# vita-epfl/CrowdNav

Hardware: AMD Instinct MI355X
Metric: env-steps/sec (whole node), 4096 envs x 5 humans, ORCA step (higher is better)
Workload: dtype f32 ORCA solve + f64 env step

## Files before the change

crowdnav_amd/_lib.py:

```python
import ctypes as C
import os

HERE = os.path.dirname(os.path.abspath(__file__))
LIB_PATH = os.environ.get('CROWDNAV_AMD_LIB') or os.path.join(HERE, 'lib', 'libcrowdnav_amd.so')
ABI_VERSION = 12

CN_OK, CN_ERR_INVALID, CN_ERR_UNSUPPORTED, CN_ERR_HIP, CN_ERR_NO_DEVICE = 0, -1, -2, -3, -4
INFO_NAMES = ('Nothing', 'Danger', 'ReachGoal', 'Collision', 'Timeout')
NOTHING, DANGER, REACH_GOAL, COLLISION, TIMEOUT = range(5)
ROBOT_EXTERNAL, ROBOT_ORCA = 0, 1
CIRCLE_CROSSING, SQUARE_CROSSING, MIXED = 0, 1, 2
HOLONOMIC, UNICYCLE = 0, 1
RECORD_FIELDS, SUMMARY_FIELDS = 6, 8
LAUNCH_COUNTERS = ('rollout_kernels', 'scheduled_kernels', 'ring_fills', 'async_fills', 'sarl_narrow', 'sarl_decide_steps')
ROLLOUT_ROUTES = ('generic', 'fused', 'fused_split', 'shard')
SARL_ROUTES = ('lds_tile', 'lds_chunked', 'narrow', 'reg_sarl', 'reg_sarl_chunk', 'reg_cadrl', 'reg_lstm', 'reg_lstm2',
               'split_f16')
PRECISIONS = ('f32', 'f16x2')
FLAG_ASYNC_SCENARIO_FILL = 1
HUMANS_ORCA, HUMANS_CONSTANT_VELOCITY = 0, 1
HUMAN_MODELS = ('orca', 'constant_velocity')
MODES_MEAN, MODES_MIN = 0, 1
MODES_REDUCE = ('mean', 'min')
MODES_MAX = 8
PREDICT_CONSTANT_VELOCITY, PREDICT_TO_GOAL = 0, 1
PREDICT_MODELS = ('constant_velocity', 'to_goal')
PREDICT_ALIASES = {'cv': 'constant_velocity'}


class CrowdNavAmdError(RuntimeError):
    def __init__(self, status, message):
        super().__init__('libcrowdnav_amd: %s (status %d)' % (message, status))
        self.status = status


class CnConfig(C.Structure):
    _fields_ = [
        ('num_envs', C.c_int32), ('num_humans', C.c_int32),
        ('time_step', C.c_double), ('time_limit', C.c_double),
        ('success_reward', C.c_double), ('collision_penalty', C.c_double),
        ('discomfort_dist', C.c_double), ('discomfort_penalty_factor', C.c_double),
        ('robot_visible', C.c_int32), ('robot_policy', C.c_int32),
        ('robot_safety_space', C.c_double), ('human_safety_space', C.c_double),
        ('neighbor_dist', C.c_double),
        ('max_neighbors', C.c_int32), ('scenario_rule', C.c_int32),
        ('time_horizon', C.c_double), ('time_horizon_obst', C.c_double),
        ('circle_radius', C.c_double), ('square_width', C.c_double),
        ('human_radius', C.c_double), ('human_v_pref', C.c_double),
        ('robot_radius', C.c_double), ('robot_v_pref', C.c_double),
        ('randomize_attributes', C.c_int32), ('device', C.c_int32),
        ('robot_kinematics', C.c_int32), ('flags', C.c_int32),
    ]


class CnRolloutIo(C.Structure):
    _fields_ = [
        ('seed_base', C.c_uint32), ('seed_mod', C.c_uint32),
        ('episode_limit', C.c_int64), ('env_offset', C.c_int64), ('env_stride', C.c_int64),
        ('record_capacity', C.c_int32),
        ('ep_outcome', C.c_void_p), ('ep_steps', C.c_void_p), ('ep_return', C.c_void_p),
        ('ep_time', C.c_void_p), ('ep_danger', C.c_void_p), ('ep_danger_dmin_sum', C.c_void_p),
        ('ep_count', C.c_void_p), ('cur_steps', C.c_void_p), ('cur_return', C.c_void_p),
        ('cur_danger', C.c_void_p), ('cur_danger_dmin_sum', C.c_void_p),
        ('active', C.c_void_p), ('transitions', C.c_void_p),
        ('summary', C.c_void_p), ('blocks', C.c_void_p), ('blocks_records', C.c_int32),
        ('env_transitions', C.c_void_p),
    ]


class CnLookaheadOut(C.Structure):
    _fields_ = [
        ('ret', C.c_void_p), ('info', C.c_void_p), ('steps', C.c_void_p), ('time', C.c_void_p),
        ('final_state8', C.c_void_p), ('final_theta', C.c_void_p),
    ]


class CnPathModes(C.Structure):
    _fields_ = [
        ('n_modes', C.c_int32), ('reduce', C.c_int32), ('risk_penalty', C.c_double),
        ('human_vel', C.c_void_p), ('weight', C.c_void_p),
    ]


class CnPredictors(C.Structure):
    _fields_ = [
        ('n_modes', C.c_int32), ('model', C.c_int32 * 8), ('reduce', C.c_int32), ('risk_penalty', C.c_double),
        ('human_vel', C.c_void_p), ('weight', C.c_void_p),
    ]


class CnModesOut(C.Structure):
    _fields_ = [
        ('score', C.c_void_p), ('risk', C.c_void_p), ('worst_mode', C.c_void_p), ('worst_info', C.c_void_p),
        ('worst_steps', C.c_void_p), ('worst_time', C.c_void_p),
        ('ret', C.c_void_p), ('info', C.c_void_p), ('steps', C.c_void_p), ('time', C.c_void_p),
    ]


class CnPlanCfg(C.Structure):
    _fields_ = [
        ('n_steps', C.c_int32), ('n_candidates', C.c_int32), ('n_elites', C.c_int32), ('iterations', C.c_int32),
        ('bootstrap', C.c_int32), ('sort_humans', C.c_int32),
        ('init_std', C.c_double), ('min_std', C.c_double), ('smoothing', C.c_double), ('seed', C.c_uint64),
    ]


class CnPlan(C.Structure):
    _fields_ = [
        ('mean', C.c_void_p), ('std', C.c_void_p), ('best_actions', C.c_void_p), ('best_score', C.c_void_p),
        ('action', C.c_void_p), ('candidates', C.c_void_p), ('look', CnLookaheadOut),
        ('value', C.c_void_p), ('score', C.c_void_p), ('order', C.c_void_p),
    ]


class CnTraceOut(C.Structure):
    _fields_ = [
        ('state8', C.c_void_p), ('episode', C.c_void_p), ('step', C.c_void_p),
        ('reward', C.c_void_p), ('info', C.c_void_p), ('dmin', C.c_void_p),
    ]


class CnSarlConfig(C.Structure):
    _fields_ = [
        ('n_actions', C.c_int32), ('with_om', C.c_int32), ('cell_num', C.c_int32), ('om_channel_size', C.c_int32),
        ('cell_size', C.c_double), ('gamma', C.c_double), ('with_global_state', C.c_int32),
        ('mlp1_dims', C.c_int32 * 2), ('mlp2_dims', C.c_int32 * 2), ('attention_dims', C.c_int32 * 3),
        ('mlp3_dims', C.c_int32 * 4), ('model', C.c_int32), ('interaction_dims', C.c_int32 * 4),
        ('constant_velocity_model', C.c_int32), ('precision', C.c_int32),
    ]


_P = C.c_void_p
SYMBOLS = {
    'cn_last_error': (C.c_char_p, []),
    'cn_abi_version': (C.c_int, []),
    'cn_create': (C.c_int, [C.POINTER(CnConfig), C.POINTER(_P)]),
    'cn_destroy': (C.c_int, [_P]),
    'cn_set_stream': (C.c_int, [_P, _P]),
    'cn_sync': (C.c_int, [_P]),
    'cn_set_state': (C.c_int, [_P, _P, _P]),
    'cn_get_state': (C.c_int, [_P, _P, _P]),
    'cn_set_theta': (C.c_int, [_P, _P]),
    'cn_get_theta': (C.c_int, [_P, _P]),
    'cn_get_human_count': (C.c_int, [_P, _P]),
    'cn_drop_robot_sim': (C.c_int, [_P]),
    'cn_drop_sims': (C.c_int, [_P]),
    'cn_set_robot_sim': (C.c_int, [_P, _P, C.c_float]),
    'cn_reset': (C.c_int, [_P, _P, _P, _P]),
    'cn_orca': (C.c_int, [_P, _P]),
    'cn_step': (C.c_int, [_P, _P, C.c_int, _P, _P, _P, _P, _P, _P, _P]),
    'cn_set_gamma': (C.c_int, [_P, C.c_double]),
    'cn_rollout_begin': (C.c_int, [_P, C.POINTER(CnRolloutIo)]),
    'cn_rollout': (C.c_int, [_P, C.POINTER(CnRolloutIo), C.c_int]),
    'cn_rollout_step': (C.c_int, [_P, C.POINTER(CnRolloutIo), _P]),
    'cn_sarl_configure': (C.c_int, [_P, C.POINTER(CnSarlConfig), _P]),
    'cn_sarl_set_weights': (C.c_int, [_P, C.POINTER(_P)]),
    'cn_sarl_select': (C.c_int, [_P, _P, _P, _P]),
    'cn_sarl_select_attention': (C.c_int, [_P, _P, _P, _P, _P]),
    'cn_sarl_explore': (C.c_int, [_P, C.c_double, _P, _P, _P, _P]),
    'cn_sarl_transform': (C.c_int, [_P, _P, C.c_int64, C.c_int]),
    'cn_sarl_sample_step': (C.c_int, [_P, C.c_double, _P, _P, _P, _P, C.c_int64, C.c_int, _P, _P, _P, _P]),
    'cn_sarl_values': (C.c_int, [_P, _P, C.c_int64, _P]),
    'cn_sarl_export': (C.c_int, [_P, C.c_int, _P, C.c_uint64]),
    'cn_rollout_records': (C.c_int, [_P, C.POINTER(CnRolloutIo), C.c_int, _P]),
    'cn_gather_records': (C.c_int, [_P, _P, C.c_int, C.c_int, _P, _P]),
    'cn_records_summary': (C.c_int, [_P, C.c_int64, C.c_int, C.c_int, _P, _P]),
    'cn_rollout_summary': (C.c_int, [_P, C.POINTER(CnRolloutIo), _P]),
    'cn_launch_counts': (C.c_int, [_P, _P]),
    'cn_lagged_fills': (C.c_int, [_P, _P]),
    'cn_mt_random': (C.c_int, [_P, C.c_uint32, C.c_int, _P]),
    'cn_trainer_create': (C.c_int, [C.POINTER(CnSarlConfig), C.c_int, C.c_int, C.c_int, C.POINTER(_P)]),
    'cn_trainer_destroy': (C.c_int, [_P]),
    'cn_trainer_set_stream': (C.c_int, [_P, _P]),
    'cn_train_step': (C.c_int, [_P, C.POINTER(_P), C.POINTER(_P), _P, _P, C.c_int64, _P, C.c_int64, C.c_double, C.c_double, _P]),
    'cn_trainer_steps': (C.c_int, [_P, C.POINTER(C.c_int64)]),
    'cn_rollout_trace': (C.c_int, [_P, C.POINTER(CnRolloutIo), C.c_int, C.POINTER(CnTraceOut)]),
    'cn_rollout_route': (C.c_int, [_P, C.c_int, C.POINTER(C.c_int)]),
    'cn_sarl_network_route': (C.c_int, [_P, C.POINTER(C.c_int)]),
    'cn_rollout_actions': (C.c_int, [_P, C.POINTER(CnRolloutIo), C.c_int, _P, C.POINTER(CnTraceOut)]),
    'cn_lookahead_actions': (C.c_int, [_P, C.c_int, C.c_int, _P, C.POINTER(CnLookaheadOut)]),
    'cn_lookahead_set_human_model': (C.c_int, [_P, C.c_int]),
    'cn_lookahead_get_human_model': (C.c_int, [_P, C.POINTER(C.c_int)]),
    'cn_sarl_state_values': (C.c_int, [_P, _P, _P, C.c_int64, C.c_int, _P]),
    'cn_lookahead_values': (C.c_int, [_P, C.c_int, C.c_int, _P, C.POINTER(CnLookaheadOut), C.c_int, _P, _P]),
    'cn_plan_reset': (C.c_int, [_P, C.POINTER(CnPlanCfg), C.POINTER(CnPlan), _P]),
    'cn_plan_draw': (C.c_int, [_P, C.POINTER(CnPlanCfg), C.POINTER(CnPlan), C.c_uint32]),
    'cn_plan_refit': (C.c_int, [_P, C.POINTER(CnPlanCfg), C.POINTER(CnPlan), C.c_int]),
    'cn_plan_cem': (C.c_int, [_P, C.POINTER(CnPlanCfg), C.POINTER(CnPlan), C.c_uint32]),
    'cn_plan_shift': (C.c_int, [_P, C.POINTER(CnRolloutIo), C.POINTER(CnPlanCfg), C.POINTER(CnPlan)]),
    'cn_plan_rollout': (C.c_int, [_P, C.POINTER(CnRolloutIo), C.c_int, C.POINTER(CnPlanCfg), C.POINTER(CnPlan), C.c_uint32]),
    'cn_plan_mppi_update': (C.c_int, [_P, C.POINTER(CnPlanCfg), C.POINTER(CnPlan), C.c_double, C.c_int, C.c_int]),
    'cn_plan_mppi': (C.c_int, [_P, C.POINTER(CnPlanCfg), C.POINTER(CnPlan), C.c_double, C.c_int, C.c_uint32]),
    'cn_plan_mppi_rollout': (C.c_int, [_P, C.POINTER(CnRolloutIo), C.c_int, C.POINTER(CnPlanCfg), C.POINTER(CnPlan), C.c_double,
                                       C.c_int, C.c_uint32]),
    'cn_lookahead_paths': (C.c_int, [_P, C.c_int, C.c_int, _P, _P, C.POINTER(CnLookaheadOut)]),
    'cn_lookahead_paths_values': (C.c_int, [_P, C.c_int, C.c_int, _P, _P, C.POINTER(CnLookaheadOut), C.c_int, _P, _P]),
    'cn_plan_cem_paths': (C.c_int, [_P, C.POINTER(CnPlanCfg), C.POINTER(CnPlan), _P, C.c_uint32]),
    'cn_plan_mppi_paths': (C.c_int, [_P, C.POINTER(CnPlanCfg), C.POINTER(CnPlan), _P, C.c_double, C.c_int, C.c_uint32]),
    'cn_lookahead_modes': (C.c_int, [_P, C.c_int, C.c_int, _P, C.POINTER(CnPathModes), C.POINTER(CnModesOut)]),
    'cn_plan_cem_modes': (C.c_int, [_P, C.POINTER(CnPlanCfg), C.POINTER(CnPlan), C.POINTER(CnPathModes), C.c_uint32]),
    'cn_plan_mppi_modes': (C.c_int, [_P, C.POINTER(CnPlanCfg), C.POINTER(CnPlan), C.POINTER(CnPathModes), C.c_double, C.c_int,
                                     C.c_uint32]),
    'cn_predict': (C.c_int, [_P, C.c_int, C.c_int, C.POINTER(C.c_int32), _P]),
    'cn_plan_cem_predict_rollout': (C.c_int, [_P, C.POINTER(CnRolloutIo), C.c_int, C.POINTER(CnPlanCfg), C.POINTER(CnPlan),
                                              C.POINTER(CnPredictors), C.c_uint32]),
    'cn_plan_mppi_predict_rollout': (C.c_int, [_P, C.POINTER(CnRolloutIo), C.c_int, C.POINTER(CnPlanCfg), C.POINTER(CnPlan),
                                               C.POINTER(CnPredictors), C.c_double, C.c_int, C.c_uint32]),
    'cn_predict_orca': (C.c_int, [_P, C.c_int, C.c_int, C.c_int, _P]),
    'cn_plan_cem_predict_orca_rollout': (C.c_int, [_P, C.POINTER(CnRolloutIo), C.c_int, C.POINTER(CnPlanCfg), C.POINTER(CnPlan),
                                                   C.POINTER(CnPredictors), C.c_int, C.c_uint32]),
    'cn_plan_mppi_predict_orca_rollout': (C.c_int, [_P, C.POINTER(CnRolloutIo), C.c_int, C.POINTER(CnPlanCfg), C.POINTER(CnPlan),
                                                    C.POINTER(CnPredictors), C.c_int, C.c_double, C.c_int, C.c_uint32]),
    'cn_predict_orca_robot': (C.c_int, [_P, C.c_int, C.c_int, C.c_int, _P, C.c_int64, _P]),
    'cn_plan_cem_predict_orca_nominal_rollout': (C.c_int, [_P, C.POINTER(CnRolloutIo), C.c_int, C.POINTER(CnPlanCfg),
                                                           C.POINTER(CnPlan), C.POINTER(CnPredictors), C.c_int, C.c_uint32]),
    'cn_plan_mppi_predict_orca_nominal_rollout': (C.c_int, [_P, C.POINTER(CnRolloutIo), C.c_int, C.POINTER(CnPlanCfg),
                                                            C.POINTER(CnPlan), C.POINTER(CnPredictors), C.c_int, C.c_double, C.c_int,
                                                            C.c_uint32]),
}

_lib = None


def load():
    global _lib
    if _lib is not None:
        return _lib
    if not os.path.exists(LIB_PATH):
        raise ImportError(
            'crowdnav_amd: %s is missing. Build the HIP library first (make -C crowdnav_amd/csrc, or '
            '__graft_entry__.build()); there is no CPU fallback.' % LIB_PATH)
    lib = C.CDLL(LIB_PATH)
    for name, (res, args) in SYMBOLS.items():
        fn = getattr(lib, name)
        fn.restype = res
        fn.argtypes = args
    got = lib.cn_abi_version()
    if got != ABI_VERSION:
        raise ImportError('crowdnav_amd: library ABI %d != binding ABI %d; rebuild' % (got, ABI_VERSION))
    _lib = lib
    return lib


def check(status):
    if status != CN_OK:
        raise CrowdNavAmdError(status, load().cn_last_error().decode('utf-8', 'replace'))
```

crowdnav_amd/csrc/crowdnav_amd.hip:

```cpp
#include "engine_host.h"
#include "scenario_ring_host.h"
#include "rollout_fused.h"
#include "records_kernels.h"
#include "lookahead_cv_kernel.h"
#include "lookahead_modes_kernel.h"

thread_local char cn_g_err[512] = "";

void cn_launch_orca(cn_engine* e, float* out_vel) {
    pick_maxl(e, [&](auto maxl) {
        pick_bool(e->P.kd, [&](auto kd) {
            hipLaunchKernelGGL((cn::orca_kernel<decltype(maxl)::value, decltype(kd)::value>), dim3(grid_envs(e)), dim3(e->P.threads),
                               e->smem, e->stream, e->P, e->S, out_vel);
        });
    });
}

static bool headline_geometry(const cn::Params& P) {
    return P.A == 6 && P.NC == 5 && P.E == 2 && P.nA == 12 && P.pairs == 60 && P.threads == 64;
}

template <class F>
static void pick_fused(const cn_engine* e, int route, F&& f) {
    if (route == CN_ROUTE_FUSED_SPLIT) {
        if (e->split_assist & cn::kAssistHead) f(cn::rollout_fused_kernel<true, true, cn::kAssistHead>, 2 * cn::kWave);
        else f(cn::rollout_fused_kernel<true, true>, 2 * cn::kWave);
    } else if (headline_geometry(e->P)) {
        f(cn::rollout_fused_kernel<true>, cn::kWave);
    } else {
        f(cn::rollout_fused_kernel<false>, cn::kWave);
    }
}

int cn_lookahead_check(const cn_engine* e, int n_steps, int n_candidates, const double* actions, const cn_lookahead_out* out) {
    if (!actions) return fail(CN_ERR_INVALID, "cn_lookahead_actions: actions is NULL");
    if (!out) return fail(CN_ERR_INVALID, "cn_lookahead_actions: out is NULL");
    if (!out->ret) return fail(CN_ERR_INVALID, "cn_lookahead_actions: out->ret is NULL");
    if (!out->info) return fail(CN_ERR_INVALID, "cn_lookahead_actions: out->info is NULL");
    if (!out->steps) return fail(CN_ERR_INVALID, "cn_lookahead_actions: out->steps is NULL");
    if (!out->time) return fail(CN_ERR_INVALID, "cn_lookahead_actions: out->time is NULL");
    if (n_steps < 0) return fail(CN_ERR_INVALID, "cn_lookahead_actions: n_steps must be >= 0 (got %d)", n_steps);
    if (n_candidates < 1) return fail(CN_ERR_INVALID, "cn_lookahead_actions: n_candidates must be >= 1 (got %d)", n_candidates);
    if (!e) return fail(CN_ERR_INVALID, "cn_lookahead_actions: engine is NULL");
    if (e->P.robot_orca)
        return fail(CN_ERR_INVALID, "cn_lookahead_actions is for CN_ROBOT_EXTERNAL engines (an ORCA robot takes no actions)");
    const uint64_t virtual_envs = (uint64_t)e->P.B * (uint64_t)n_candidates, rows = virtual_envs * (uint64_t)n_steps;
    if (virtual_envs > (uint64_t)INT32_MAX - cn::kWave)
        return fail(CN_ERR_UNSUPPORTED, "cn_lookahead_actions: num_envs * n_candidates = %llu exceeds the %llu branches a launch "
                    "indexes", (unsigned long long)virtual_envs, (unsigned long long)((uint64_t)INT32_MAX - cn::kWave));
    if (rows > ((uint64_t)1 << 59))
        return fail(CN_ERR_UNSUPPORTED, "cn_lookahead_actions: num_envs * n_candidates * n_steps = %llu action rows exceed 2^59",
                    (unsigned long long)rows);
    if (!e->discount || e->discount_len <= 0)
        return fail(CN_ERR_INVALID, "cn_lookahead_actions: the engine has no discount table (cn_set_gamma)");
    return CN_OK;
}

static int upload_look(cn_engine* e, const cn_lookahead_out* out) {
    if (!e->look_valid || std::memcmp(&e->look_host, out, sizeof(*out)) != 0) {
        e->look_host = *out;
        CN_HIP(hipMemcpyAsync(e->look_dev, &e->look_host, sizeof(*out), hipMemcpyHostToDevice, e->stream));
        e->look_valid = true;
    }
    return CN_OK;
}

static cn::CvParams cv_params(const cn_engine* e, int n_steps, int n_candidates) {
    const cn::Params& P = e->P;
    cn::CvParams C{};
    C.B = P.B, C.K = n_candidates, C.A = P.A, C.n_steps = n_steps;
    C.chunks = (n_candidates + cn::kWave - 1) / cn::kWave;
    C.discount_len = e->discount_len, C.discount = e->discount;
    C.dt = P.dt, C.time_limit = P.time_limit, C.success_reward = P.success_reward, C.collision_penalty = P.collision_penalty;
    C.discomfort_dist = P.discomfort_dist, C.discomfort_factor = P.discomfort_factor;
    C.pos = e->S.pos, C.vel = e->S.vel, C.goal = e->S.goal, C.rv = e->S.rv, C.gtime = e->S.gtime, C.theta = e->S.theta;
    return C;
}

extern "C" {

const char* cn_last_error(void) { return cn_g_err; }
int cn_abi_version(void) { return CN_ABI_VERSION; }

static int check_config(const cn_config* c) {
    if (c->num_envs < 1) return fail(CN_ERR_INVALID, "num_envs must be >= 1 (got %d)", c->num_envs);
    if (c->num_humans < 1 || c->num_humans > 63)
        return fail(CN_ERR_UNSUPPORTED, "num_humans must be in 1..63 (got %d)", c->num_humans);
    if (c->max_neighbors < 0 || c->max_neighbors > cn::kMaxNb)
        return fail(CN_ERR_UNSUPPORTED, "max_neighbors must be in 0..%d (got %d)", cn::kMaxNb, c->max_neighbors);
    if (!(c->time_step > 0.0)) return fail(CN_ERR_INVALID, "time_step must be > 0");
    if (c->scenario_rule != CN_CIRCLE_CROSSING && c->scenario_rule != CN_SQUARE_CROSSING && c->scenario_rule != CN_MIXED)
        return fail(CN_ERR_UNSUPPORTED, "scenario_rule %d not supported", c->scenario_rule);
    if (c->scenario_rule == CN_MIXED) {
        if (c->num_humans < 5 || c->num_humans > 8)
            return fail(CN_ERR_UNSUPPORTED, "scenario_rule mixed draws up to 5 humans per episode: num_humans must be in 5..8 (got %d)",
                        c->num_humans);
        if (c->randomize_attributes && c->robot_policy == CN_ROBOT_ORCA)
            return fail(CN_ERR_UNSUPPORTED,
                        "mixed + randomize_attributes + the ORCA robot: the reference rebuilds the robot's rvo2 simulator "
                        "whenever the number of humans changes (orca.py:95-98), which the per-env radius capture does not model");
    }
    if (c->robot_policy != CN_ROBOT_EXTERNAL && c->robot_policy != CN_ROBOT_ORCA)
        return fail(CN_ERR_INVALID, "robot_policy %d unknown", c->robot_policy);
    if (c->robot_kinematics != CN_HOLONOMIC && c->robot_kinematics != CN_UNICYCLE)
        return fail(CN_ERR_INVALID, "robot_kinematics %d unknown", c->robot_kinematics);
    if (c->robot_kinematics == CN_UNICYCLE && c->robot_policy == CN_ROBOT_ORCA)
        return fail(CN_ERR_INVALID, "the ORCA robot policy is holonomic (orca.py:59); a unicycle robot needs CN_ROBOT_EXTERNAL");
    int ndev = 0;
    if (hipGetDeviceCount(&ndev) != hipSuccess || ndev == 0)
        return fail(CN_ERR_NO_DEVICE, "no HIP device visible: the MI355X engine has no CPU fallback");
    if (c->device < 0 || c->device >= ndev) return fail(CN_ERR_INVALID, "device %d out of range", c->device);
    return CN_OK;
}

static void copy_config(cn_engine* e) {
    const cn_config* c = &e->cfg;
    cn::Params& P = e->P;
    P.robot_visible = c->robot_visible ? 1 : 0;
    P.robot_orca = c->robot_policy == CN_ROBOT_ORCA;
    P.robot_unicycle = c->robot_kinematics == CN_UNICYCLE;
    P.dt = c->time_step;
    P.time_limit = c->time_limit;
    P.success_reward = c->success_reward;
    P.collision_penalty = c->collision_penalty;
    P.discomfort_dist = c->discomfort_dist;
    P.discomfort_factor = c->discomfort_penalty_factor;
    P.robot_safety = c->robot_safety_space;
    P.human_safety = c->human_safety_space;
    P.orca.neighbor_dist = (float)c->neighbor_dist;
    P.orca.inv_time_horizon = 1.0f / (float)c->time_horizon;
    P.orca.inv_time_step = 1.0f / (float)c->time_step;
    P.orca.max_neighbors = c->max_neighbors;
    e->C.num_agents = c->num_humans + 1;
    e->C.rule = c->scenario_rule;
    e->C.randomize = c->randomize_attributes ? 1 : 0;
    e->C.circle_radius = c->circle_radius;
    e->C.square_width = c->square_width;
    e->C.discomfort_dist = c->discomfort_dist;
    e->C.human_radius = c->human_radius;
    e->C.human_v_pref = c->human_v_pref;
    e->C.robot_radius = c->robot_radius;
    e->C.robot_v_pref = c->robot_v_pref;
}

static void pick_geometry(cn_engine* e) {
    const cn_config* c = &e->cfg;
    cn::Params& P = e->P;
    P.B = c->num_envs;
    P.A = c->num_humans + 1;
    P.NC = P.A - 1;
    const int e_max = cn::kWave / P.A;
    const bool small_lp = (P.NC < c->max_neighbors ? P.NC : c->max_neighbors) <= 5;
    int e_want = env_int("CROWDNAV_AMD_ENVS_PER_WAVE", small_lp ? (P.B > 2048 ? 2 : 1) : (P.B + 4095) / 4096);
    P.E = e_want < 1 ? 1 : (e_want > e_max ? e_max : e_want);
    int w_want = env_int("CROWDNAV_AMD_WAVES_PER_BLOCK", 1);
    const int w_useful = (P.E * P.A * P.NC + cn::kWave - 1) / cn::kWave;
    if (w_want > w_useful) w_want = w_useful;
    if (w_want > cn::kMaxBlock / cn::kWave) w_want = cn::kMaxBlock / cn::kWave;
    P.threads = cn::kWave * (w_want < 1 ? 1 : w_want);
    P.nA = P.E * P.A;
    P.pairs = P.nA * P.NC;
    e->maxl = small_lp ? 5 : 10;
    P.kd = P.A > cn::kKdLeaf ? 1 : 0;
    P.kdl = cn::kd_layout(P.nA, P.A, P.E);
    e->smem = cn::smem_bytes(P.nA, P.pairs, e->maxl, P.A, P.E);
}

static void read_knobs(cn_engine* e) {
    const cn_config* c = &e->cfg;
    cn::Params& P = e->P;
    P.sched = -1;
    e->sched_min = env_int("CROWDNAV_AMD_SCHED_MIN_STEPS", 24);
    e->sched_force = env_int("CROWDNAV_AMD_SCHED_FORCE", 0) != 0;
    e->sched_reserve = env_int("CROWDNAV_AMD_DYN_RESERVE", 0);
    e->sched_dynamic = env_int("CROWDNAV_AMD_SCHED_DYNAMIC", 1) != 0;
    e->dyn_visits = env_int("CROWDNAV_AMD_DYN_VISITS", 0);
    P.dyn_visits = 3;
    e->use_fused = env_int("CROWDNAV_AMD_FUSED", 1) != 0;
    e->fused_split = env_int("CROWDNAV_AMD_FUSED_SPLIT", 1);
    e->split_assist = env_int("CROWDNAV_AMD_SPLIT_ASSIST", 1) != 0 ? cn::kAssistHead : 0;
    int cap_log2 = env_int("CROWDNAV_AMD_MAX_ATTEMPTS_LOG2", c->num_humans > 8 ? 23 : 20);
    if (cap_log2 < 6) cap_log2 = 6;
    if (cap_log2 > 40) cap_log2 = 40;
    e->C.max_attempts = 1ull << cap_log2;
    hipDeviceProp_t prop;
    const bool ok = hipGetDeviceProperties(&prop, c->device) == hipSuccess && prop.multiProcessorCount > 0;
    e->sched_slots = 12 * (ok ? prop.multiProcessorCount : 256);
    e->ring.configure(e, ok ? prop.multiProcessorCount : 256);
    e->split_slots = 0;
    if (ok && headline_geometry(P))
        pick_fused(e, CN_ROUTE_FUSED_SPLIT, [&](auto kernel, int threads) {
            int per_cu = 0;
            if (hipOccupancyMaxActiveBlocksPerMultiprocessor(&per_cu, kernel, threads, e->smem) == hipSuccess)
                e->split_slots = per_cu * prop.multiProcessorCount;
        });
}

static int alloc_state(cn_engine* e) {
    const cn::Params& P = e->P;
    const size_t n = (size_t)P.B * P.A;
    int rc = CN_OK;
    cn::StateView& S = e->S;
    if ((rc = dev_alloc(e, &S.pos, n)) || (rc = dev_alloc(e, &S.vel, n)) || (rc = dev_alloc(e, &S.goal, n)) ||
        (rc = dev_alloc(e, &S.rv, n)) || (rc = dev_alloc(e, &S.gtime, (size_t)P.B)) ||
        (rc = dev_alloc(e, &S.theta, (size_t)P.B)) ||
        (rc = dev_alloc(e, &S.rsim_radius, n)) || (rc = dev_alloc(e, &S.rsim_max_speed, (size_t)P.B)) ||
        (rc = dev_alloc(e, &S.rsim_valid, (size_t)P.B)) || (rc = dev_alloc(e, &S.mt_key, (size_t)624 * P.B)) ||
        (rc = dev_alloc(e, &S.mt_pos, (size_t)P.B)) || (rc = dev_alloc(e, &e->probe_key, (size_t)624)) ||
        (rc = e->ring.create(e)) ||
        (rc = dev_alloc(e, &e->summary_scratch, (size_t)cn::kSummaryBlocks * cn::kSummaryFields + 1)) ||
        (rc = dev_alloc(e, &S.ep_word, (size_t)P.B)) || (rc = dev_alloc(e, &S.dyn_queue, (size_t)P.B + 1)) ||
        (rc = dev_alloc(e, &S.kd_order, P.kd ? n * cn::kd_row_bytes(P.A) : (size_t)4)) ||
        (rc = dev_alloc(e, &S.kd_valid, P.kd ? n : (size_t)4)) ||
        (rc = dev_alloc(e, &S.wg_partial, (size_t)P.B * (CN_SUMMARY_FIELDS + 1))) ||
        (rc = dev_alloc(e, &S.group_partial, (size_t)cn::kEpilogueGroups * (CN_SUMMARY_FIELDS + 1))) ||
        (rc = dev_alloc(e, &S.tickets, (size_t)(cn::kEpilogueGroups + 1) * cn::kTicketStride)) ||
        (rc = dev_alloc(e, &e->io_dev, (size_t)1)) || (rc = dev_alloc(e, &e->C.error, (size_t)1)) ||
        (rc = dev_alloc(e, &e->S_dev, (size_t)1)) || (rc = dev_alloc(e, &e->look_dev, (size_t)1)))
        return rc;
    e->S.error = e->C.error;
    if (hipMemcpy(e->S_dev, &e->S, sizeof(cn::StateView), hipMemcpyHostToDevice) != hipSuccess)
        return fail(CN_ERR_HIP, "cn_create: state view upload failed");
    return CN_OK;
}

int cn_create(const cn_config* c, cn_engine** out) {
    if (!c || !out) return fail(CN_ERR_INVALID, "cn_create: NULL argument");
    *out = nullptr;
    int rc = check_config(c);
    if (rc) return rc;
    CN_HIP(hipSetDevice(c->device));

    cn_engine* e = new (std::nothrow) cn_engine();
    if (!e) return fail(CN_ERR_INVALID, "out of host memory");
    e->cfg = *c;
    copy_config(e);
    pick_geometry(e);
    read_knobs(e);
    if ((rc = alloc_state(e)) || (rc = cn_set_gamma(e, 0.9))) {
        cn_destroy(e);
        return rc;
    }
    *out = e;
    return CN_OK;
}

int cn_destroy(cn_engine* e) {
    if (!e) return CN_OK;
    (void)hipSetDevice(e->cfg.device);
    (void)hipStreamSynchronize(e->stream);
    e->ring.destroy();
    e->alloc_rollback(cn_engine::AllocMark{});
    if (e->discount) (void)hipFree(e->discount);
    cn_sarl_release(e);
    delete e;
    return CN_OK;
}

int cn_set_stream(cn_engine* e, void* hip_stream) {
    if (!e) return fail(CN_ERR_INVALID, "engine is NULL");
    e->stream = static_cast<hipStream_t>(hip_stream);
    e->orca_fresh = false;
    return CN_OK;
}

int cn_sync(cn_engine* e) {
    int rc = bind(e);
    if (rc) return rc;
    CN_HIP(hipStreamSynchronize(e->stream));
    if ((rc = e->ring.drain(e))) return rc;
    int gen_error = 0;
    CN_HIP(hipMemcpy(&gen_error, e->C.error, sizeof(int), hipMemcpyDeviceToHost));
    if (gen_error) {
        CN_HIP(hipMemset(e->C.error, 0, sizeof(int)));
        if (gen_error & 4)
            return fail(CN_ERR_HIP,
                        "the shard kernel's dynamic schedule: a workgroup waited ~2 s for an env's previous visit and went on "
                        "without it (results of this rollout are not to be trusted); CROWDNAV_AMD_SCHED_DYNAMIC=0 selects the "
                        "static schedule");
        if (gen_error & 2)
            return fail(CN_ERR_INVALID,
                        "cn_sarl_explore needs each env's numpy stream: (re)start the episodes with cn_reset (the scenario "
                        "ring of cn_rollout_* and the wave generator used for more than 8 humans do not keep it)");
        return fail(CN_ERR_INVALID,
                    "scenario generation gave up on a human after %llu rejected placements (the reference's rejection "
                    "sampling would not have terminated either: too many humans for this circle/square); the affected "
                    "scenario holds an overlapping placement",
                    e->C.max_attempts);
    }
    return CN_OK;
}

namespace {

__global__ void pack_state_kernel(int n, const double* state8, cn::StateView S) {
    const int i = blockIdx.x * blockDim.x + threadIdx.x;
    if (i >= n) return;
    const double* s = state8 + (size_t)i * 8;
    S.pos[i] = make_double2(s[0], s[1]);
    S.vel[i] = make_double2(s[2], s[3]);
    S.goal[i] = make_double2(s[4], s[5]);
    S.rv[i] = make_double2(s[6], s[7]);
}

__global__ void unpack_state_kernel(int n, double* state8, cn::StateView S) {
    const int i = blockIdx.x * blockDim.x + threadIdx.x;
    if (i >= n) return;
    double* s = state8 + (size_t)i * 8;
    const double2 p = S.pos[i], v = S.vel[i], g = S.goal[i], q = S.rv[i];
    s[0] = p.x, s[1] = p.y, s[2] = v.x, s[3] = v.y, s[4] = g.x, s[5] = g.y, s[6] = q.x, s[7] = q.y;
}

}

int cn_set_state(cn_engine* e, const double* state8, const double* global_time) {
    int rc = bind(e);
    if (rc || (rc = e->ring.settle(e))) return rc;
    const int n = e->P.B * e->P.A;
    if (state8) hipLaunchKernelGGL(pack_state_kernel, dim3((n + 255) / 256), dim3(256), 0, e->stream, n, state8, e->S);
    if (global_time)
        CN_HIP(hipMemcpyAsync(e->S.gtime, global_time, sizeof(double) * e->P.B, hipMemcpyDeviceToDevice, e->stream));
    CN_HIP(hipGetLastError());
    return CN_OK;
}

int cn_get_state(cn_engine* e, double* state8, double* global_time) {
    int rc = bind(e);
    if (rc || (rc = e->ring.settle(e))) return rc;
    const int n = e->P.B * e->P.A;
    if (state8) hipLaunchKernelGGL(unpack_state_kernel, dim3((n + 255) / 256), dim3(256), 0, e->stream, n, state8, e->S);
    if (global_time)
        CN_HIP(hipMemcpyAsync(global_time, e->S.gtime, sizeof(double) * e->P.B, hipMemcpyDeviceToDevice, e->stream));
    CN_HIP(hipGetLastError());
    return CN_OK;
}

int cn_set_theta(cn_engine* e, const double* theta) {
    int rc = bind(e);
    if (rc) return rc;
    if (!theta) return fail(CN_ERR_INVALID, "cn_set_theta: NULL");
    CN_HIP(hipMemcpyAsync(e->S.theta, theta, sizeof(double) * e->P.B, hipMemcpyDeviceToDevice, e->stream));
    return CN_OK;
}

int cn_get_theta(cn_engine* e, double* theta) {
    int rc = bind(e);
    if (rc) return rc;
    if (!theta) return fail(CN_ERR_INVALID, "cn_get_theta: NULL");
    CN_HIP(hipMemcpyAsync(theta, e->S.theta, sizeof(double) * e->P.B, hipMemcpyDeviceToDevice, e->stream));
    return CN_OK;
}

namespace {
__global__ void human_count_kernel(int B, int A, const double2* pos, int32_t* out) {
    const int b = blockIdx.x * blockDim.x + threadIdx.x;
    if (b >= B) return;
    int n = 0;
    for (int i = 1; i < A; ++i) n += cn::is_parked(pos[(size_t)b * A + i]) ? 0 : 1;
    out[b] = n;
}
}

int cn_get_human_count(cn_engine* e, int32_t* count) {
    int rc = bind(e);
    if (rc) return rc;
    if (!count) return fail(CN_ERR_INVALID, "cn_get_human_count: NULL");
    hipLaunchKernelGGL(human_count_kernel, dim3((e->P.B + 255) / 256), dim3(256), 0, e->stream, e->P.B, e->P.A, e->S.pos, count);
    CN_HIP(hipGetLastError());
    return CN_OK;
}

namespace {
__global__ void set_robot_sim_kernel(int B, int A, const float* radii, float max_speed, cn::StateView S) {
    const int i = blockIdx.x * blockDim.x + threadIdx.x;
    if (i >= B * A) return;
    S.rsim_radius[i] = radii[i % A];
    if (i % A == 0) {
        S.rsim_max_speed[i / A] = max_speed;
        S.rsim_valid[i / A] = 1;
    }
}
}

int cn_set_robot_sim(cn_engine* e, const float* radii_host, float max_speed) {
    int rc = bind(e);
    if (rc) return rc;
    if (!radii_host) return fail(CN_ERR_INVALID, "cn_set_robot_sim: NULL");
    float* staged = reinterpret_cast<float*>(e->probe_key);
    CN_HIP(hipMemcpyAsync(staged, radii_host, sizeof(float) * e->P.A, hipMemcpyHostToDevice, e->stream));
    CN_HIP(hipStreamSynchronize(e->stream));
    hipLaunchKernelGGL(set_robot_sim_kernel, dim3((e->P.B * e->P.A + 255) / 256), dim3(256), 0, e->stream, e->P.B, e->P.A,
                       staged, max_speed, e->S);
    CN_HIP(hipGetLastError());
    return CN_OK;
}

int cn_drop_robot_sim(cn_engine* e) {
    int rc = bind(e);
    if (rc) return rc;
    CN_HIP(hipMemsetAsync(e->S.rsim_valid, 0, (size_t)e->P.B, e->stream));
    if (e->P.kd)
        CN_HIP(hipMemset2DAsync(e->S.kd_valid, (size_t)e->P.A, 0, 1, (size_t)e->P.B, e->stream));
    return CN_OK;
}

int cn_drop_sims(cn_engine* e) {
    int rc = cn_drop_robot_sim(e);
    if (rc) return rc;
    if (e->P.kd) CN_HIP(hipMemsetAsync(e->S.kd_valid, 0, (size_t)e->P.B * e->P.A, e->stream));
    return CN_OK;
}

int cn_reset(cn_engine* e, const uint32_t* seeds, const uint8_t* mask, uint64_t* draws) {
    int rc = bind(e);
    if (rc || (rc = e->ring.settle(e))) return rc;
    if (!seeds) return fail(CN_ERR_INVALID, "cn_reset: seeds is NULL");
    if (e->ring.gen_wave)
        hipLaunchKernelGGL(cn::reset_wave_kernel, dim3(e->P.B), dim3(cn::kWave), 0, e->stream, e->P, e->C, e->S, seeds, mask,
                           draws);
    else
        hipLaunchKernelGGL(cn::reset_kernel, dim3(grid_lanes(e)), dim3(cn::kWave), 0, e->stream, e->P, e->C, e->S, seeds, mask,
                           draws);
    CN_HIP(hipGetLastError());
    return CN_OK;
}

int cn_orca(cn_engine* e, float* out_vel) {
    int rc = bind(e);
    if (rc) return rc;
    if (!out_vel) return fail(CN_ERR_INVALID, "cn_orca: out_vel is NULL");
    cn_launch_orca(e, out_vel);
    CN_HIP(hipGetLastError());
    return CN_OK;
}

int cn_step(cn_engine* e, const double* action, int update, double* reward, uint8_t* done, uint8_t* info,
            double* dmin, double* action_out, float* orca_vel, double* obs) {
    int rc = bind(e);
    if (rc || (rc = e->ring.settle(e))) return rc;
    if (!reward || !done || !info) return fail(CN_ERR_INVALID, "cn_step: reward/done/info must not be NULL");
    if (e->P.robot_orca && action)
        return fail(CN_ERR_INVALID, "cn_step: action must be NULL when robot_policy == CN_ROBOT_ORCA");
    if (!e->P.robot_orca && !action)
        return fail(CN_ERR_INVALID, "cn_step: action is required when robot_policy == CN_ROBOT_EXTERNAL");
    cn::StepIo io{action, reward, done, info, dmin, action_out, orca_vel, obs, update ? 1 : 0};
    pick_maxl_uni_kd(e, [&](auto maxl, auto uni, auto kd) {
        hipLaunchKernelGGL((cn::step_kernel<decltype(maxl)::value, decltype(uni)::value, decltype(kd)::value>), dim3(grid_envs(e)),
                           dim3(e->P.threads), e->smem, e->stream, e->P, e->S, io);
    });
    CN_HIP(hipGetLastError());
    return CN_OK;
}

int cn_set_gamma(cn_engine* e, double gamma) {
    int rc = bind(e);
    if (rc) return rc;
    const int len = (int)std::ceil(e->cfg.time_limit / e->cfg.time_step) + 8;
    if (len > cn::kMaxDiscount)
        return fail(CN_ERR_UNSUPPORTED, "time_limit / time_step = %d steps per episode exceeds the %d the rollout kernel tabulates",
                    len - 8, cn::kMaxDiscount - 8);
    std::vector<double> table((size_t)len);
    for (int t = 0; t < len; ++t) table[(size_t)t] = std::pow(gamma, t * e->cfg.time_step * e->cfg.robot_v_pref);
    CN_HIP(hipStreamSynchronize(e->stream));
    if (e->discount) CN_HIP(hipFree(e->discount));
    e->discount = nullptr;
    CN_HIP(hipMalloc(reinterpret_cast<void**>(&e->discount), sizeof(double) * len));
    CN_HIP(hipMemcpy(e->discount, table.data(), sizeof(double) * len, hipMemcpyHostToDevice));
    e->discount_len = len;
    return CN_OK;
}

static int upload_io(cn_engine* e, const cn_rollout_io* io) {
    if (e->io_valid && std::memcmp(&e->io_host, io, sizeof(*io)) == 0) return CN_OK;
    if (e->rollout_begun && (io->seed_base != e->begin_seed_base || io->seed_mod != e->begin_seed_mod))
        return fail(CN_ERR_INVALID, "rollout io: seed_base / seed_mod (%u / %u) differ from cn_rollout_begin's (%u / %u); call "
                    "cn_rollout_begin to renumber the episodes", io->seed_base, io->seed_mod, e->begin_seed_base, e->begin_seed_mod);
    int rc = e->ring.drain(e);
    if (rc) return rc;
    e->io_host = *io;
    CN_HIP(hipMemcpyAsync(e->io_dev, &e->io_host, sizeof(*io), hipMemcpyHostToDevice, e->stream));
    e->io_valid = true;
    return CN_OK;
}

static int check_io(const cn_engine* e, const cn_rollout_io* io) {
    if (!io) return fail(CN_ERR_INVALID, "rollout io is NULL");
    if (io->seed_mod == 0) return fail(CN_ERR_INVALID, "seed_mod must be >= 1");
    if (!io->ep_count || !io->cur_steps || !io->cur_return || !io->active)
        return fail(CN_ERR_INVALID, "rollout io: ep_count, cur_steps, cur_return and active are required");
    if (io->record_capacity < 0) return fail(CN_ERR_INVALID, "record_capacity must be >= 0");
    if (io->blocks && io->blocks_records < 1) return fail(CN_ERR_INVALID, "rollout io: blocks needs blocks_records >= 1");
    if (io->env_offset < 0 || io->env_stride < io->env_offset + e->P.B)
        return fail(CN_ERR_INVALID, "rollout io: need env_offset >= 0 and env_stride >= env_offset + num_envs");
    return CN_OK;
}

int cn_rollout_begin(cn_engine* e, const cn_rollout_io* io) {
    int rc = bind(e);
    if (rc) return rc;
    if ((rc = check_io(e, io)) || (rc = e->ring.drain(e))) return rc;
    e->rollout_begun = false;
    if ((rc = upload_io(e, io))) return rc;
    e->rollout_begun = true, e->begin_seed_base = io->seed_base, e->begin_seed_mod = io->seed_mod;
    return e->ring.begin(e, io->seed_mod);
}

static int rollout_route(const cn_engine* e, const double* action) {
    const cn::Params& P = e->P;
    static const bool use_geom20 = env_int("CROWDNAV_AMD_GEOM20", 1) != 0;
    if (e->use_fused && e->ring.mode != ScenarioRing::Fill::WorkList && e->maxl == 5 && !P.robot_unicycle && P.NC <= cn::kFusedMaxNC && P.pairs <= cn::kWave &&
        P.nA * 5 <= cn::kWave && P.threads == cn::kWave) {
#if defined(CN_PHASE_TIMING) || defined(CN_WAVE_TRACE)
        (void)action;
        return CN_ROUTE_FUSED;
#else
        const bool split = e->fused_split != 0 && headline_geometry(P) && P.robot_orca && action == nullptr &&
                           (grid_envs(e) <= e->split_slots || e->fused_split == 2);
        return split ? CN_ROUTE_FUSED_SPLIT : CN_ROUTE_FUSED;
#endif
    }
    if (use_geom20 && e->maxl == 10 && !P.robot_unicycle && P.A == 21 && P.NC == 20 && P.E == 1 && P.threads == 64 &&
        P.orca.max_neighbors == 10 && P.kd)
        return CN_ROUTE_SHARD;
    return CN_ROUTE_GENERIC;
}

static void launch_shard(cn_engine* e, const cn::RolloutView& R, const int* levels, int n_steps, const double* action) {
    const cn::Params& P = e->P;
    const size_t smem20 = cn::smem_bytes_compact(P.nA, P.pairs, P.A, P.E);
    const auto launch = [&](const cn::Params& Pk, int grid, int steps) {
        hipLaunchKernelGGL((cn::rollout_kernel<10, false, true, true>), dim3(grid), dim3(64), smem20, e->stream, Pk,
                           (const cn::StateView*)e->S_dev, levels, R, steps, action);
    };
    cn::Params Pk = e->P;
    Pk.sched = -1;
    const int slots = e->sched_slots;
    const bool beside_generators = e->ring.mode == ScenarioRing::Fill::WorkList;
    const int reserve = beside_generators ? e->sched_reserve : 0;
    const int G = P.B < slots - reserve ? P.B : slots - reserve;
    int visits = e->dyn_visits > 0 ? e->dyn_visits : (n_steps + 28) / 56;
    if (visits < 3) visits = 3;
    if (visits > n_steps) visits = n_steps;
    Pk.dyn_visits = visits;
    const bool helps = e->sched_force || beside_generators || P.B > G;
    if (e->sched_dynamic && G > 0 && n_steps >= e->sched_min && action == nullptr && helps && !e->io_host.summary &&
        !e->io_host.blocks) {
        (void)hipMemsetAsync(e->S.dyn_queue, 0, sizeof(int) * ((size_t)P.B + 1), e->stream);
        Pk.sched = cn::kSchedDynamic;
        e->launch_counts[CN_COUNT_ROLLOUT_KERNELS] += 1;
        e->launch_counts[CN_COUNT_SCHEDULED_KERNELS] += 1;
        launch(Pk, G, n_steps);
        return;
    }
    const int rounds_plain = (P.B + slots - 1) / slots, rounds_sched = (P.B / 4 * 3 + slots - 1) / slots;
    const bool sched = P.B % 4 == 0 && n_steps >= (e->sched_min > 48 ? e->sched_min : 48) && action == nullptr &&
                       (e->sched_force || 4 * rounds_sched < 3 * rounds_plain);
    const int q = sched ? n_steps / 3 : 0, rest = n_steps - 3 * q;
    e->launch_counts[CN_COUNT_ROLLOUT_KERNELS] += (rest > 0 ? 1 : 0) + (q > 0 ? 4 : 0);
    e->launch_counts[CN_COUNT_SCHEDULED_KERNELS] += q > 0 ? 4 : 0;
    if (rest > 0) launch(Pk, grid_envs(e), rest);
    for (int k = 0; k < 4 && q > 0; ++k) {
        Pk.sched = k;
        launch(Pk, P.B / 4 * 3, q);
    }
}

static void launch_rollout(cn_engine* e, const cn::RolloutView& R, const int* levels, int n_steps, const double* action) {
    const int route = rollout_route(e, action);
    if (route == CN_ROUTE_SHARD) return launch_shard(e, R, levels, n_steps, action);
    if (route == CN_ROUTE_GENERIC)
        pick_maxl_uni_kd(e, [&](auto maxl, auto uni, auto kd) {
            hipLaunchKernelGGL((cn::rollout_kernel<decltype(maxl)::value, decltype(uni)::value, false, decltype(kd)::value>),
                               dim3(grid_envs(e)), dim3(e->P.threads), e->smem, e->stream, e->P, (const cn::StateView*)e->S_dev,
                               levels, R, n_steps, action);
        });
    else
        pick_fused(e, route, [&](auto kernel, int threads) {
            hipLaunchKernelGGL(kernel, dim3(grid_envs(e)), dim3(threads), e->smem, e->stream, e->P, (const cn::StateView*)e->S_dev,
                               levels, R, n_steps, action);
        });
    e->launch_counts[CN_COUNT_ROLLOUT_KERNELS] += 1;
}

enum { kNothingToLaunch = 1, kWrongRobotPolicy = 2, kNoAction = 3 };
static int rollout_prepare(cn_engine* e, const cn_rollout_io* io, int n_steps, bool need_orca_robot,
                           const double* action = nullptr) {
    int rc = bind(e);
    if (rc) return rc;
    if ((rc = check_io(e, io))) return rc;
    if (n_steps < 0) return fail(CN_ERR_INVALID, "n_steps must be >= 0");
    if (n_steps == 0) return kNothingToLaunch;
    if ((e->P.robot_orca != 0) != need_orca_robot) return kWrongRobotPolicy;
    if (!need_orca_robot && !action) return kNoAction;
    return upload_io(e, io);
}

int cn_rollout(cn_engine* e, const cn_rollout_io* io, int n_steps) {
    const int rc = rollout_prepare(e, io, n_steps, true);
    if (rc == kNothingToLaunch) return CN_OK;
    if (rc == kWrongRobotPolicy)
        return fail(CN_ERR_UNSUPPORTED, "cn_rollout needs an on-device robot policy (robot_policy == CN_ROBOT_ORCA); with "
                                        "CN_ROBOT_EXTERNAL use cn_rollout_step(action)");
    if (rc) return rc;
    return e->ring.around_launch(e, n_steps, [&](const cn::RolloutView& R, const int* levels) {
        launch_rollout(e, R, levels, n_steps, nullptr);
    });
}

int cn_rollout_trace(cn_engine* e, const cn_rollout_io* io, int n_steps, const cn_trace_out* out) {
    if (!e) return fail(CN_ERR_INVALID, "cn_rollout_trace: engine is NULL");
    if (!out) return fail(CN_ERR_INVALID, "cn_rollout_trace: out is NULL");
    if (!out->state8) return fail(CN_ERR_INVALID, "cn_rollout_trace: out->state8 is NULL");
    if (!out->episode) return fail(CN_ERR_INVALID, "cn_rollout_trace: out->episode is NULL");
    if (!out->step) return fail(CN_ERR_INVALID, "cn_rollout_trace: out->step is NULL");
    if (!e->P.robot_orca)
        return fail(CN_ERR_UNSUPPORTED, "cn_rollout_trace needs an on-device robot policy (robot_policy == CN_ROBOT_ORCA); with "
                                        "CN_ROBOT_EXTERNAL use cn_rollout_step(action)");
    const int rc = rollout_prepare(e, io, n_steps, true);
    if (rc == kNothingToLaunch) return CN_OK;
    if (rc) return rc;
    const cn_trace_out T = *out;
    return e->ring.around_launch(e, n_steps, [&](const cn::RolloutView& R, const int* levels) {
        pick_maxl(e, [&](auto maxl) {
            pick_bool(e->P.kd, [&](auto kd) {
                hipLaunchKernelGGL((cn::rollout_trace_kernel<decltype(maxl)::value, decltype(kd)::value>), dim3(grid_envs(e)),
                                   dim3(e->P.threads), e->smem, e->stream, e->P, (const cn::StateView*)e->S_dev, levels, R, n_steps,
                                   T);
            });
        });
        e->launch_counts[CN_COUNT_ROLLOUT_KERNELS] += 1;
    });
}

int cn_rollout_step(cn_engine* e, const cn_rollout_io* io, const double* action) {
    const int rc = rollout_prepare(e, io, 1, false, action);
    if (rc == kWrongRobotPolicy) return fail(CN_ERR_INVALID, "cn_rollout_step is for CN_ROBOT_EXTERNAL engines (use cn_rollout)");
    if (rc == kNoAction) return fail(CN_ERR_INVALID, "cn_rollout_step: action is NULL");
    if (rc) return rc;
    return e->ring.around_launch(e, 1, [&](const cn::RolloutView& R, const int* levels) { launch_rollout(e, R, levels, 1, action); });
}

int cn_rollout_actions(cn_engine* e, const cn_rollout_io* io, int n_steps, const double* actions, const cn_trace_out* out) {
    if (!actions) return fail(CN_ERR_INVALID, "cn_rollout_actions: actions is NULL");
    if (out && !out->state8) return fail(CN_ERR_INVALID, "cn_rollout_actions: out->state8 is NULL");
    if (out && !out->episode) return fail(CN_ERR_INVALID, "cn_rollout_actions: out->episode is NULL");
    if (out && !out->step) return fail(CN_ERR_INVALID, "cn_rollout_actions: out->step is NULL");
    if (n_steps < 0) return fail(CN_ERR_INVALID, "n_steps must be >= 0");
    if (!e) return fail(CN_ERR_INVALID, "cn_rollout_actions: engine is NULL");
    if (e->P.robot_orca)
        return fail(CN_ERR_INVALID, "cn_rollout_actions is for CN_ROBOT_EXTERNAL engines (use cn_rollout)");
    const int rc = rollout_prepare(e, io, n_steps, false, actions);
    if (rc == kNothingToLaunch) return CN_OK;
    if (rc) return rc;
    return e->ring.around_launch(e, n_steps, [&](const cn::RolloutView& R, const int* levels) {
        pick_maxl_uni_kd(e, [&](auto maxl, auto uni, auto kd) {
            constexpr int kMaxl = decltype(maxl)::value;
            constexpr bool kUni = decltype(uni)::value, kKd = decltype(kd)::value;
            if (out)
                hipLaunchKernelGGL((cn::rollout_actions_trace_kernel<kMaxl, kUni, kKd>), dim3(grid_envs(e)), dim3(e->P.threads),
                                   e->smem, e->stream, e->P, (const cn::StateView*)e->S_dev, levels, R, n_steps, actions, *out);
            else
                hipLaunchKernelGGL((cn::rollout_actions_kernel<kMaxl, kUni, kKd>), dim3(grid_envs(e)), dim3(e->P.threads), e->smem,
                                   e->stream, e->P, (const cn::StateView*)e->S_dev, levels, R, n_steps, actions);
        });
        e->launch_counts[CN_COUNT_ROLLOUT_KERNELS] += 1;
    });
}

int cn_lookahead_actions(cn_engine* e, int n_steps, int n_candidates, const double* actions, const cn_lookahead_out* out) {
    int rc = cn_lookahead_check(e, n_steps, n_candidates, actions, out);
    if (rc || n_steps == 0) return rc;
    if ((rc = bind(e)) || (rc = upload_look(e, out))) return rc;
    const uint64_t virtual_envs = (uint64_t)e->P.B * (uint64_t)n_candidates;
    if (e->look_human_model == CN_HUMANS_CONSTANT_VELOCITY) {
        const cn::CvParams C = cv_params(e, n_steps, n_candidates);
        pick_bool(e->P.robot_unicycle, [&](auto uni) {
            hipLaunchKernelGGL((cn::lookahead_cv_kernel<decltype(uni)::value>), dim3((unsigned)C.B * (unsigned)C.chunks),
                               dim3(cn::kWave), 0, e->stream, C, actions, (const cn_lookahead_out*)e->look_dev);
        });
        CN_HIP(hipGetLastError());
        return CN_OK;
    }
    cn::Params Pv = e->P;
    Pv.B = (int)virtual_envs;
    const cn::RolloutView R{nullptr, e->discount, e->discount_len};
    pick_maxl_uni_kd(e, [&](auto maxl, auto uni, auto kd) {
        hipLaunchKernelGGL((cn::rollout_lookahead_kernel<decltype(maxl)::value, decltype(uni)::value, decltype(kd)::value>),
                           dim3((Pv.B + Pv.E - 1) / Pv.E), dim3(Pv.threads), e->smem, e->stream, Pv, (const cn::StateView*)e->S_dev, R,
                           n_steps, actions, (const cn_lookahead_out*)e->look_dev, n_candidates);
    });
    CN_HIP(hipGetLastError());
    return CN_OK;
}

int cn_lookahead_paths(cn_engine* e, int n_steps, int n_candidates, const double* actions, const double* human_vel,
                       const cn_lookahead_out* out) {
    if (!human_vel) return fail(CN_ERR_INVALID, "cn_lookahead_paths: human_vel is NULL");
    int rc = cn_lookahead_check(e, n_steps, n_candidates, actions, out);
    if (rc || n_steps == 0) return rc;
    if ((rc = bind(e)) || (rc = upload_look(e, out))) return rc;
    const cn::CvParams C = cv_params(e, n_steps, n_candidates);
    pick_bool(e->P.robot_unicycle, [&](auto uni) {
        hipLaunchKernelGGL((cn::lookahead_paths_kernel<decltype(uni)::value>), dim3((unsigned)C.B * (unsigned)C.chunks),
                           dim3(cn::kWave), 0, e->stream, C, actions, human_vel, (const cn_lookahead_out*)e->look_dev);
    });
    CN_HIP(hipGetLastError());
    return CN_OK;
}

int cn_lookahead_modes(cn_engine* e, int n_steps, int n_candidates, const double* actions, const cn_path_modes* modes,
                       const cn_modes_out* out) {
    if (!modes) return fail(CN_ERR_INVALID, "cn_lookahead_modes: modes is NULL");
    if (!modes->human_vel) return fail(CN_ERR_INVALID, "cn_lookahead_modes: modes->human_vel is NULL");
    if (!out) return fail(CN_ERR_INVALID, "cn_lookahead_modes: out is NULL");
    if (!out->score) return fail(CN_ERR_INVALID, "cn_lookahead_modes: out->score is NULL");
    if (modes->n_modes < 1) return fail(CN_ERR_INVALID, "cn_lookahead_modes: n_modes must be >= 1 (got %d)", modes->n_modes);
    if (modes->n_modes > cn::kModesMax)
        return fail(CN_ERR_UNSUPPORTED, "cn_lookahead_modes: n_modes = %d exceeds the %d modes a lane keeps in registers",
                    modes->n_modes, cn::kModesMax);
    if (modes->reduce != CN_MODES_MEAN && modes->reduce != CN_MODES_MIN)
        return fail(CN_ERR_INVALID, "cn_lookahead_modes: reduce %d unknown (CN_MODES_MEAN = 0, CN_MODES_MIN = 1)", modes->reduce);
    if (!(modes->risk_penalty >= 0.0) || !std::isfinite(modes->risk_penalty))
        return fail(CN_ERR_INVALID, "cn_lookahead_modes: risk_penalty must be >= 0 and finite (got %g)", modes->risk_penalty);
    const cn_lookahead_out probe{out->score, reinterpret_cast<uint8_t*>(out->score), reinterpret_cast<int32_t*>(out->score),
                                 out->score, nullptr, nullptr};
    int rc = cn_lookahead_check(e, n_steps, n_candidates, actions, &probe);
    if (rc) return rc;
    const uint64_t mode_rows = (uint64_t)e->P.B * (uint64_t)n_candidates * (uint64_t)modes->n_modes;
    if (mode_rows > (uint64_t)INT32_MAX)
        return fail(CN_ERR_UNSUPPORTED, "cn_lookahead_modes: num_envs * n_candidates * n_modes = %llu exceeds the %llu per-mode "
                    "rows a launch indexes", (unsigned long long)mode_rows, (unsigned long long)INT32_MAX);
    if (n_steps == 0) return CN_OK;
    if ((rc = bind(e))) return rc;
    const cn::CvParams C = cv_params(e, n_steps, n_candidates);
    const cn::ModesParams Q{modes->n_modes, modes->reduce, modes->risk_penalty, modes->human_vel, modes->weight, *out};
    const size_t lds = cn::modes_lds_bytes(Q.M, C.A - 1);
    pick_bool(e->P.robot_unicycle, [&](auto uni) {
        hipLaunchKernelGGL((cn::lookahead_modes_kernel<decltype(uni)::value>), dim3((unsigned)C.B * (unsigned)C.chunks),
                           dim3(cn::kWave), lds, e->stream, C, actions, Q);
    });
    CN_HIP(hipGetLastError());
    return CN_OK;
}

int cn_lookahead_set_human_model(cn_engine* e, int model) {
    if (!e) return fail(CN_ERR_INVALID, "cn_lookahead_set_human_model: engine is NULL");
    if (model != CN_HUMANS_ORCA && model != CN_HUMANS_CONSTANT_VELOCITY)
        return fail(CN_ERR_INVALID, "cn_lookahead_set_human_model: model %d unknown (CN_HUMANS_ORCA = 0, "
                    "CN_HUMANS_CONSTANT_VELOCITY = 1)", model);
    e->look_human_model = model;
    return CN_OK;
}

int cn_lookahead_get_human_model(const cn_engine* e, int* model_host) {
    if (!e) return fail(CN_ERR_INVALID, "cn_lookahead_get_human_model: engine is NULL");
    if (!model_host) return fail(CN_ERR_INVALID, "cn_lookahead_get_human_model: model_host is NULL");
    *model_host = e->look_human_model;
    return CN_OK;
}

int cn_rollout_route(cn_engine* e, int n_steps, int* route_host) {
    if (!e || !route_host) return fail(CN_ERR_INVALID, "cn_rollout_route: NULL argument");
    if (n_steps < 0) return fail(CN_ERR_INVALID, "n_steps must be >= 0");
    *route_host = rollout_route(e, nullptr);
    return CN_OK;
}

int cn_lagged_fills(cn_engine* e, uint64_t* count_host) {
    if (!e || !count_host) return fail(CN_ERR_INVALID, "cn_lagged_fills: NULL argument");
    *count_host = e->ring.lagged_fills;
    return CN_OK;
}

int cn_launch_counts(cn_engine* e, uint64_t* counts_host) {
    if (!e || !counts_host) return fail(CN_ERR_INVALID, "cn_launch_counts: NULL argument");
    for (int i = 0; i < CN_LAUNCH_COUNTERS; ++i) counts_host[i] = e->launch_counts[i];
    return CN_OK;
}

int cn_rollout_records(cn_engine* e, const cn_rollout_io* io, int max_records, double* blocks) {
    int rc = bind(e);
    if (rc) return rc;
    if ((rc = check_io(e, io))) return rc;
    if (max_records < 1 || !blocks) return fail(CN_ERR_INVALID, "cn_rollout_records: need max_records >= 1 and blocks");
    if ((rc = upload_io(e, io))) return rc;
    const int n = e->P.B * max_records;
    hipLaunchKernelGGL(cn::records_pack_kernel, dim3((n + 255) / 256), dim3(256), 0, e->stream, e->P.B, max_records, e->io_dev,
                       blocks);
    CN_HIP(hipGetLastError());
    return CN_OK;
}

int cn_records_summary(cn_engine* e, int64_t n_envs, int max_records, int record_capacity, const double* blocks,
                       double* summary) {
    int rc = bind(e);
    if (rc) return rc;
    if (n_envs < 0 || max_records < 1 || record_capacity < 0 || !blocks || !summary)
        return fail(CN_ERR_INVALID, "cn_records_summary: bad arguments");
    const cn::BlockRecords src{blocks, cn::record_block_doubles(max_records)};
    if (n_envs * max_records <= cn::kSummarySmallItems)
        hipLaunchKernelGGL(cn::records_summary_small_kernel<cn::BlockRecords>, dim3(1), dim3(cn::kSummarySmallThreads), 0, e->stream,
                           n_envs, max_records, record_capacity, src, summary);
    else
        hipLaunchKernelGGL(cn::records_summary_kernel<cn::BlockRecords>, dim3(cn::kSummaryBlocks), dim3(cn::kSummaryThreads), 0,
                           e->stream, n_envs, max_records, record_capacity, src, summary, e->summary_scratch);
    CN_HIP(hipGetLastError());
    return CN_OK;
}

int cn_rollout_summary(cn_engine* e, const cn_rollout_io* io, double* summary) {
    int rc = bind(e);
    if (rc) return rc;
    if ((rc = check_io(e, io))) return rc;
    if (!summary) return fail(CN_ERR_INVALID, "cn_rollout_summary: summary is NULL");
    if (io->record_capacity < 1) return fail(CN_ERR_INVALID, "cn_rollout_summary: the rollout keeps no records (record_capacity 0)");
    if ((rc = upload_io(e, io))) return rc;
    if ((int64_t)e->P.B * io->record_capacity <= cn::kSummarySmallItems)
        hipLaunchKernelGGL(cn::records_summary_small_kernel<cn::RingRecords>, dim3(1), dim3(cn::kSummarySmallThreads), 0, e->stream,
                           (int64_t)e->P.B, io->record_capacity, io->record_capacity, cn::RingRecords{e->io_dev}, summary);
    else
        hipLaunchKernelGGL(cn::records_summary_kernel<cn::RingRecords>, dim3(cn::kSummaryBlocks), dim3(cn::kSummaryThreads), 0,
                           e->stream, (int64_t)e->P.B, io->record_capacity, io->record_capacity, cn::RingRecords{e->io_dev}, summary,
                           e->summary_scratch);
    CN_HIP(hipGetLastError());
    return CN_OK;
}

namespace {
struct RcclApi {
    int (*all_gather)(const void*, void*, size_t, int, void*, hipStream_t);
    const char* (*error_string)(int);
    bool ok;
};
const RcclApi* rccl_api() {
    static RcclApi api = [] {
        RcclApi a{};
        void* h = dlopen("librccl.so.1", RTLD_NOW | RTLD_GLOBAL);
        if (!h) h = dlopen("/opt/rocm/lib/librccl.so.1", RTLD_NOW | RTLD_GLOBAL);
        if (!h) return a;
        a.all_gather = reinterpret_cast<int (*)(const void*, void*, size_t, int, void*, hipStream_t)>(dlsym(h, "ncclAllGather"));
        a.error_string = reinterpret_cast<const char* (*)(int)>(dlsym(h, "ncclGetErrorString"));
        a.ok = a.all_gather && a.error_string;
        return a;
    }();
    return &api;
}
constexpr int kNcclFloat64 = 8;
}

int cn_gather_records(cn_engine* e, void* rccl_comm, int n_ranks, int max_records, const double* blocks,
                      double* blocks_all) {
    int rc = bind(e);
    if (rc) return rc;
    if (!rccl_comm || n_ranks < 1 || max_records < 1 || !blocks || !blocks_all)
        return fail(CN_ERR_INVALID, "cn_gather_records: bad arguments");
    const RcclApi* api = rccl_api();
    if (!api->ok) return fail(CN_ERR_UNSUPPORTED, "cn_gather_records: librccl.so.1 could not be loaded");
    const size_t n = (size_t)e->P.B * cn::record_block_doubles(max_records);
    const int st = api->all_gather(blocks, blocks_all, n, kNcclFloat64, rccl_comm, e->stream);
    if (st) return fail(CN_ERR_HIP, "cn_gather_records: RCCL error %d (%s)", st, api->error_string(st));
    return CN_OK;
}

int cn_mt_random(cn_engine* e, uint32_t seed, int n, double* out) {
    int rc = bind(e);
    if (rc) return rc;
    if (n < 0 || !out) return fail(CN_ERR_INVALID, "cn_mt_random: bad arguments");
    hipLaunchKernelGGL(cn::mt_probe_kernel, dim3(1), dim3(1), 0, e->stream, e->probe_key, seed, n, out);
    CN_HIP(hipGetLastError());
    return CN_OK;
}

}

#ifdef CN_PHASE_TIMING
extern "C" int cn_debug_phase_cycles(unsigned long long* out16, int reset) {
    if (out16 && hipMemcpyFromSymbol(out16, HIP_SYMBOL(cn::cn_phase_cycles), 16 * sizeof(unsigned long long)) != hipSuccess) return -1;
    if (reset) {
        unsigned long long zero[16] = {};
        zero[13] = ~0ull;
        if (hipMemcpyToSymbol(HIP_SYMBOL(cn::cn_phase_cycles), zero, sizeof(zero)) != hipSuccess) return -1;
    }
    return 0;
}
#endif
#ifdef CN_PHASE_TIMING
extern "C" int cn_debug_lazy_counts(unsigned long long* out8, int reset) {
    if (out8 && hipMemcpyFromSymbol(out8, HIP_SYMBOL(cn::cn_lazy_counts), 16 * sizeof(unsigned long long)) != hipSuccess) return -1;
    if (reset) {
        unsigned long long zero[16] = {};
        if (hipMemcpyToSymbol(HIP_SYMBOL(cn::cn_lazy_counts), zero, sizeof(zero)) != hipSuccess) return -1;
    }
    return 0;
}
#endif
#ifdef CN_SPLIT_PROBE
extern "C" int cn_debug_split_probe(unsigned long long* out32, int reset) {
    if (out32 && hipMemcpyFromSymbol(out32, HIP_SYMBOL(cn::cn_split_probe), 32 * sizeof(unsigned long long)) != hipSuccess) return -1;
    if (reset) {
        unsigned long long zero[32] = {};
        if (hipMemcpyToSymbol(HIP_SYMBOL(cn::cn_split_probe), zero, sizeof(zero)) != hipSuccess) return -1;
    }
    return 0;
}
#endif
#ifdef CN_WAVE_TRACE
extern "C" int cn_debug_wave_trace(unsigned long long* out, int waves) {
    if (waves > 8192) waves = 8192;
    return hipMemcpyFromSymbol(out, HIP_SYMBOL(cn::cn_wave_trace), (size_t)waves * 6 * sizeof(unsigned long long)) == hipSuccess ? 0 : -1;
}
#endif
```

crowdnav_amd/csrc/engine_host.h:

```cpp
#pragma once
#include <hip/hip_runtime.h>

#include <cmath>
#include <cstdarg>
#include <cstdio>
#include <cstdlib>
#include <cstring>
#include <dlfcn.h>
#include <new>
#include <type_traits>
#include <utility>
#include <vector>

#include "../../include/crowdnav_amd.h"
#include "fill_plan.h"
#include "step_kernels.h"



extern thread_local char cn_g_err[512];

namespace {

[[maybe_unused]] int fail(int code, const char* fmt, ...) {
    va_list ap;
    va_start(ap, fmt);
    vsnprintf(cn_g_err, sizeof(cn_g_err), fmt, ap);
    va_end(ap);
    return code;
}

#define CN_HIP(call)                                                                              \
    do {                                                                                          \
        hipError_t err__ = (call);                                                                \
        if (err__ != hipSuccess)                                                                  \
            return fail(CN_ERR_HIP, "%s failed: %s (%s:%d)", #call, hipGetErrorString(err__), __FILE__, \
                        __LINE__);                                                                \
    } while (0)

}

struct ScenarioRing {
    enum class Fill { InFront, Beside, WorkList };
    static constexpr int kFillStreams = 8;
    bool gen_wave = false;
    Fill mode = Fill::InFront;
    bool scenario_cache = true;
    cn::FillPlan plan;
    hipStream_t fill_streams[kFillStreams] = {};
    hipEvent_t rollout_done = nullptr;
    hipEvent_t fill_done = nullptr;
    int next_fill_stream = 0;
    int* fill_list = nullptr;
    int fill_queue_wgs = 1;
    int* ep_snap = nullptr;
    uint64_t lagged_fills = 0;

    void configure(cn_engine* e, int compute_units);
    int create(cn_engine* e);
    void destroy();
    int begin(cn_engine* e, uint32_t seed_mod);
    template <class Launch>
    int around_launch(cn_engine* e, int n_steps, Launch&& launch);
    int settle(cn_engine* e);
    int drain(cn_engine* e);
};

struct cn_engine {
    cn_config cfg{};
    cn::Params P{};
    cn::ScenarioCfg C{};
    cn::StateView S{};
    hipStream_t stream = nullptr;
    cn_rollout_io io_host{};
    cn_rollout_io* io_dev = nullptr;
    cn::StateView* S_dev = nullptr;
    cn_lookahead_out look_host{};
    cn_lookahead_out* look_dev = nullptr;
    bool look_valid = false;
    int look_human_model = CN_HUMANS_ORCA;
    ScenarioRing ring;
    bool io_valid = false;
    bool rollout_begun = false;
    uint32_t begin_seed_base = 0, begin_seed_mod = 0;
    struct cn_sarl* sarl = nullptr;
    bool orca_fresh = false;
    double* discount = nullptr;
    int discount_len = 0;
    uint32_t* probe_key = nullptr;
    double* summary_scratch = nullptr;
    int maxl = 10;
    size_t smem = 0;
    int sched_min = 0, sched_slots = 0, sched_reserve = 0, dyn_visits = 0;
    bool sched_force = false, sched_dynamic = true;
    bool use_fused = true;
    int fused_split = 1;
    int split_assist = 0;
    int split_slots = 0;
    uint64_t launch_counts[CN_LAUNCH_COUNTERS] = {};
    struct Slab {
        char* base;
        size_t size, used;
    };
    std::vector<Slab> slabs;
    struct AllocMark {
        std::vector<size_t> used;
    };
    AllocMark alloc_mark() const {
        AllocMark m;
        for (const Slab& s : slabs) m.used.push_back(s.used);
        return m;
    }
    void alloc_rollback(const AllocMark& m) {
        while (slabs.size() > m.used.size()) {
            (void)hipFree(slabs.back().base);
            slabs.pop_back();
        }
        for (size_t i = 0; i < slabs.size(); ++i) slabs[i].used = m.used[i];
    }
};

namespace {

constexpr size_t kSlabBytes = (size_t)32 << 20, kSlabAlign = 4096;

template <typename T>
int dev_alloc(cn_engine* e, T** out, size_t n) {
    const size_t bytes = (n * sizeof(T) + kSlabAlign - 1) / kSlabAlign * kSlabAlign;
    size_t k = 0;
    while (k < e->slabs.size() && e->slabs[k].used + bytes > e->slabs[k].size) ++k;
    if (k == e->slabs.size()) {
        const size_t size = bytes > kSlabBytes ? (bytes + ((size_t)2 << 20) - 1) >> 21 << 21 : kSlabBytes;
        void* p = nullptr;
        CN_HIP(hipMalloc(&p, size));
        e->slabs.push_back({static_cast<char*>(p), size, 0});
    }
    cn_engine::Slab& sl = e->slabs[k];
    void* p = sl.base + sl.used;
    sl.used += bytes;
    CN_HIP(hipMemset(p, 0, bytes));
    *out = static_cast<T*>(p);
    return CN_OK;
}

[[maybe_unused]] int bind(cn_engine* e) {
    if (!e) return fail(CN_ERR_INVALID, "engine is NULL");
    e->orca_fresh = false;
    CN_HIP(hipSetDevice(e->cfg.device));
    return CN_OK;
}

inline int grid_envs(const cn_engine* e) { return (e->P.B + e->P.E - 1) / e->P.E; }

template <int... Vs, class F>
inline bool pick_int(int v, F&& f) {
    return ((v == Vs ? (f(std::integral_constant<int, Vs>{}), true) : false) || ...);
}
template <class F>
inline void pick_bool(bool b, F&& f) {
    if (b) f(std::true_type{});
    else f(std::false_type{});
}
template <class F>
inline void pick_maxl(const cn_engine* e, F&& f) {
    if (!pick_int<5>(e->maxl, f)) f(std::integral_constant<int, 10>{});
}
template <class F>
inline void pick_maxl_uni_kd(const cn_engine* e, F&& f) {
    pick_maxl(e, [&](auto maxl) {
        pick_bool(e->P.robot_unicycle, [&](auto uni) { pick_bool(e->P.kd, [&](auto kd) { f(maxl, uni, kd); }); });
    });
}

[[maybe_unused]] int env_int(const char* name, int fallback) {
    const char* v = std::getenv(name);
    return (v && *v) ? std::atoi(v) : fallback;
}
inline int grid_lanes(const cn_engine* e) { return (e->P.B + cn::kWave - 1) / cn::kWave; }

}


void cn_sarl_release(cn_engine* e);
void cn_launch_orca(cn_engine* e, float* out_vel);
int cn_lookahead_check(const cn_engine* e, int n_steps, int n_candidates, const double* actions, const cn_lookahead_out* out);
```

crowdnav_amd/csrc/rollout_fused.h:

```cpp
#pragma once
#include "rollout_kernels.h"

namespace cn {

constexpr int kFusedMaxNC = 5;

template <typename T>
__device__ __forceinline__ T in_vgpr(T x) {
    asm volatile("" : "+v"(x));
    return x;
}

__device__ __forceinline__ void stage_agent(const Params& P, const Smem& s, const Lane& L, const AgentRegs& r,
                                            double human_safety, float4* kin) {
    if (L.lane >= P.nA) return;
    kin[L.lane] = make_float4((float)r.px, (float)r.py, (float)r.vx, (float)r.vy);
    s.posd[L.lane] = make_double2(r.px, r.py);
    s.rad[L.lane] = r.rad;
    s.hview[L.lane] = (float)(r.rad + 0.01 + human_safety);
}

__device__ __forceinline__ void preferred_velocity(const AgentRegs& r, float max_speed, bool solve, float4& sol, float4& start) {
    const double gdx = r.gx - r.px, gdy = r.gy - r.py;
    const double speed = norm2(gdx, gdy);
// ... 32 lines not shown
template <typename Mid>
__device__ __forceinline__ void fused_pair_body(const Params& P, const Smem& s, const PairRow& pr, float range_sq, float rsum,
                                                const float4 me, const float4 other, Mid&& mid) {
    const int my_info = pr.my_info;
    const int q = my_info & 0xff, c = (my_info >> 16) & 0xff;
    const float odx = me.x - other.x, ody = me.y - other.y;
    const float mine = odx * odx + ody * ody;
    uint32_t vbk[kFusedMaxNC];
#pragma unroll
    for (int k = 0; k < kFusedMaxNC; ++k) {
        const uint32_t got = (uint32_t)__builtin_amdgcn_ds_bpermute(pr.xbase + 4 * k, (int)__float_as_uint(mine));
        vbk[k] = k < P.NC ? got : 0x7f800000u;
    }
    int rank = 0, within = 0;
    {
        const uint32_t mb = __float_as_uint(mine), rb = __float_as_uint(range_sq);
        uint32_t before = 0u, inside = 0u;
#pragma unroll
        for (int k = 0; k < kFusedMaxNC; ++k) {
            const uint32_t vb = vbk[k];
            const uint32_t tie = (uint32_t)(k - c) >> 31;
            before = __builtin_amdgcn_alignbit(before, vb - mb - tie, 31);
            inside = __builtin_amdgcn_alignbit(inside, vb - rb, 31);
        }
        within = __popc(inside);
        rank = __popc(before & inside);
    }
    mid();
    if (c == 0) s.count[q] = within < P.orca.max_neighbors ? within : P.orca.max_neighbors;
    if (mine < range_sq && rank < P.orca.max_neighbors)
        s.lines[q * kLineStride + rank] =
            make_half_plane(P.orca, me.x, me.y, me.z, me.w, other.x, other.y, other.z, other.w, rsum);
}
template <typename Mid>
__device__ __forceinline__ void fused_pair_phase(const Params& P, const Smem& s, const PairRow& pr, float range_sq, float rsum,
                                                 Mid&& mid) {
    const float4 me = s.kin[pr.my_info & 0xff];
    const float4 other = s.kin[pr.my_slot];
    fused_pair_body(P, s, pr, range_sq, rsum, me, other, mid);
}

template <int MAXL>
__device__ __forceinline__ void fused_candidates(const Params& P, const Smem& s, int lane) {
    if (lane < P.nA * MAXL) {
        const int q = lane / MAXL, k = lane - q * MAXL;
        const float4 so = s.sol[q];
        const float4* lq = s.lines + q * kLineStride;
        s.cand2[q * kLineStride + k] = lp_line_candidate_pairs5(lq, k, lane, so.z, so.x, so.y);
    }
}

__device__ __forceinline__ void split_barrier() {
    asm volatile("s_waitcnt lgkmcnt(0)\n\ts_barrier" ::: "memory");
}

struct Lp3Item {
    int a, m, i, base;
    bool item;
    float4 li, lj;
    float radius;
};
template <int MAXL>
__device__ __forceinline__ Lp3Item lp3_item_of(const Smem& s, int lane, unsigned long long mask) {
    constexpr int kPairs = MAXL * (MAXL - 1) / 2;
    Lp3Item it;
    const int t = lane / kPairs;
    it.m = lane - t * kPairs;
    it.a = 0;
    unsigned long long rest = mask;
#pragma unroll
    for (int u = 0; u < kWave / kPairs; ++u) {
        const int bit = rest ? __ffsll((long long)rest) - 1 : 0;
        it.a = (u == t) ? bit : it.a;
        rest &= rest - 1ull;
    }
    it.item = lane < (int)__popcll(mask) * kPairs;
    it.i = lp3_program_of(it.m), it.base = it.i * (it.i - 1) / 2;
    const float4* la = s.lines + it.a * kLineStride;
    it.li = la[it.i], it.lj = la[it.m - it.base];
    it.radius = s.sol[it.a].z;
    return it;
}
template <int MAXL>
__device__ __forceinline__ void lp3_head(const Smem& s, const Lp3Item& it) {
    const float4 pr = lp3_project(it.li, it.lj);
    if (it.item) s.proj[it.a * kLineStride + it.m] = pr;
    CN_FUSED_SYNC();
    if (it.item) {
        const float4* pa = s.proj + it.a * kLineStride + it.base;
        s.cand3[it.a * kLineStride + it.m] =
            lp_line_candidate<MAXL - 2>(pa[it.m - it.base], pa, it.m - it.base, it.radius, -it.li.w, it.li.z, true);
    }
}

template <int MAXL>
__device__ __forceinline__ bool split_has_head(unsigned int pred, int u, int n_steps) {
    return pred != 0u && __popc(pred) * (MAXL * (MAXL - 1) / 2) <= kWave && u < n_steps;
}

struct NoOp {
    __device__ __forceinline__ void operator()() const {}
};
template <int MAXL, int BASE_PRIO = 0, typename AfterScan = NoOp>
__device__ __forceinline__ unsigned long long fused_solve(const Params& P, const Smem& s, int lane, bool solve, float& rx,
                                                          float& ry, PhaseClock* clk, unsigned long long have = 0ull,
                                                          AfterScan&& after_scan = NoOp{}) {
    (void)P, (void)clk;
    rx = 0.0f, ry = 0.0f;
    int n = 0, fail = 0;
    if (solve) {
        n = s.count[lane];
        const float4 start = s.res[lane];
        rx = start.x, ry = start.y;
        fail = lp_planar_scan<MAXL>(s.lines + lane * kLineStride, s.cand2 + lane * kLineStride, n, rx, ry);
    }
    CN_TICK(clk, 3);
    const bool need = solve && fail < n;
    const unsigned long long nm = __ballot(need);
#ifdef CN_PHASE_TIMING
    if (clk) clk->acc[9] += __popcll(nm);
#endif
    after_scan();
    if (nm == 0ull) __builtin_amdgcn_s_setprio(BASE_PRIO);
    if (nm != 0ull) {
        __builtin_amdgcn_s_setprio(3);
        constexpr int kPairs = MAXL * (MAXL - 1) / 2;
        const int n_todo = __popcll(nm);
        bool one_pass_done = false;
        if (n_todo * kPairs <= kWave) {
            const Lp3Item it = lp3_item_of<MAXL>(s, lane, nm);
            const bool item = it.item;
            const int a = it.a, i = it.i, m = it.m, base = it.base;
            const float4 li = it.li;
            const float radius = it.radius;
            const bool hit = (nm & ~have) == 0ull;
            if (!hit) {
                lp3_head<MAXL>(s, it);
                CN_FUSED_SYNC();
            }
            if (item && m == base)
                s.cand2[a * kLineStride + i] = lp3_inner_program(s.proj + a * kLineStride, s.cand3 + a * kLineStride, i, li, radius);
            CN_FUSED_SYNC();
            if (need)
                lp3_outer_scan(s.lines + lane * kLineStride, s.cand2 + lane * kLineStride, n, fail, s.sol[lane].z, rx, ry);
            one_pass_done = true;
        } else {
            if (need) s.todo[__popcll(nm & ((1ull << lane) - 1ull))] = lane;
            CN_FUSED_SYNC();
            const int items = n_todo * kPairs;
            for (int p = lane; p < items; p += kWave) {
                const int t = p / kPairs, m = p - t * kPairs;
                const int a = s.todo[t];
                const int i = lp3_program_of(m), j = m - i * (i - 1) / 2;
                const float4* la = s.lines + a * kLineStride;
                s.proj[a * kLineStride + m] = lp3_project(la[i], la[j]);
            }
            CN_FUSED_SYNC();
            for (int p = lane; p < items; p += kWave) {
                const int t = p / kPairs, m = p - t * kPairs;
                const int a = s.todo[t];
                const int i = lp3_program_of(m), base = i * (i - 1) / 2;
                const float4 li = s.lines[a * kLineStride + i];
                const float4* pa = s.proj + a * kLineStride + base;
                s.cand3[a * kLineStride + m] = lp_line_candidate<MAXL - 2>(pa[m - base], pa, m - base, s.sol[a].z, -li.w, li.z, true);
            }
            CN_FUSED_SYNC();
        }
        if (need && !one_pass_done)
            lp3_scan(s.lines + lane * kLineStride, s.proj + lane * kLineStride, s.cand3 + lane * kLineStride, n,
                     fail, s.sol[lane].z, rx, ry);
    }
    return nm;
}

struct StepConsts {
    double dt, limit, limit1, success, collision, ddist, dfactor, hsafety;
};
__device__ __forceinline__ StepConsts step_consts(const Params& P) {
    StepConsts K;
    K.dt = in_vgpr(P.dt), K.limit = in_vgpr(P.time_limit), K.limit1 = in_vgpr(P.time_limit - 1.0);
    K.success = in_vgpr(P.success_reward), K.collision = in_vgpr(P.collision_penalty);
    K.ddist = in_vgpr(P.discomfort_dist), K.dfactor = in_vgpr(P.discomfort_factor);
    K.hsafety = in_vgpr(P.human_safety);
    return K;
}

__device__ __forceinline__ double swept_distance(const AgentRegs& r, bool human, double2 rp, double act_x, double act_y,
                                                 double new_vx, double new_vy, double dt, double robot_rad) {
    const double x1 = r.px - rp.x, y1 = r.py - rp.y;
    const double wx = r.vx - act_x, wy = r.vy - act_y;
    const double2 cp = closest_point(x1, y1, wx, wy, dt);
    const double endx = r.px + new_vx * dt, endy = r.py + new_vy * dt;
    const double d = norm2(human ? cp.x : endx - r.gx, human ? cp.y : endy - r.gy);
    return human ? d - r.rad - robot_rad : d;
}

struct StepOutcome {
    double reward, dmin;
    int info;
    bool done;
};
__device__ __forceinline__ StepOutcome reduce_env(const Params& P, const Smem& s, int ebase, double gtime, const StepConsts& K) {
    const double goal_dist = s.closest[ebase];
    const double robot_rad = s.rad[ebase];
    double dmin = std::numeric_limits<double>::infinity();
    bool collision = false;
    for (int i = 1; i < P.A; ++i) {
        const double c = s.closest[ebase + i];
        const bool hit = c < 0.0;
        dmin = (!collision & !hit & (c < dmin)) ? c : dmin;
        collision = collision | hit;
    }
    const bool timeout = gtime >= K.limit1;
    const bool reaching = goal_dist < robot_rad;
    const bool danger = dmin < K.ddist;
    double reward = danger ? (dmin - K.ddist) * K.dfactor * K.dt : 0.0;
    int info = danger ? CN_DANGER : CN_NOTHING;
    reward = reaching ? K.success : reward, info = reaching ? CN_REACH_GOAL : info;
    reward = collision ? K.collision : reward, info = collision ? CN_COLLISION : info;
    reward = timeout ? 0.0 : reward, info = timeout ? CN_TIMEOUT : info;
    const bool done = timeout | collision | reaching;
    return StepOutcome{reward, dmin, info, done};
}


#ifdef CN_WAVE_TRACE
static __device__ unsigned long long cn_wave_trace[8192 * 6];
#endif

constexpr int kSplitOrcaPrio = 1;
constexpr int kAssistHead = 1;
#ifndef CN_SPLIT_HEAD_PRIO
#define CN_SPLIT_HEAD_PRIO 2
#endif
#ifndef CN_SPLIT_HEAD_TAIL_PRIO
#define CN_SPLIT_HEAD_TAIL_PRIO 1
#endif

#ifdef CN_SPLIT_PROBE
constexpr bool kSplitProbe = true;
static __device__ unsigned long long cn_split_probe[32];
#define SPLIT_PROBE_DECL()                                                                                   \
    unsigned long long sp_cnt[7] = {}, sp_wait[3] = {}, sp_w1[2] = {}, sp_n1[2] = {}, sp_dt = 0ull; \
    bool sp_prev_head = false
#define SPLIT_PROBE_WAIT(k, barrier)                                   \
    do {                                                               \
        const unsigned long long sp_t0 = __builtin_readcyclecounter(); \
        barrier;                                                       \
        sp_dt = __builtin_readcyclecounter() - sp_t0;                  \
        sp_wait[k] += sp_dt;                                           \
    } while (0)
#define SPLIT_PROBE_AFTER_1(word, head)                               \
    do {                                                               \
        if ((word) != 0u) sp_w1[0] += sp_dt, ++sp_n1[0];               \
        if (sp_prev_head) sp_w1[1] += sp_dt, ++sp_n1[1];               \
        sp_prev_head = (head);                                         \
    } while (0)
#define SPLIT_PROBE_STEP(ended, nm, head, pred)                                  \
    do {                                                                         \
        const bool sp_hit = (head) && (nm) != 0ull && ((nm) & ~(unsigned long long)(pred)) == 0ull; \
        ++sp_cnt[0], sp_cnt[1] += (ended) ? 1 : 0, sp_cnt[2] += (nm) != 0ull ? 1 : 0, sp_cnt[3] += (head) ? 1 : 0; \
        sp_cnt[4] += sp_hit ? 1 : 0, sp_cnt[5] += ((nm) != 0ull && !sp_hit) ? 1 : 0, sp_cnt[6] += ((head) && (nm) == 0ull) ? 1 : 0; \
    } while (0)
#define SPLIT_PROBE_FLUSH(lane, base)                                                        \
    do {                                                                                     \
        if ((lane) == 0) {                                                                   \
            if ((base) == 0)                                                                 \
                for (int k = 0; k < 7; ++k) atomicAdd(&cn_split_probe[k], sp_cnt[k]);        \
            for (int k = 0; k < 3; ++k) atomicAdd(&cn_split_probe[((base) ? 10 : 7) + k], sp_wait[k]); \
            for (int k = 0; k < 2; ++k) {                                                    \
                atomicAdd(&cn_split_probe[((base) ? 17 : 13) + k], sp_w1[k]);                \
                atomicAdd(&cn_split_probe[((base) ? 19 : 15) + k], sp_n1[k]);                \
            }                                                                                \
        }                                                                                    \
    } while (0)
#else
constexpr bool kSplitProbe = false;
#define SPLIT_PROBE_DECL() (void)0
#define SPLIT_PROBE_WAIT(k, barrier) barrier
#define SPLIT_PROBE_AFTER_1(word, head) (void)0
#define SPLIT_PROBE_STEP(ended, nm, head, pred) (void)0
#define SPLIT_PROBE_FLUSH(lane, base) (void)0
#endif

template <int MAXL, int ASSIST>
__device__ __forceinline__ void split_orca_wave(const Params& P, const Smem& s, int n_steps) {
    const int lane = (int)threadIdx.x - kWave;
    float2* const vel = reinterpret_cast<float2*>(s.act);
    const float range_sq = P.orca.neighbor_dist * P.orca.neighbor_dist;
    const double c_dt = in_vgpr(P.dt);
    split_barrier();
    __builtin_amdgcn_s_setprio(kSplitOrcaPrio);
    const PairRow pr = pair_row_of(P, s, lane);
    double px = 0.0, py = 0.0;
    float rx = 0.0f, ry = 0.0f;
    bool solved = false;
    float rsum = 0.0f;
    const int pq = pr.my_info & 0xff;
    SPLIT_PROBE_DECL();
    for (int u = 0;;) {
        SPLIT_PROBE_WAIT(0, split_barrier());
        const int2 words = make_int2(s.flag[0], ((ASSIST & kAssistHead) || kSplitProbe) ? s.flag[1] : 0);
        float4 me = s.kin[pq], other = s.kin[pr.my_slot];
        const bool ended = __builtin_amdgcn_readfirstlane(words.x) != 0;
        const unsigned int pred = ((ASSIST & kAssistHead) || kSplitProbe) ? (unsigned int)__builtin_amdgcn_readfirstlane(words.y) : 0u;
        if (!ended) ++u;
        if (u >= n_steps) {
            split_barrier();
            break;
        }
        const bool head = (ASSIST & kAssistHead) ? split_has_head<MAXL>(pred, u, n_steps) : false;
        SPLIT_PROBE_AFTER_1(pred, head);
        if (ended) {
            if (lane < P.nA) {
                const double2 p = s.posd[lane];
                px = p.x, py = p.y;
                s.kin[lane] = reinterpret_cast<const float4*>(s.d2)[lane];
            }
            CN_FUSED_SYNC();
            me = s.kin[pq], other = s.kin[pr.my_slot];
        }
        if (ended) rsum = pair_rsum(s, pr);
        if (lane < P.pairs) fused_pair_body(P, s, pr, range_sq, rsum, me, other, [] {});
        SPLIT_PROBE_WAIT(1, split_barrier());
        fused_candidates<MAXL>(P, s, lane);
        CN_FUSED_SYNC();
        if (ended) solved = lane < P.nA && s.sol[lane < P.nA ? lane : 0].w != 0.0f;
        const unsigned long long nm = fused_solve<MAXL, kSplitOrcaPrio>(P, s, lane, solved, rx, ry, nullptr, head ? pred : 0u, [&] {
            if (head) SPLIT_PROBE_WAIT(2, split_barrier());
        });
        if (lane < P.nA) vel[lane] = make_float2(rx, ry);
        if (((ASSIST & kAssistHead) || kSplitProbe) && lane == 0) s.flag[1] = (int)nm;
        if (solved) {
            px = px + (double)rx * c_dt;
            py = py + (double)ry * c_dt;
            s.kin[lane] = make_float4((float)px, (float)py, rx, ry);
        }
        SPLIT_PROBE_STEP(ended, nm, head, pred);
    }
    SPLIT_PROBE_FLUSH(lane, 0);
}

template <bool HEADLINE, bool SPLIT = false, int ASSIST = 0>
__global__ __launch_bounds__((SPLIT ? 2 : 1) * kWave, (SPLIT ? 4 : HEADLINE ? 3 : 1)) void rollout_fused_kernel(
    Params P_in, const StateView* Sd, const int* ring_filled_in, RolloutView R, int n_steps, const double* ext_action) {
    static_assert(HEADLINE || !SPLIT, "the two-wave kernel exists for the headline geometry only");
    static_assert(SPLIT || ASSIST == 0, "the env wave assists an ORCA wave: two-wave kernel only");
#ifdef CN_WAVE_TRACE
    const unsigned long long wt_entry = __builtin_amdgcn_s_memrealtime();
    unsigned long long wt_fallbacks = 0ull, wt_ends = 0ull;
#endif
    constexpr int MAXL = 5;
    Params P = P_in;
    P.async_fill = 0;
    if (HEADLINE) {
        P.A = 6, P.NC = 5, P.E = 2, P.nA = 12, P.pairs = 60, P.threads = 64;
    }
    const Smem s = carve<MAXL>(P);
    if constexpr (SPLIT) {
        if (__builtin_amdgcn_readfirstlane((int)threadIdx.x) >= kWave) {
            split_orca_wave<MAXL, ASSIST>(P, s, n_steps);
            return;
        }
    }
    const Lane L = lane_of(P);
    AgentRegs r = {};
    float robot_max_speed = 0.0f;
    const bool robot = L.valid && L.a == 0;
    const cn_rollout_io* iop = R.io;
    double theta = 0.0;
    EpisodeBook ep = {};
    {
        const StateView S = *Sd;
        const cn_rollout_io io = *iop;
        const size_t gi = L.valid ? L.gi : 0;
        const int env = L.valid ? L.env : 0;
        const double2 p0 = S.pos[gi], v0 = S.vel[gi], g0 = S.goal[gi], q0 = S.rv[gi];
        const bool have = P.robot_orca ? S.rsim_valid[env] != 0 : false;
        const float rr_kept = P.robot_orca ? S.rsim_radius[gi] : 0.0f;
        const float ms_kept = P.robot_orca ? S.rsim_max_speed[env] : 0.0f;
        const double theta0 = S.theta[env];
        EpisodeBook ep0;
        CN_LOAD_EPISODE(P, ep0, S, io, ring_filled_in, env);
        if (L.valid) {
            r.px = p0.x, r.py = p0.y, r.vx = v0.x, r.vy = v0.y, r.gx = g0.x, r.gy = g0.y, r.rad = q0.x, r.vpref = q0.y;
            ep = ep0;
            if (L.a == 0) theta = theta0;
            if (P.robot_orca) {
                const float rr = have ? rr_kept : (float)(r.rad + 0.01 + P.robot_safety);
                if (!have) S.rsim_radius[L.gi] = rr;
                s.rview[L.lane] = rr;
                if (L.a == 0) {
                    robot_max_speed = have ? ms_kept : (float)r.vpref;
                    if (!have) S.rsim_max_speed[L.env] = robot_max_speed;
                }
            }
        }
    }
    build_pairs(P, s);

    if (L.valid && ep.state == kWaitingScenario && scenario_ready(P, *Sd, L.env, ep.ep_count, ep.ring_filled)) {
        load_from_ring(P, *Sd, L, ep.ep_count % P.ring_mod, r);
        ep.state = kRunning;
        ep.gtime = 0.0;
        theta = 1.5707963267948966;
    }
    unsigned int transitions = 0;
    for (int t = threadIdx.x; t < kMaxDiscount; t += P.threads) s.disc[t] = t < R.discount_len ? R.discount[t] : 0.0;
    CN_FUSED_SYNC();
    if (L.lane == 0) s.kin[P.nA] = make_float4(std::numeric_limits<float>::infinity(), std::numeric_limits<float>::infinity(), 0.0f, 0.0f);
    const PairRow pr = pair_row_of(P, s, L.lane);
    const StepConsts K = step_consts(P);
    float4* const kin_stage = SPLIT ? reinterpret_cast<float4*>(s.d2) : s.kin;
    stage_agent(P, s, L, r, K.hsafety, kin_stage);
    CN_FUSED_SYNC();

#ifdef CN_PHASE_TIMING
    PhaseClock clock = {};
    PhaseClock* clk = &clock;
    clock.last = __builtin_readcyclecounter();
#else
    PhaseClock* clk = nullptr;
    (void)clk;
#endif
    const float range_sq = P.orca.neighbor_dist * P.orca.neighbor_dist;
#ifdef CN_WAVE_TRACE
    const unsigned long long wt_loop = __builtin_amdgcn_s_memrealtime();
#endif
    if constexpr (SPLIT) {
        float2* const vel = reinterpret_cast<float2*>(s.act);
        if (L.lane == 0) s.flag[0] = 1, s.flag[1] = 0;
        split_barrier();
        bool skip = true;
        const bool mirror = L.lane >= 16 && L.lane < 16 + P.nA;
        const int m_lane = L.lane & 15;
        const int m_ebase = __shfl(L.ebase, m_lane);
        const bool m_robot = __shfl((int)(L.a == 0), m_lane) != 0;
        bool m_running = false;
        const auto copy_to_mirror = [&] {
            const double px = __shfl(r.px, m_lane), py = __shfl(r.py, m_lane), gx = __shfl(r.gx, m_lane), gy = __shfl(r.gy, m_lane);
            const int run = __shfl((int)(L.valid && ep.state == kRunning), m_lane);
            if (mirror) r.px = px, r.py = py, r.gx = gx, r.gy = gy, m_running = run != 0;
        };
        copy_to_mirror();
        SPLIT_PROBE_DECL();
        for (int u = 0;;) {
            SPLIT_PROBE_WAIT(0, split_barrier());
            if (!skip) ++u;
            const unsigned int pred = ((ASSIST & kAssistHead) || kSplitProbe) ? (unsigned int)__builtin_amdgcn_readfirstlane(s.flag[1]) : 0u;
            SPLIT_PROBE_AFTER_1(pred, (ASSIST & kAssistHead) != 0 && split_has_head<MAXL>(pred, u, n_steps));
            const bool running = L.valid && ep.state == kRunning;
            const AgentRegs r0 = r;
            double act_x = 0.0, act_y = 0.0, new_vx = 0.0, new_vy = 0.0;
            if (!skip && (L.lane < P.nA || mirror)) {
                const float2 mine = vel[m_lane], robots = vel[m_ebase];
                act_x = (double)robots.x, act_y = (double)robots.y;
                new_vx = m_robot ? act_x : (double)mine.x;
                new_vy = m_robot ? act_y : (double)mine.y;
                if (mirror ? m_running : running) {
                    r.px = r.px + new_vx * K.dt;
                    r.py = r.py + new_vy * K.dt;
                    r.vx = new_vx;
                    r.vy = new_vy;
                }
            }
            if (u < n_steps && (L.lane < P.nA || mirror)) {
                const double gdx = r.gx - r.px, gdy = r.gy - r.py;
                const double speed = norm2(gdx, gdy);
                const double num = mirror ? gdy : gdx;
                const float pref = (float)(speed > 1.0 ? num / speed : num);
                const float pref_y = __uint_as_float(__builtin_amdgcn_permlane16_swap(__float_as_uint(pref), __float_as_uint(pref), false, false)[1]);
                if (L.lane < P.nA) {
                    const float max_speed = (L.a == 0) ? robot_max_speed : (float)r.vpref;
                    float sx, sy;
                    lp_start_point(max_speed, pref, pref_y, sx, sy);
                    s.sol[L.lane] = make_float4(pref, pref_y, max_speed, (running && (L.a > 0 || P.robot_orca)) ? 1.0f : 0.0f);
                    s.res[L.lane] = make_float4(sx, sy, 0.0f, 0.0f);
                }
            }
            SPLIT_PROBE_WAIT(1, split_barrier());
            if constexpr ((ASSIST & kAssistHead) != 0) {
                if (split_has_head<MAXL>(pred, u, n_steps)) {
                    __builtin_amdgcn_s_setprio(CN_SPLIT_HEAD_PRIO);
                    const Lp3Item it = lp3_item_of<MAXL>(s, L.lane, (unsigned long long)pred);
                    lp3_head<MAXL>(s, it);
                    __builtin_amdgcn_s_setprio(CN_SPLIT_HEAD_TAIL_PRIO);
                    SPLIT_PROBE_WAIT(2, split_barrier());
                }
            }
            bool ended = false;
            if (!skip) {
                const double2 rp = make_double2(__shfl(r0.px, L.ebase), __shfl(r0.py, L.ebase));
                if (L.valid) s.closest[L.lane] = swept_distance(r0, L.a > 0, rp, act_x, act_y, new_vx, new_vy, K.dt, s.rad[L.ebase]);
                CN_FUSED_SYNC();
                bool done = false;
                if (running) {
                    const double disc_t = s.disc[ep.cur_steps < kMaxDiscount ? ep.cur_steps : kMaxDiscount - 1];
                    const StepOutcome o = reduce_env(P, s, L.ebase, ep.gtime, K);
                    done = o.done;
                    ep.gtime += K.dt;
                    ++transitions;
                    CN_BOOK_TRANSITION(ep, ep.cur_steps < kMaxDiscount ? disc_t : 0.0, o.reward, o.info, o.dmin);
                    if (done) {
                        const cn_rollout_io io = *iop;
                        const StateView S = *Sd;
                        AgentRegs next = r;
                        load_from_ring(P, S, L, (ep.ep_count + 1) % P.ring_mod, next);
                        CN_END_EPISODE(P, S, io, L.env, L.a == 0, K.limit, o.info, ep, r = next; theta = 1.5707963267948966);
                    }
                }
                ended = __ballot(done) != 0ull;
            }
            if (ended) stage_agent(P, s, L, r, K.hsafety, kin_stage);
            if (ended) copy_to_mirror();
            if (L.lane == 0) s.flag[0] = ended ? 1 : 0;
            skip = ended;
            if constexpr ((ASSIST & kAssistHead) != 0 && CN_SPLIT_HEAD_TAIL_PRIO != 0) __builtin_amdgcn_s_setprio(0);
            if (u >= n_steps) break;
        }
        SPLIT_PROBE_FLUSH(L.lane, 10);
    }
    const int one_wave_steps = SPLIT ? 0 : n_steps;
    for (int step = 0; step < one_wave_steps; ++step) {
        const bool running = L.valid && ep.state == kRunning;
        const bool solve = running && (L.a > 0 || P.robot_orca);

        if (L.lane < P.pairs) {
            float4 sol4, start4;
            fused_pair_phase(P, s, pr, range_sq, pair_rsum(s, pr), [&] {
                preferred_velocity(r, (L.a == 0) ? robot_max_speed : (float)r.vpref, solve, sol4, start4);
            });
            if (L.lane < P.nA) {
                s.sol[L.lane] = sol4;
                s.res[L.lane] = start4;
            }
        }
        CN_FUSED_SYNC();
        CN_TICK(clk, 2);

        fused_candidates<MAXL>(P, s, L.lane);
        CN_FUSED_SYNC();

        float rx, ry;
        const bool fell_back = fused_solve<MAXL>(P, s, L.lane, solve, rx, ry, clk) != 0ull;
        (void)fell_back;
#ifdef CN_WAVE_TRACE
        if (fell_back) ++wt_fallbacks;
#endif
        CN_TICK(clk, 8);

        double act_x, act_y;
        if (P.robot_orca) {
            act_x = (double)__shfl(rx, L.ebase);
            act_y = (double)__shfl(ry, L.ebase);
        } else {
            act_x = L.valid ? ext_action[2 * (size_t)L.env] : 0.0;
            act_y = L.valid ? ext_action[2 * (size_t)L.env + 1] : 0.0;
        }
        const double new_vx = (L.a == 0) ? act_x : (double)rx;
        const double new_vy = (L.a == 0) ? act_y : (double)ry;

        if (L.valid)
            s.closest[L.lane] = swept_distance(r, L.a > 0, s.posd[L.ebase], act_x, act_y, new_vx, new_vy, K.dt, s.rad[L.ebase]);
        CN_FUSED_SYNC();
        CN_TICK(clk, 5);

        if (running) {
            const double disc_t = s.disc[ep.cur_steps < kMaxDiscount ? ep.cur_steps : kMaxDiscount - 1];
            const StepOutcome o = reduce_env(P, s, L.ebase, ep.gtime, K);
            const double reward = o.reward, dmin = o.dmin;
            const int info = o.info;
            const bool done = o.done;
            ep.gtime += K.dt;
            r.px = r.px + new_vx * K.dt;
            r.py = r.py + new_vy * K.dt;
            r.vx = new_vx;
            r.vy = new_vy;
            ++transitions;
            CN_BOOK_TRANSITION(ep, ep.cur_steps < kMaxDiscount ? disc_t : 0.0, reward, info, dmin);
#ifdef CN_WAVE_TRACE
            if (__ballot(done) != 0ull) ++wt_ends;
#endif
            if (done) {
                const cn_rollout_io io = *iop;
                CN_END_EPISODE(P, *Sd, io, L.env, L.a == 0, K.limit, info, ep,
                               load_from_ring(P, *Sd, L, ep.ep_count % P.ring_mod, r); theta = 1.5707963267948966);
            }
        }
        stage_agent(P, s, L, r, K.hsafety, kin_stage);
        CN_FUSED_SYNC();
        CN_TICK(clk, 7);
    }
#ifdef CN_PHASE_TIMING
    if ((threadIdx.x & (kWave - 1)) == 0) {
        unsigned long long total = 0ull;
        for (int k = 0; k < 10; ++k) {
            atomicAdd(&cn_phase_cycles[k], clock.acc[k]);
            if (k != 9) total += clock.acc[k];
        }
        atomicMax(&cn_phase_cycles[14], total);
        atomicMin(&cn_phase_cycles[13], total);
        atomicAdd(&cn_phase_cycles[15], 1ull);
    }
#endif

#ifdef CN_WAVE_TRACE
    const unsigned long long wt_exit = __builtin_amdgcn_s_memrealtime();
#endif
    const StateView S = *Sd;
    if (L.valid) CN_STORE_AGENT(S, L.gi, r);
    const cn_rollout_io io = *iop;
    if (robot) CN_STORE_EPISODE(P, S, io, L.env, ep, theta);
    rollout_epilogue(P, S, io, L, robot, transitions, ep.ep_count, reinterpret_cast<double*>(s.lines));
#ifdef CN_WAVE_TRACE
    if (threadIdx.x == 0 && blockIdx.x < 8192) {
        unsigned long long* w = cn_wave_trace + 6 * blockIdx.x;
        unsigned hw;
        asm volatile("s_getreg_b32 %0, hwreg(HW_REG_HW_ID)" : "=s"(hw));
        w[0] = wt_entry, w[1] = wt_loop, w[2] = wt_exit, w[3] = __builtin_amdgcn_s_memrealtime();
        w[4] = wt_fallbacks | (wt_ends << 32), w[5] = hw;
    }
#endif
}

}
```

crowdnav_amd/csrc/scenario_ring.h:

```cpp
#pragma once
#include "step_kernels.h"

namespace cn {

__device__ __forceinline__ uint64_t generate_scenario_lane(const ScenarioCfg& C, uint32_t seed, size_t base,
                                                           double2* pos, double2* vel, double2* goal, double2* rv,
                                                           uint32_t* hbm_column, int hbm_stride, bool keep_state,
                                                           int* pos_out) {
    if (!keep_state) {
        Mt19937Head head;
        const uint64_t n = generate_scenario(C, head, seed, base, pos, vel, goal, rv);
        if (!head.dead()) return n;
    }
    Mt19937 rng{hbm_column, hbm_stride, 0};
    const uint64_t n = generate_scenario(C, rng, seed, base, pos, vel, goal, rv);
    if (keep_state && pos_out) *pos_out = rng.pos;
    return n;
}

__device__ __forceinline__ void clear_human_sims(const Params& P, const StateView& S, int b, int first, int stride) {
    if (P.kd)
        for (int a = first; a < P.A; a += stride) S.kd_valid[(size_t)b * P.A + a] = 0;
}

__global__ __launch_bounds__(kWave) void reset_kernel(Params P, ScenarioCfg C, StateView S, const uint32_t* seeds,
                                                     const uint8_t* mask, uint64_t* draws) {
    const int b = blockIdx.x * blockDim.x + threadIdx.x;
    if (b >= P.B) return;
    if (mask && !mask[b]) return;
    const uint64_t n = generate_scenario_lane(C, seeds[b], (size_t)b * P.A, S.pos, S.vel, S.goal, S.rv,
                                                      S.mt_key + b, P.B, true, &S.mt_pos[b]);
    S.gtime[b] = 0.0;
    S.theta[b] = 1.5707963267948966;
    if (draws) draws[b] = n;
    clear_human_sims(P, S, b, 1, 1);
}

__global__ void mt_probe_kernel(uint32_t* key, uint32_t seed, int n, double* out) {
    if (threadIdx.x != 0 || blockIdx.x != 0) return;
    Mt19937 rng{key, 1, 0};
    rng.seed(seed);
    for (int i = 0; i < n; ++i) out[i] = rng.random();
}

struct RolloutView {
    const cn_rollout_io* io;
    const double* discount;
    int discount_len;
};

enum { kRetired = 0, kRunning = 1, kWaitingScenario = 2 };

__device__ __forceinline__ int64_t episode_id(const cn_rollout_io& io, int b, int ordinal) {
    return io.env_offset + b + (int64_t)ordinal * io.env_stride;
}
__device__ __forceinline__ uint32_t episode_seed(const cn_rollout_io& io, int64_t c) {
    return io.seed_base + (uint32_t)((uint64_t)c % io.seed_mod);
}

__device__ __forceinline__ bool past_episode_limit(const cn_rollout_io& io, int64_t c) {
    return io.episode_limit >= 0 && c >= io.episode_limit;
}
__device__ __forceinline__ int ring_next_ordinal(int ep_count, int state) { return ep_count + (state == kWaitingScenario ? 0 : 1); }
__device__ __forceinline__ int ring_slot_ordinal(int next, int slot, int D) { return next + ((slot - next % D) + D) % D; }
__device__ __forceinline__ bool ring_claim_slot(const StateView& S, int idx, int ordinal) {
    const int want = ordinal + 1;
    const int have = S.ring_claim[idx];
    return have < want && atomicCAS(&S.ring_claim[idx], have, want) == have;
}
__device__ __forceinline__ void ring_publish_slot(const StateView& S, int idx, int ordinal) {
    __builtin_amdgcn_fence(__ATOMIC_RELEASE, "agent");
    __syncthreads();
    if (threadIdx.x == 0) __hip_atomic_store(&S.ring_ready[idx], ordinal + 1, __ATOMIC_RELEASE, __HIP_MEMORY_SCOPE_AGENT);
}

__device__ __forceinline__ void begin_env(const StateView& S, const cn_rollout_io& io, int b, bool on) {
    io.active[b] = on ? kRunning : kRetired;
    S.ep_word[b] = on ? kRunning : kRetired;
    io.ep_count[b] = 0;
    io.cur_steps[b] = 0;
    io.cur_return[b] = 0.0;
    if (io.cur_danger) io.cur_danger[b] = 0;
    if (io.cur_danger_dmin_sum) io.cur_danger_dmin_sum[b] = 0.0;
    S.ring_filled_in[b] = 0;
    S.ring_filled_out[b] = 0;
}

__global__ __launch_bounds__(kWave) void rollout_begin_kernel(Params P, ScenarioCfg C, StateView S, RolloutView R) {
    const int b = blockIdx.x * blockDim.x + threadIdx.x;
    if (b >= P.B) return;
    const cn_rollout_io io = *R.io;
    const int64_t c0 = episode_id(io, b, 0);
    const bool on = !past_episode_limit(io, c0);
    begin_env(S, io, b, on);
    clear_human_sims(P, S, b, 1, 1);
    if (!on) return;
    generate_scenario_lane(C, episode_seed(io, c0), (size_t)b * P.A, S.pos, S.vel, S.goal, S.rv, S.mt_key + b,
                                   P.B, false, nullptr);
    S.mt_pos[b] = -1;
    S.gtime[b] = 0.0;
}

constexpr int kRedoLanes = 4096;
__global__ __launch_bounds__(kWave) void ring_fill_begin_kernel(int B, const int* ep_word, int* ep_snap, int* redo_count) {
    const int b = blockIdx.x * blockDim.x + threadIdx.x;
    if (b == 0) *redo_count = 0;
    if (b < B) ep_snap[b] = __hip_atomic_load(&ep_word[b], __ATOMIC_RELAXED, __HIP_MEMORY_SCOPE_AGENT);
}
__global__ __launch_bounds__(kWave) void ring_fill_kernel(Params P, ScenarioCfg C, StateView S, RolloutView R, const int* ep_snap) {
    const int idx = blockIdx.x * blockDim.x + threadIdx.x;
    const int D = P.ring_mod;
    if (idx >= P.B * D) return;
    const bool by_slot = D == P.ring_depth;
    const int k = by_slot ? idx % D : idx / P.B, b = by_slot ? idx / D : idx - k * P.B;
    const cn_rollout_io* io = R.io;
    const int state = ep_snap ? ep_snap[b] & 3 : io->active[b];
    const int next = ring_next_ordinal(ep_snap ? ep_snap[b] >> 2 : io->ep_count[b], state);
    if (k == 0) S.ring_filled_out[b] = next + D;
    if (state == kRetired) return;
    const int level = S.ring_filled_in[b];
    const int ordinal = by_slot ? ring_slot_ordinal(next, k, D) : max(level, next) + k;
    if (ordinal < level || ordinal >= next + D) return;
    const int64_t c = episode_id(*io, b, ordinal);
    if (past_episode_limit(*io, c)) return;
    const uint32_t seed = episode_seed(*io, c);
    const int ring_idx = b * D + ordinal % D;
    Mt19937Head head;
    generate_scenario(C, head, seed, (size_t)ring_idx * P.A, S.ring_pos, nullptr, S.ring_goal, S.ring_rv);
    if (head.dead()) S.redo_list[atomicAdd(S.redo_count, 1)] = make_int2(ring_idx, (int)seed);
}

__global__ __launch_bounds__(kWave) void ring_redo_kernel(Params P, ScenarioCfg C, StateView S) {
    const int lane = blockIdx.x * blockDim.x + threadIdx.x;
    const int n = *S.redo_count;
    for (int k = lane; k < n; k += kRedoLanes) {
        const int2 job = S.redo_list[k];
        Mt19937 rng{S.ring_mt_key + lane, kRedoLanes, 0};
        generate_scenario(C, rng, (uint32_t)job.y, (size_t)job.x * P.A, S.ring_pos, nullptr, S.ring_goal, S.ring_rv);
    }
}

__global__ __launch_bounds__(kWave) void reset_wave_kernel(Params P, ScenarioCfg C, StateView S, const uint32_t* seeds,
                                                          const uint8_t* mask, uint64_t* draws) {
    __shared__ WaveScratch scratch;
    const int b = blockIdx.x;
    if (mask && !mask[b]) return;
    const uint64_t n = generate_scenario_wave(C, scratch, seeds[b], (size_t)b * P.A, S.pos, S.vel, S.goal, S.rv, S.mt_key + b,
                                              P.B, &S.mt_pos[b]);
    if (threadIdx.x == 0) {
        S.gtime[b] = 0.0;
        S.theta[b] = 1.5707963267948966;
        if (draws) draws[b] = n;
    }
    clear_human_sims(P, S, b, 1 + threadIdx.x, blockDim.x);
}

__global__ __launch_bounds__(kWave) void rollout_begin_wave_kernel(Params P, ScenarioCfg C, StateView S, RolloutView R) {
    __shared__ WaveScratchFill scratch;
    const int b = blockIdx.x;
    const cn_rollout_io io = *R.io;
    const int64_t c0 = episode_id(io, b, 0);
    const bool on = !past_episode_limit(io, c0);
    if (threadIdx.x == 0) {
        begin_env(S, io, b, on);
        S.gtime[b] = 0.0;
        S.mt_pos[b] = -1;
    }
    clear_human_sims(P, S, b, 1 + threadIdx.x, blockDim.x);
    if (P.async_fill)
        for (int t = threadIdx.x; t < P.ring_depth; t += blockDim.x) {
            S.ring_ready[(size_t)b * P.ring_depth + t] = 0;
            S.ring_claim[(size_t)b * P.ring_depth + t] = 0;
        }
    if (!on) return;
    generate_scenario_wave(C, scratch, episode_seed(io, c0), (size_t)b * P.A, S.pos, S.vel, S.goal, S.rv);
}

constexpr int kScenarioCacheMax = 4096;
template <class Scratch>
__device__ __forceinline__ void cached_scenario_wave(const Params& P, const ScenarioCfg& C, const StateView& S, Scratch& scratch,
                                                     const cn_rollout_io& io, int64_t c, size_t base) {
    const int lane = threadIdx.x;
    const bool use = S.cache_n > 0;
    const int k = use ? (int)((uint64_t)c % io.seed_mod) : 0;
    if (use && __hip_atomic_load(&S.cache_state[k], __ATOMIC_ACQUIRE, __HIP_MEMORY_SCOPE_AGENT) == 1) {
        if (lane < P.A) {
            const size_t ci = (size_t)k * P.A + lane;
            S.ring_pos[base + lane] = S.cache_pos[ci];
            S.ring_goal[base + lane] = S.cache_goal[ci];
            S.ring_rv[base + lane] = S.cache_rv[ci];
        }
        return;
    }
    generate_scenario_wave(C, scratch, episode_seed(io, c), base, S.ring_pos, nullptr, S.ring_goal, S.ring_rv);
    if (!use) return;
    __syncthreads();
    if (lane < P.A) {
        const size_t ci = (size_t)k * P.A + lane;
        S.cache_pos[ci] = S.ring_pos[base + lane];
        S.cache_goal[ci] = S.ring_goal[base + lane];
        S.cache_rv[ci] = S.ring_rv[base + lane];
    }
    __builtin_amdgcn_fence(__ATOMIC_RELEASE, "agent");
    __syncthreads();
    if (lane == 0) __hip_atomic_store(&S.cache_state[k], 1, __ATOMIC_RELEASE, __HIP_MEMORY_SCOPE_AGENT);
}

__global__ __launch_bounds__(kWave) void ring_fill_wave_kernel(Params P, ScenarioCfg C, StateView S, RolloutView R) {
    __shared__ WaveScratchFill scratch;
    const int idx = blockIdx.x;
    const int D = P.ring_depth;
    const int b = idx / D, slot = idx - b * D;
    const cn_rollout_io io = *R.io;
    const int state = io.active[b];
    const int next = ring_next_ordinal(io.ep_count[b], state);
    if (slot == 0 && threadIdx.x == 0) S.ring_filled_out[b] = next + D;
    if (state == kRetired) return;
    const int ordinal = ring_slot_ordinal(next, slot, D);
    if (ordinal < S.ring_filled_in[b]) return;
    const int64_t c = episode_id(io, b, ordinal);
    if (past_episode_limit(io, c)) return;
    cached_scenario_wave(P, C, S, scratch, io, c, ((size_t)b * D + slot) * P.A);
}

__global__ __launch_bounds__(256) void ring_fill_scan_kernel(Params P, StateView S, RolloutView R, int* list) {
    const int D = P.ring_depth;
    const int total = P.B * D;
    const cn_rollout_io* io = R.io;
    const int item = blockIdx.x * blockDim.x + threadIdx.x;
    const int u = item / P.B, b = item - u * P.B;
    int ordinal = 0;
    bool claimed = false;
    if (item < total) {
        const int word = __hip_atomic_load(&S.ep_word[b], __ATOMIC_RELAXED, __HIP_MEMORY_SCOPE_AGENT);
        const int state = word & 3;
        if (state != kRetired) {
            ordinal = ring_next_ordinal(word >> 2, state) + u;
            if (!past_episode_limit(*io, episode_id(*io, b, ordinal))) claimed = ring_claim_slot(S, b * D + ordinal % D, ordinal);
        }
    }
    const unsigned long long m = __ballot(claimed);
    if (m == 0ull) return;
    const int lane = threadIdx.x & (kWave - 1);
    int base = 0;
    if (lane == __ffsll((long long)m) - 1) base = atomicAdd(&list[0], __popcll(m));
    base = __shfl(base, __ffsll((long long)m) - 1);
    if (claimed) {
        const int k = base + __popcll(m & ((1ull << lane) - 1ull));
        list[2 + 2 * k] = b;
        list[3 + 2 * k] = ordinal;
    }
}

constexpr int kFillJobBatch = 4;
__global__ __launch_bounds__(kWave) void ring_fill_jobs_kernel(Params P, ScenarioCfg C, StateView S, RolloutView R, int* list) {
    __shared__ WaveScratchFill scratch;
    const int lane = threadIdx.x;
    const int D = P.ring_depth;
    const cn_rollout_io* io = R.io;
    const int jobs = list[0];
    int first = 0;
    do {
        if (lane == 0) first = atomicAdd(&list[1], kFillJobBatch);
        first = __shfl(first, 0);
        int jb = 0, jord = 0;
        const bool have = lane < kFillJobBatch && first + lane < jobs;
        if (have) jb = list[2 + 2 * (first + lane)], jord = list[3 + 2 * (first + lane)];
        unsigned long long todo = __ballot(have);
        while (todo) {
            const int src = __ffsll((long long)todo) - 1;
            todo &= todo - 1ull;
            const int b = __shfl(jb, src), ord = __shfl(jord, src);
            const int idx = b * D + ord % D;
            cached_scenario_wave(P, C, S, scratch, *io, episode_id(*io, b, ord), (size_t)idx * P.A);
            ring_publish_slot(S, idx, ord);
        }
    } while (first + kFillJobBatch < jobs);
}

__device__ __forceinline__ bool scenario_ready(const Params& P, const StateView& S, int env, int ordinal, int ring_filled) {
    if (!P.async_fill) return ordinal < ring_filled;
    const int* flag = S.ring_ready + (size_t)env * P.ring_depth + ordinal % P.ring_depth;
    return __hip_atomic_load(flag, __ATOMIC_ACQUIRE, __HIP_MEMORY_SCOPE_AGENT) == ordinal + 1;
}

__device__ __forceinline__ void load_from_ring(const Params& P, const StateView& S, const Lane& L, int slot,
                                               AgentRegs& r) {
    const size_t ri = ((size_t)L.env * P.ring_mod + slot) * P.A + L.a;
    const double2 p = S.ring_pos[ri], g = S.ring_goal[ri], q = S.ring_rv[ri];
    r.px = p.x, r.py = p.y, r.vx = 0.0, r.vy = 0.0, r.gx = g.x, r.gy = g.y, r.rad = q.x, r.vpref = q.y;
}

}
```

crowdnav_amd/csrc/scenario_ring_host.h:

```cpp
#pragma once
#include "engine_host.h"
#include "scenario_ring.h"

static inline void swap_levels(cn::StateView& S) { std::swap(S.ring_filled_in, S.ring_filled_out); }

inline void ScenarioRing::configure(cn_engine* e, int compute_units) {
    const cn_config* c = &e->cfg;
    cn::Params& P = e->P;
    gen_wave = env_int("CROWDNAV_AMD_WAVE_SCENARIOS", c->num_humans > 8 ? 1 : 0) != 0;
    if ((c->flags & CN_FLAG_ASYNC_SCENARIO_FILL) != 0 && gen_wave) mode = Fill::WorkList;
    else if (!gen_wave && env_int("CROWDNAV_AMD_LAGGED_FILL", 1) != 0 && grid_envs(e) <= 8 * compute_units) mode = Fill::Beside;
    else mode = Fill::InFront;
    P.async_fill = mode == Fill::WorkList ? 1 : 0;
    P.ring_depth = env_int("CROWDNAV_AMD_RING_DEPTH", 48);
    if (P.ring_depth < 1) P.ring_depth = 1;
    if (mode == Fill::WorkList && !getenv("CROWDNAV_AMD_RING_DEPTH")) P.ring_depth = 144;
    plan.configure(P.ring_depth, mode == Fill::Beside);
    P.ring_mod = plan.C;
    scenario_cache = env_int("CROWDNAV_AMD_SCENARIO_CACHE", 1) != 0;
    fill_queue_wgs = env_int("CROWDNAV_AMD_FILL_QUEUE_WGS", 1024);
    if (fill_queue_wgs < 1) fill_queue_wgs = 1;
}

inline int ScenarioRing::create(cn_engine* e) {
    const cn::Params& P = e->P;
    const size_t n = (size_t)P.B * P.A, slots = (size_t)P.B * P.ring_depth, cache = (size_t)cn::kScenarioCacheMax * P.A;
    const bool work_list = mode == Fill::WorkList;
    int rc = CN_OK;
    cn::StateView& S = e->S;
    if ((rc = dev_alloc(e, &S.ring_pos, n * P.ring_mod)) || (rc = dev_alloc(e, &S.ring_goal, n * P.ring_mod)) ||
        (rc = dev_alloc(e, &S.ring_rv, n * P.ring_mod)) ||
        (rc = dev_alloc(e, &S.ring_mt_key, gen_wave ? (size_t)64 : (size_t)624 * cn::kRedoLanes)) ||
        (rc = dev_alloc(e, &S.redo_list, gen_wave ? (size_t)1 : (size_t)P.B * P.ring_mod)) ||
        (rc = dev_alloc(e, &ep_snap, mode == Fill::Beside ? (size_t)P.B : (size_t)1)) ||
        (rc = dev_alloc(e, &S.redo_count, (size_t)1)) ||
        (rc = dev_alloc(e, &S.ring_filled_in, (size_t)P.B)) || (rc = dev_alloc(e, &S.ring_filled_out, (size_t)P.B)) ||
        (rc = dev_alloc(e, &S.ring_ready, work_list ? slots : (size_t)1)) ||
        (rc = dev_alloc(e, &S.ring_claim, work_list ? slots : (size_t)1)) ||
        (rc = dev_alloc(e, &fill_list, work_list ? (size_t)kFillStreams * (2 + 2 * slots) : (size_t)2)) ||
        (rc = dev_alloc(e, &S.cache_pos, gen_wave ? cache : (size_t)1)) ||
        (rc = dev_alloc(e, &S.cache_goal, gen_wave ? cache : (size_t)1)) ||
        (rc = dev_alloc(e, &S.cache_rv, gen_wave ? cache : (size_t)1)) ||
        (rc = dev_alloc(e, &S.cache_state, (size_t)cn::kScenarioCacheMax)))
        return rc;
    if (work_list) {
        bool ok = hipEventCreateWithFlags(&rollout_done, hipEventDisableTiming) == hipSuccess;
        for (int i = 0; ok && i < kFillStreams; ++i)
            ok = hipStreamCreateWithFlags(&fill_streams[i], hipStreamNonBlocking) == hipSuccess;
        if (!ok) return fail(CN_ERR_HIP, "cn_create: side streams for the asynchronous scenario fill");
    }
    if (mode == Fill::Beside) {
        int least = 0, greatest = 0;
        if (hipEventCreateWithFlags(&rollout_done, hipEventDisableTiming) != hipSuccess ||
            hipEventCreateWithFlags(&fill_done, hipEventDisableTiming) != hipSuccess ||
            hipDeviceGetStreamPriorityRange(&least, &greatest) != hipSuccess ||
            hipStreamCreateWithPriority(&fill_streams[0], hipStreamNonBlocking, least) != hipSuccess)
            return fail(CN_ERR_HIP, "cn_create: side stream for the lagged scenario fill");
    }
    return CN_OK;
}

static inline hipError_t sync_fill_streams(const ScenarioRing& ring) {
    hipError_t first = hipSuccess;
    for (hipStream_t fs : ring.fill_streams)
        if (fs) {
            const hipError_t err = hipStreamSynchronize(fs);
            if (first == hipSuccess) first = err;
        }
    return first;
}

inline void ScenarioRing::destroy() {
    (void)sync_fill_streams(*this);
    for (hipStream_t fs : fill_streams)
        if (fs) (void)hipStreamDestroy(fs);
    if (rollout_done) (void)hipEventDestroy(rollout_done);
    if (fill_done) (void)hipEventDestroy(fill_done);
}

inline int ScenarioRing::drain(cn_engine* e) {
    CN_HIP(sync_fill_streams(*this));
    if (plan.settle()) swap_levels(e->S);
    return CN_OK;
}

inline int ScenarioRing::settle(cn_engine* e) { return plan.pending ? drain(e) : CN_OK; }

inline int ScenarioRing::begin(cn_engine* e, uint32_t seed_mod) {
    const cn::RolloutView R{e->io_dev, e->discount, e->discount_len};
    e->S.cache_n = (gen_wave && scenario_cache && seed_mod <= (uint32_t)cn::kScenarioCacheMax) ? (int)seed_mod : 0;
    if (gen_wave) {
        CN_HIP(hipMemsetAsync(e->S.cache_state, 0, sizeof(int) * cn::kScenarioCacheMax, e->stream));
        hipLaunchKernelGGL(cn::rollout_begin_wave_kernel, dim3(e->P.B), dim3(cn::kWave), 0, e->stream, e->P, e->C, e->S, R);
    } else {
        hipLaunchKernelGGL(cn::rollout_begin_kernel, dim3(grid_lanes(e)), dim3(cn::kWave), 0, e->stream, e->P, e->C, e->S, R);
    }
    CN_HIP(hipGetLastError());
    plan.begin();
    return CN_OK;
}

template <class Launch>
int ScenarioRing::around_launch(cn_engine* e, int n_steps, Launch&& launch) {
    const cn::RolloutView R{e->io_dev, e->discount, e->discount_len};
    cn::FillPlan::Decision plan_says{false, false, false};
    if (mode == Fill::WorkList) {
        const int this_stream = next_fill_stream;
        hipStream_t fs = fill_streams[this_stream];
        next_fill_stream = (next_fill_stream + 1) % kFillStreams;
        CN_HIP(hipEventRecord(rollout_done, e->stream));
        CN_HIP(hipStreamWaitEvent(fs, rollout_done, 0));
        int* list = fill_list + (size_t)this_stream * (2 + 2 * (size_t)e->P.B * e->P.ring_depth);
        CN_HIP(hipMemsetAsync(list, 0, 2 * sizeof(int), fs));
        const int items = e->P.B * e->P.ring_depth;
        hipLaunchKernelGGL(cn::ring_fill_scan_kernel, dim3((items + 255) / 256), dim3(256), 0, fs, e->P, e->S, R, list);
        hipLaunchKernelGGL(cn::ring_fill_jobs_kernel, dim3(fill_queue_wgs), dim3(cn::kWave), 0, fs, e->P, e->C, e->S, R, list);
        e->launch_counts[CN_COUNT_ASYNC_FILLS] += 1;
    } else {
        plan_says = plan.call(n_steps);
    }
    const int fill_lanes = e->P.B * e->P.ring_mod;
    const dim3 fill_grid((fill_lanes + cn::kWave - 1) / cn::kWave), redo_grid(cn::kRedoLanes / cn::kWave);
    if (plan_says.take_levels) {
        CN_HIP(hipStreamWaitEvent(e->stream, fill_done, 0));
        swap_levels(e->S);
    }
    if (plan_says.sync_fill) {
        if (gen_wave) {
            hipLaunchKernelGGL(cn::ring_fill_wave_kernel, dim3(fill_lanes), dim3(cn::kWave), 0, e->stream, e->P, e->C, e->S, R);
        } else {
            CN_HIP(hipMemsetAsync(e->S.redo_count, 0, sizeof(int), e->stream));
            hipLaunchKernelGGL(cn::ring_fill_kernel, fill_grid, dim3(cn::kWave), 0, e->stream, e->P, e->C, e->S, R, nullptr);
            hipLaunchKernelGGL(cn::ring_redo_kernel, redo_grid, dim3(cn::kWave), 0, e->stream, e->P, e->C, e->S);
        }
        swap_levels(e->S);
        e->launch_counts[CN_COUNT_RING_FILLS] += 1;
    }
    if (plan_says.lagged_fill) CN_HIP(hipEventRecord(rollout_done, e->stream));
    launch(R, (const int*)e->S.ring_filled_in);
    CN_HIP(hipGetLastError());
    if (plan_says.lagged_fill) {
        hipStream_t fs = fill_streams[0];
        CN_HIP(hipStreamWaitEvent(fs, rollout_done, 0));
        hipLaunchKernelGGL(cn::ring_fill_begin_kernel, dim3(grid_lanes(e)), dim3(cn::kWave), 0, fs, e->P.B, e->S.ep_word, ep_snap,
                           e->S.redo_count);
        hipLaunchKernelGGL(cn::ring_fill_kernel, fill_grid, dim3(cn::kWave), 0, fs, e->P, e->C, e->S, R, (const int*)ep_snap);
        hipLaunchKernelGGL(cn::ring_redo_kernel, redo_grid, dim3(cn::kWave), 0, fs, e->P, e->C, e->S);
        CN_HIP(hipEventRecord(fill_done, fs));
        e->launch_counts[CN_COUNT_RING_FILLS] += 1;
        lagged_fills += 1;
    }
    return CN_OK;
}
```

crowdnav_amd/csrc/step_kernels.h:

```cpp
#pragma once
#include <hip/hip_runtime.h>
#include <limits>

#include "../../include/crowdnav_amd.h"
#include "orca_device.h"
#include "kd_order.h"
#include "scenario_device.h"
#include "scenario_wave.h"
#include "transition.h"

namespace cn {


constexpr int kMaxBlock = 512;

struct Params {
    int B, A;
    int E;
    int threads;
    int nA;
    int NC;
    int pairs;
    int ring_depth;
    int robot_visible, robot_orca;
    int robot_unicycle;
    int async_fill;
    int sched;
    int dyn_visits;
    int kd;
    KdLayout kdl;
    double dt, time_limit, success_reward, collision_penalty, discomfort_dist, discomfort_factor;
    double robot_safety, human_safety;
    OrcaParams orca;
    int ring_mod;
};

struct StateView {
    double2* pos;
    double2* vel;
    double2* goal;
    double2* rv;
    double* gtime;
    double* theta;
    float* rsim_radius;
    float* rsim_max_speed;
    uint8_t* rsim_valid;
    uint32_t* mt_key;
    uint32_t* ring_mt_key;
    int2* redo_list;
    int* redo_count;
    int* mt_pos;
    double2* ring_pos;
    double2* ring_goal;
    double2* ring_rv;
    int* ring_filled_in;
    int* ring_filled_out;
    int* ring_ready;
    int* ring_claim;
    uint8_t* kd_order;
    uint8_t* kd_valid;
    double2* cache_pos;
    double2* cache_goal;
    double2* cache_rv;
    int* cache_state;
    int cache_n;
    int* error;
    int* dyn_queue;
    int* ep_word;
    double* wg_partial;
    double* group_partial;
    unsigned* tickets;
};

constexpr int kEpilogueGroups = 32;
constexpr int kTicketStride = 64;

struct StepIo {
    const double* action;
    double* reward;
    uint8_t* done;
    uint8_t* info;
    double* dmin;
    double* action_out;
    float* orca_vel;
    double* obs;
    int update;
};

struct Smem {
    float4* kin;
    double2* posd;
    double2* act;
    float4* lines;
    float4* proj;
    float4* cand2;
    float4* cand3;
    double* rad;
    double* closest;
    float* hview;
    float* rview;
    float* d2;
    int* pinfo;
    int* count;
    int* flag;
    float4* sol;
    float4* res;
    int* todo;
    double* disc;
    uint32_t kd_off;
    double2* goal2;
    double* vpref;
};

constexpr int kCompactScratchDoubles = 16;
constexpr int kMaxDiscount = 256;
__host__ __device__ inline size_t proj_bytes(int nA, int ) { return (size_t)16 * kLineStride * nA; }

__host__ __device__ inline size_t smem_bytes(int nA, int pairs, int maxl, int A = 0, int E = 1) {
    return (size_t)nA * (16 + 16 + 16 + (maxl == 5 ? 3 : 1) * 16 * kLineStride + 16 + 16 + 8 + 8 + 4 + 4 + 4 + 4 + 4) + proj_bytes(nA, maxl) +
           (size_t)pairs * 8 + 64 + 8 + 16 + 16 + sizeof(double) * kMaxDiscount + (A > kKdLeaf ? 16 + kd_lds_bytes(nA, A, E) : 0);
}

constexpr int kLazyRows = (kWave / (kMaxNb - 1)) * (kMaxNb - 1);
__host__ __device__ inline size_t smem_bytes_compact(int nA, int pairs, int A, int E) {
    size_t n = (size_t)16 * (nA + 1) + 16 * nA + 16 * E + (size_t)16 * kLineStride * nA + 16 * kLazyRows;
    n += (size_t)nA * (16 + 16 + 16 + 8 + 8 + 8 + 4 + 4 + 4 + 4) + 4 * (nA + 1) + 16;
    n += (size_t)pairs * 4 + (size_t)pairs * 2 + 16 + 16 + 8 * kCompactScratchDoubles + (A > kKdLeaf ? 16 + kd_lds_bytes(nA, A, E) : 0);
    if (A > kKdLeaf) n -= (size_t)nA * kd_row_bytes(A) + (size_t)nA * (kd_max_nodes(A) + 1) * 2;
    return n;
}

template <int MAXL, bool COMPACT = false>
__device__ __forceinline__ Smem carve(const Params& P) {
    extern __shared__ double2 smem_raw[];
    Smem s;
    char* p = reinterpret_cast<char*>(smem_raw);
    const int nA = P.nA;
    s.kin = reinterpret_cast<float4*>(p), p += 16 * (nA + 1);
    s.posd = reinterpret_cast<double2*>(p), p += 16 * nA;
    s.act = reinterpret_cast<double2*>(p), p += 16 * (COMPACT ? P.E : nA);
    s.lines = reinterpret_cast<float4*>(p), p += 16 * kLineStride * nA;
    s.proj = reinterpret_cast<float4*>(p), p += COMPACT ? (size_t)16 * kLazyRows : proj_bytes(nA, MAXL);
    s.cand2 = s.cand3 = nullptr;
    if (MAXL == 5) {
        s.cand2 = reinterpret_cast<float4*>(p), p += 16 * kLineStride * nA;
        s.cand3 = reinterpret_cast<float4*>(p), p += 16 * kLineStride * nA;
    }
    s.sol = reinterpret_cast<float4*>(p), p += 16 * nA;
    s.res = reinterpret_cast<float4*>(p), p += 16 * nA;
    s.goal2 = nullptr, s.vpref = nullptr;
    if (COMPACT) {
        s.goal2 = reinterpret_cast<double2*>(p), p += 16 * nA;
        s.vpref = reinterpret_cast<double*>(p), p += 8 * nA;
    }
    s.rad = reinterpret_cast<double*>(p), p += 8 * nA;
    s.closest = reinterpret_cast<double*>(p), p += 8 * nA;
    s.hview = reinterpret_cast<float*>(p), p += 4 * nA;
    s.rview = reinterpret_cast<float*>(p), p += 4 * nA;
    s.count = reinterpret_cast<int*>(p), p += 4 * nA;
    s.flag = reinterpret_cast<int*>(p), p += 4 * nA;
    s.todo = reinterpret_cast<int*>(p), p += 4 * (nA + 1);
    p += (16 - (reinterpret_cast<size_t>(p) & 15)) & 15;
    s.d2 = reinterpret_cast<float*>(p), p += 4 * P.pairs;
    s.pinfo = reinterpret_cast<int*>(p), p += (COMPACT ? 2 : 4) * P.pairs;
    s.disc = reinterpret_cast<double*>(p + ((8 - (reinterpret_cast<size_t>(p) & 7)) & 7));
    {
        char* q = reinterpret_cast<char*>(s.disc + (COMPACT ? kCompactScratchDoubles : kMaxDiscount));
        q += (16 - (reinterpret_cast<size_t>(q) & 15)) & 15;
        s.kd_off = (uint32_t)(q - reinterpret_cast<char*>(smem_raw));
    }
    return s;
}

enum { kParDt = 0, kParLimit, kParSuccess, kParCollision, kParDDist, kParDFactor, kParHSafety, kParCount };
template <bool COMPACT>
__device__ __forceinline__ double step_param(const Params& P, const Smem& s, int which) {
    if (COMPACT) return s.disc[which];
    return which == kParDt ? P.dt : which == kParLimit ? P.time_limit : which == kParSuccess ? P.success_reward :
           which == kParCollision ? P.collision_penalty : which == kParDDist ? P.discomfort_dist :
           which == kParDFactor ? P.discomfort_factor : P.human_safety;
}

__device__ __forceinline__ void block_sync(const Params& P) {
    if (P.threads == kWave) wave_lds_sync();
    else __syncthreads();
}
__device__ __forceinline__ int block_sync_or(const Params& P, int v) {
    if (P.threads == kWave) return __ballot(v != 0) != 0ull ? 1 : 0;
    return __syncthreads_or(v);
}

struct Lane {
    int lane, env, a, ebase;
    bool valid;
    size_t gi;
};

__device__ __forceinline__ Lane lane_of(const Params& P, int block = -1, int tid = -1) {
    Lane L;
    L.lane = tid < 0 ? (int)threadIdx.x : tid;
    const int el = L.lane / P.A;
    L.a = L.lane - el * P.A;
    L.env = (block < 0 ? (int)blockIdx.x : block) * P.E + el;
    L.valid = (L.lane < P.nA) && (L.env < P.B);
    L.ebase = el * P.A;
    L.gi = (size_t)L.env * P.A + L.a;
    return L;
}

struct AgentRegs {
    double px, py, vx, vy, gx, gy, rad, vpref;
};

__device__ __forceinline__ void load_agent(const StateView& S, size_t gi, AgentRegs& r) {
    const double2 p = S.pos[gi], v = S.vel[gi], g = S.goal[gi], q = S.rv[gi];
    r.px = p.x, r.py = p.y, r.vx = v.x, r.vy = v.y, r.gx = g.x, r.gy = g.y, r.rad = q.x, r.vpref = q.y;
}

template <bool COMPACT>
__device__ __forceinline__ int pair_info(const Params& P, const Smem& s, int p) {
    if (!COMPACT) return s.pinfo[p];
    const int w = reinterpret_cast<const uint16_t*>(s.pinfo)[p];
    const int q = w & 31;
    return q | (((w >> 5) & 31) << 8) | ((p - q * P.NC) << 16) | (((w >> 10) & 3) << 24);
}

template <bool COMPACT = false>
__device__ __forceinline__ void build_pairs(const Params& P, const Smem& s, bool every_env_exists = false) {
    for (int p = threadIdx.x; p < P.pairs; p += P.threads) {
        const int q = p / P.NC;
        const int c = p - q * P.NC;
        const int el = q / P.A;
        const int a = q - el * P.A;
        int j;
        bool exists = every_env_exists || ((int)blockIdx.x * P.E + el) < P.B;
        if (a == 0) {
            j = c + 1;
        } else {
            j = c + 1 + (c + 1 >= a ? 1 : 0);
            if (j >= P.A) {
                j = 0;
                exists = exists && P.robot_visible;
            }
        }
        if (COMPACT)
            reinterpret_cast<uint16_t*>(s.pinfo)[p] = (uint16_t)(q | ((el * P.A + j) << 5) | (exists ? 1 << 10 : 0) | (a == 0 ? 1 << 11 : 0));
        else
            s.pinfo[p] = q | ((el * P.A + j) << 8) | (c << 16) | (exists ? 1 << 24 : 0) | (a == 0 ? 1 << 25 : 0);
    }
}

__device__ __forceinline__ void load_robot_view(const Params& P, const StateView& S, const Smem& s,
                                                const Lane& L, const AgentRegs& r, float& robot_max_speed, bool preloaded = false,
                                                bool pre_have = false, float pre_radius = 0.0f, float pre_max_speed = 0.0f) {
    robot_max_speed = 0.0f;
    if (!L.valid) return;
    const bool have = preloaded ? pre_have : S.rsim_valid[L.env] != 0;
    float rr;
    if (have) {
        rr = preloaded ? pre_radius : S.rsim_radius[L.gi];
    } else {
        rr = (float)(r.rad + 0.01 + P.robot_safety);
        S.rsim_radius[L.gi] = rr;
    }
    s.rview[L.lane] = rr;
    if (L.a == 0) {
        if (have) {
            robot_max_speed = preloaded ? pre_max_speed : S.rsim_max_speed[L.env];
        } else {
            robot_max_speed = (float)r.vpref;
            S.rsim_max_speed[L.env] = robot_max_speed;
        }
    }
}

__device__ __forceinline__ KdSmem kd_view(const Params& P, const Smem& s) {
    extern __shared__ double2 smem_raw[];
    return kd_carve(reinterpret_cast<char*>(smem_raw) + s.kd_off, P.kdl);
}

template <bool COMPACT>
__device__ __forceinline__ KdSmem kd_scratch_view(const Params& P, const Smem& s) {
    KdSmem k = kd_view(P, s);
    if (COMPACT) {
        k.visit = reinterpret_cast<uint8_t*>(s.lines);
        k.stack = reinterpret_cast<uint16_t*>(reinterpret_cast<char*>(s.lines) + (size_t)P.nA * k.row);
    }
    return k;
}

__device__ __forceinline__ void kd_load(const Params& P, const StateView& S, const Smem& s, const Lane& L) {
    if (!P.kd) return;
    const KdSmem k = kd_view(P, s);
    if (L.lane < P.nA) {
        uint8_t* row = k.ord + (size_t)L.lane * k.row;
        if (L.valid && S.kd_valid[L.gi] != 0) {
            const uint32_t* src = reinterpret_cast<const uint32_t*>(S.kd_order + L.gi * k.row);
            for (int w = 0; w < k.row / 4; ++w) reinterpret_cast<uint32_t*>(row)[w] = src[w];
        } else {
            kd_identity_row(row, k.row, P.A, L.a, P.robot_visible);
        }
    }
    if (threadIdx.x == 0) *k.gen = 0;
    for (int i = threadIdx.x; i < P.E * 2 * 2; i += P.threads) k.count[i] = 0;
}

__device__ __forceinline__ void kd_store(const Params& P, const StateView& S, const Smem& s, const Lane& L) {
    if (!P.kd || !L.valid) return;
    const KdSmem k = kd_view(P, s);
    const uint32_t* row = reinterpret_cast<const uint32_t*>(k.ord + (size_t)L.lane * k.row);
    uint32_t* dst = reinterpret_cast<uint32_t*>(S.kd_order + L.gi * k.row);
    for (int w = 0; w < k.row / 4; ++w) dst[w] = row[w];
    S.kd_valid[L.gi] = 1;
}

__device__ __forceinline__ void kd_new_episode(const Params& P, const Smem& s, const Lane& L) {
    if (!P.kd) return;
    const KdSmem k = kd_view(P, s);
    if (L.a > 0) kd_identity_row(k.ord + (size_t)L.lane * k.row, k.row, P.A, L.a, P.robot_visible);
    if (L.a == 0) {
        const int last = *k.gen, el = L.ebase / P.A;
        k.count[(last * P.E + el) * 2 + 0] = 0;
        k.count[(last * P.E + el) * 2 + 1] = 0;
    }
}

__device__ __forceinline__ void kd_build_trees(const Params& P, const Smem& s, const Lane& L, int g) {
    const KdSmem k = kd_view(P, s);
    const int tid = threadIdx.x;
    const bool agent = L.lane < P.nA;
    const int el = agent ? L.ebase / P.A : 0;
    const float4 me = agent ? s.kin[L.lane] : make_float4(0.0f, 0.0f, 0.0f, 0.0f);
    const uint32_t kx = kd_key(me.x), ky = kd_key(me.y);
    const uint64_t amask = P.A >= 64 ? ~0ull : ((1ull << P.A) - 1ull);
    for (int t = 0; t < 2; ++t) {
        KdNode* list = k.nodes + ((size_t)(g * P.E + el) * 2 + t) * k.mn;
        int* cnt = k.count + (g * P.E + el) * 2 + t;
        if (!kd_tree_on(P.A, t, P.robot_visible)) {
            if (agent && L.a == 0) *cnt = 0;
            continue;
        }
        for (int i = tid; i < P.E * k.mn; i += P.threads) {
            k.bb[4 * i + 0] = 0xffffffffu, k.bb[4 * i + 1] = 0u, k.bb[4 * i + 2] = 0xffffffffu, k.bb[4 * i + 3] = 0u;
        }
        const KdNode* old = k.nodes + ((size_t)((g ^ 1) * P.E + el) * 2 + t) * k.mn;
        const int n_old = agent ? k.count[((g ^ 1) * P.E + el) * 2 + t] : 0;
        int first_dirty = 1 << 20;
        if (agent && L.a == 0) {
            list[0].meta = (uint32_t)kd_tree_size(P.A, t) << 8;
            list[0].set = t == 0 ? amask : (amask & ~1ull);
            *cnt = 1;
        }
        block_sync(P);
        for (int r = 0;; ++r) {
            const int c = agent ? *cnt : 0;
            const bool live = agent && r < c;
            if (!block_sync_or(P, live ? 1 : 0)) break;
            KdNode nd = KdNode{0u, 0u, 0ull, 0ull, 0ull};
            bool member = false;
            uint32_t* acc = k.bb + ((size_t)el * k.mn + r) * 4;
            if (live) {
                nd = list[r];
                member = (t == 0 || L.a > 0) && ((nd.set >> L.a) & 1ull) != 0ull;
                if (member) {
                    atomicMin(acc + 0, kx), atomicMax(acc + 1, kx);
                    atomicMin(acc + 2, ky), atomicMax(acc + 3, ky);
                }
            }
            block_sync(P);
            bool lower = false;
            if (live) {
                const float min_x = kd_unkey(acc[0]), max_x = kd_unkey(acc[1]), min_y = kd_unkey(acc[2]), max_y = kd_unkey(acc[3]);
                const bool vertical = (max_x - min_x) > (max_y - min_y);
                const float split = vertical ? 0.5f * (max_x + min_x) : 0.5f * (max_y + min_y);
// ... 655 lines not shown
```

crowdnav_amd/engine.py:

```python
import ctypes as C
import weakref

import numpy as np
import torch

from . import _lib
from ._lib import CnConfig, CnLookaheadOut, CnRolloutIo, CnTraceOut, check

_DEFAULTS = dict(
    num_envs=1, num_humans=5, time_step=0.25, time_limit=25.0, success_reward=1.0,
    collision_penalty=-0.25, discomfort_dist=0.2, discomfort_penalty_factor=0.5, robot_visible=0,
    robot_policy=_lib.ROBOT_ORCA, robot_safety_space=0.0, human_safety_space=0.0, neighbor_dist=10.0,
    max_neighbors=10, scenario_rule=_lib.CIRCLE_CROSSING, time_horizon=5.0, time_horizon_obst=5.0,
    circle_radius=4.0, square_width=10.0, human_radius=0.3, human_v_pref=1.0, robot_radius=0.3,
    robot_v_pref=1.0, randomize_attributes=0, device=0, robot_kinematics=_lib.HOLONOMIC, flags=0)


def default_config(**overrides):
    d = dict(_DEFAULTS)
    unknown = set(overrides) - set(d)
    if unknown:
        raise TypeError('unknown config keys: %s' % sorted(unknown))
    d.update(overrides)
    return d
# ... 317 lines not shown
        if n > 0:
            a, temporary = self._borrow(actions, torch.float64, (self.B, K, n, 2))
            v, temporary_v = self._borrow(human_vel, torch.float64, (self.B, n, self.H, 2))
            lo = C.byref(_struct(CnLookaheadOut, out))
            head = (self._h, n, K, _ptr(a)) + (() if v is None else (_ptr(v),)) + (lo,)
            if bootstrap:
                call = self._lib.cn_lookahead_values if v is None else self._lib.cn_lookahead_paths_values
                check(call(*head, int(bool(sort_humans)), _ptr(out['value']), _ptr(out['score'])))
            else:
                check((self._lib.cn_lookahead_actions if v is None else self._lib.cn_lookahead_paths)(*head))
            self._release(temporary, temporary_v)
        return out

    def set_lookahead_human_model(self, model):
        if model not in _lib.HUMAN_MODELS:
            raise ValueError('lookahead human model: one of %s, got %r' % (_lib.HUMAN_MODELS, model))
        check(self._lib.cn_lookahead_set_human_model(self._h, _lib.HUMAN_MODELS.index(model)))

    @property
    def lookahead_human_model(self):
        model = C.c_int()
        check(self._lib.cn_lookahead_get_human_model(self._h, C.byref(model)))
        return _lib.HUMAN_MODELS[model.value]

    def plan_begin(self, K, n, elites, iterations, init_std, min_std=0.0, smoothing=0.0, seed=0, bootstrap=False,
                   sort_humans=False):
        K, n = int(K), int(n)
        if K < 1 or n < 1:
            raise ValueError('plan_begin: K and n must be >= 1')
        return Plan(self, K, n, int(elites), int(iterations), float(init_std), float(min_std), float(smoothing), int(seed),
                    bool(bootstrap), bool(sort_humans))

    def _plan_call(self, name, plan, *args, rollout=False, n_real=None, counter=None):
        io, bufs = self._roll() if rollout else (None, None)
        if not isinstance(plan, Plan) or plan.engine() is not self:
            raise ValueError('plan: a Plan made by this engine\'s plan_begin()')
        head = [] if not rollout else [C.byref(io)] if n_real is None else [C.byref(io), int(n_real)]
        tail = [] if counter is None else [int(counter) & 0xffffffff]
        check(getattr(self._lib, 'cn_plan_' + name)(self._h, *head, C.byref(plan.cfg), C.byref(plan.c), *args, *tail))
        return bufs

    def plan_reset(self, plan, mask=None):
        m, temporary = self._borrow(mask, torch.uint8, (self.B,))
        self._plan_call('reset', plan, _ptr(m))
        self._release(temporary)
        return plan

    def plan_draw(self, plan, counter):
        self._plan_call('draw', plan, counter=counter)
        return plan.candidates

    def plan_refit(self, plan, keep_best=False):
        self._plan_call('refit', plan, int(bool(keep_best)))
        return plan

    def plan_cem(self, plan, counter):
        self._plan_call('cem', plan, counter=counter)
        return plan

    def plan_shift(self, plan):
        self._plan_call('shift', plan, rollout=True)
        return plan

    def plan_rollout(self, plan, n_real, counter):
        return self._plan_call('rollout', plan, rollout=True, n_real=n_real, counter=counter)

    def plan_mppi_update(self, plan, temperature, fit_std=False, keep_best=False):
        self._plan_call('mppi_update', plan, float(temperature), int(bool(fit_std)), int(bool(keep_best)))
        return plan

    def plan_mppi(self, plan, temperature, counter, fit_std=False):
        self._plan_call('mppi', plan, float(temperature), int(bool(fit_std)), counter=counter)
        return plan

    def _plan_paths(self, name, plan, human_vel, *args, counter):
        if not isinstance(plan, Plan) or plan.engine() is not self:
            raise ValueError('plan: a Plan made by this engine\'s plan_begin()')
        v, temporary = self._borrow(human_vel, torch.float64, (self.B, plan.n, self.H, 2))
        if v is None:
            raise ValueError('plan_%s: human_vel is required ([%d, %d, %d, 2])' % (name, self.B, plan.n, self.H))
        self._plan_call(name, plan, _ptr(v), *args, counter=counter)
        self._release(temporary)
        return plan

    def plan_cem_paths(self, plan, human_vel, counter):
        return self._plan_paths('cem_paths', plan, human_vel, counter=counter)

    def plan_mppi_paths(self, plan, human_vel, temperature, counter, fit_std=False):
        return self._plan_paths('mppi_paths', plan, human_vel, float(temperature), int(bool(fit_std)), counter=counter)

    def _path_modes(self, who, n, human_vel, weights, reduce, risk_penalty):
        vshape = tuple(getattr(human_vel, 'shape', np.shape(human_vel)))
        if len(vshape) != 5 or vshape[:1] + vshape[2:] != (self.B, n, self.H, 2) or not 1 <= vshape[1] <= _lib.MODES_MAX:
            raise ValueError('%s: human_vel must be [%d, M in 1..%d, n = %d, %d, 2], got %s'
                             % (who, self.B, _lib.MODES_MAX, n, self.H, vshape))
        M = int(vshape[1])
        if reduce not in _lib.MODES_REDUCE:
            raise ValueError('%s: reduce must be one of %s, got %r' % (who, _lib.MODES_REDUCE, reduce))
        if weights is not None:
            wshape = tuple(getattr(weights, 'shape', np.shape(weights)))
            if wshape != (self.B, M):
                raise ValueError('%s: weights must be [%d, M = %d], got %s' % (who, self.B, M, wshape))
        v, temporary_v = self._borrow(human_vel, torch.float64, (self.B, M, n, self.H, 2))
        w, temporary_w = self._borrow(weights, torch.float64, (self.B, M))
        modes = _lib.CnPathModes(n_modes=M, reduce=_lib.MODES_REDUCE.index(reduce), risk_penalty=float(risk_penalty),
                                 human_vel=v.data_ptr(), weight=None if w is None else w.data_ptr())
        return modes, M, (v, w), (temporary_v, temporary_w)

    def lookahead_modes(self, actions, human_vel, weights=None, reduce='mean', risk_penalty=0.0, per_mode=False, out=None):
        who = 'lookahead_modes'
        shape = tuple(getattr(actions, 'shape', np.shape(actions)))
        if len(shape) != 4 or shape[0] != self.B or shape[1] < 1 or shape[3] != 2:
            raise ValueError('%s: actions must be [%d, K >= 1, n, 2], got %s' % (who, self.B, shape))
        K, n = int(shape[1]), int(shape[2])
        modes, M, keep, temporary = self._path_modes(who, n, human_vel, weights, reduce, risk_penalty)
        spec = dict(score=(torch.float64, (self.B, K)), risk=(torch.float64, (self.B, K)), worst_mode=(torch.int32, (self.B, K)),
                    worst_info=(torch.uint8, (self.B, K)), worst_steps=(torch.int32, (self.B, K)),
                    worst_time=(torch.float64, (self.B, K)))
        if per_mode:
            spec.update(ret=(torch.float64, (self.B, K, M)), info=(torch.uint8, (self.B, K, M)),
                        steps=(torch.int32, (self.B, K, M)), time=(torch.float64, (self.B, K, M)))
        out = self._rows(who, spec, out)
        if n > 0:
            a, temporary_a = self._borrow(actions, torch.float64, (self.B, K, n, 2))
            check(self._lib.cn_lookahead_modes(self._h, n, K, _ptr(a), C.byref(modes), C.byref(_struct(_lib.CnModesOut, out))))
            self._release(temporary_a, *temporary)
        del keep
        return out

    def _plan_modes(self, name, plan, human_vel, weights, reduce, risk_penalty, *args, counter):
        if not isinstance(plan, Plan) or plan.engine() is not self:
            raise ValueError('plan: a Plan made by this engine\'s plan_begin()')
        modes, _, keep, temporary = self._path_modes('plan_' + name, plan.n, human_vel, weights, reduce, risk_penalty)
        self._plan_call(name, plan, C.byref(modes), *args, counter=counter)
        self._release(*temporary)
        del keep
        return plan

    def plan_cem_modes(self, plan, human_vel, counter, weights=None, reduce='mean', risk_penalty=0.0):
        return self._plan_modes('cem_modes', plan, human_vel, weights, reduce, risk_penalty, counter=counter)

    def plan_mppi_modes(self, plan, human_vel, temperature, counter, weights=None, reduce='mean', risk_penalty=0.0, fit_std=False):
        return self._plan_modes('mppi_modes', plan, human_vel, weights, reduce, risk_penalty, float(temperature),
                                int(bool(fit_std)), counter=counter)

    def plan_mppi_rollout(self, plan, n_real, temperature, counter, fit_std=False):
        return self._plan_call('mppi_rollout', plan, float(temperature), int(bool(fit_std)), rollout=True, n_real=n_real,
                               counter=counter)

    def predict(self, n, models='to_goal', out=None):
        codes, single = _predict_models('predict', models)
        n = int(n)
        if n < 0:
            raise ValueError('predict: n must be >= 0')
        shape = (self.B, n, self.H, 2) if single else (self.B, len(codes), n, self.H, 2)
        if out is None:
            out = self._new(shape, torch.float64)
        elif not self._dense(out, torch.float64, shape):
            raise ValueError('predict: out must be a contiguous %s %s tensor on %s' % (torch.float64, shape, self.device))
        if n > 0:
            check(self._lib.cn_predict(self._h, n, len(codes), (C.c_int32 * len(codes))(*codes), _ptr(out)))
        return out

    def plan_predict_begin(self, plan, models, weights=None, reduce='mean', risk_penalty=0.0):
        if not isinstance(plan, Plan) or plan.engine() is not self:
            raise ValueError('plan: a Plan made by this engine\'s plan_begin()')
        codes, _ = _predict_models('plan_predict_begin', models)
        if reduce not in _lib.MODES_REDUCE:
            raise ValueError('plan_predict_begin: reduce must be one of %s, got %r' % (_lib.MODES_REDUCE, reduce))
        if weights is not None:
            wshape = tuple(getattr(weights, 'shape', np.shape(weights)))
            if wshape != (self.B, len(codes)):
                raise ValueError('plan_predict_begin: weights must be [%d, M = %d], got %s' % (self.B, len(codes), wshape))
        return Predictors(self, plan, codes, weights, reduce, risk_penalty)

    def plan_predict_rollout(self, plan, pred, n_real, counter, temperature=None, fit_std=False):
        if not isinstance(plan, Plan) or plan.engine() is not self:
            raise ValueError('plan: a Plan made by this engine\'s plan_begin()')
        if not isinstance(pred, Predictors) or pred.engine() is not self or pred.plan() is not plan:
            raise ValueError('pred: the Predictors made by this engine\'s plan_predict_begin() for this plan')
        if temperature is None:
            return self._plan_call('cem_predict_rollout', plan, C.byref(pred.c), rollout=True, n_real=n_real, counter=counter)
        return self._plan_call('mppi_predict_rollout', plan, C.byref(pred.c), float(temperature), int(bool(fit_std)), rollout=True,
                               n_real=n_real, counter=counter)

    def predict_orca(self, n, out=None, mode=None):
        return self._predict_orca('predict_orca', n, out, mode, None)

    def _predict_orca(self, who, n, out, mode, robot_actions):
        n = int(n)
        if n < 0:
            raise ValueError('%s: n must be >= 0' % who)
        rows = None if robot_actions is None else self._action_rows(who, robot_actions, n)
        if mode is None:
            M, m, shape = 1, 0, (self.B, n, self.H, 2)
            if out is None:
                out = self._new(shape, torch.float64)
        else:
            if out is None:
                raise ValueError('%s: mode needs out, the [%d, M, %d, %d, 2] table whose slot is filled' % (who, self.B, n, self.H))
            oshape = tuple(getattr(out, 'shape', ()))
            M = int(oshape[1]) if len(oshape) == 5 else 0
            if not 1 <= M <= _lib.MODES_MAX:
                raise ValueError('%s: out must be [%d, M in 1..%d, n = %d, %d, 2], got %s'
                                 % (who, self.B, _lib.MODES_MAX, n, self.H, oshape))
            if isinstance(mode, bool) or not isinstance(mode, (int, np.integer)) or not 0 <= mode < M:
                raise ValueError('%s: mode must be an int in 0 .. M - 1 = %d, got %r' % (who, M - 1, mode))
            m, shape = int(mode), (self.B, M, n, self.H, 2)
        if not self._dense(out, torch.float64, shape):
            raise ValueError('%s: out must be a contiguous %s %s tensor on %s' % (who, torch.float64, shape, self.device))
        if n > 0 and rows is None:
            check(self._lib.cn_predict_orca(self._h, n, M, m, _ptr(out)))
        elif n > 0:
            a, stride, temporary = rows
            check(self._lib.cn_predict_orca_robot(self._h, n, M, m, _ptr(a), stride, _ptr(out)))
            self._release(temporary)
        return out

    def _action_rows(self, who, robot_actions, n):
        shape = tuple(getattr(robot_actions, 'shape', np.shape(robot_actions)))
        if shape != (self.B, n, 2):
            raise ValueError('%s: robot_actions must be [%d, n = %d, 2], got %s' % (who, self.B, n, shape))
        t = robot_actions
        if not (torch.is_tensor(t) and t.device == self.device and t.dtype == torch.float64):
            t, temporary = self._borrow(t, torch.float64, shape)
            return t, n, temporary
        if n == 0:
            return t, 0, False
        between, row, last = t.stride()
        if last != 1 or (n > 1 and row != 2):
            raise ValueError('%s: robot_actions: the last two dimensions must be contiguous (strides %s)' % (who, (between, row, last)))
        if self.B == 1:
            return t, n, False
        if between % 2 or between < 2 * n:
            raise ValueError('%s: robot_actions: %d elements between envs are not a whole number of rows >= n = %d'
                             % (who, between, n))
        return t, between // 2, False

    def predict_orca_robot(self, n, robot_actions, out=None, mode=None):
        if robot_actions is None:
            raise ValueError('predict_orca_robot: robot_actions is required ([%d, n, 2]); predict_orca(n) leaves the robot out' % self.B)
        return self._predict_orca('predict_orca_robot', n, out, mode, robot_actions)

    def plan_predict_orca_rollout(self, plan, pred, n_real, counter, orca_mode=0, temperature=None, fit_std=False):
        return self._orca_rollout('plan_predict_orca_rollout', 'predict_orca_rollout', plan, pred, n_real, counter, orca_mode,
                                  temperature, fit_std)

    def plan_predict_orca_nominal_rollout(self, plan, pred, n_real, counter, orca_mode=0, temperature=None, fit_std=False):
        return self._orca_rollout('plan_predict_orca_nominal_rollout', 'predict_orca_nominal_rollout', plan, pred, n_real, counter,
                                  orca_mode, temperature, fit_std)

    def _orca_rollout(self, who, name, plan, pred, n_real, counter, orca_mode, temperature, fit_std):
        if not isinstance(plan, Plan) or plan.engine() is not self:
            raise ValueError('plan: a Plan made by this engine\'s plan_begin()')
        if not isinstance(pred, Predictors) or pred.engine() is not self or pred.plan() is not plan:
            raise ValueError('pred: the Predictors made by this engine\'s plan_predict_begin() for this plan')
        if isinstance(orca_mode, bool) or not isinstance(orca_mode, (int, np.integer)) or not 0 <= orca_mode < pred.c.n_modes:
            raise ValueError('%s: orca_mode must be an int in 0 .. M - 1 = %d, got %r' % (who, pred.c.n_modes - 1, orca_mode))
        if temperature is None:
            return self._plan_call('cem_' + name, plan, C.byref(pred.c), int(orca_mode), rollout=True, n_real=n_real, counter=counter)
        return self._plan_call('mppi_' + name, plan, C.byref(pred.c), int(orca_mode), float(temperature), int(bool(fit_std)),
                               rollout=True, n_real=n_real, counter=counter)

    def rollout_records(self, max_records=None):
        io, bufs = self._roll()
        K = int(bufs['ep_outcome'].shape[1] if max_records is None else max_records)
        blocks = self._new((self.B, 1 + K * _lib.RECORD_FIELDS), torch.float64)
        check(self._lib.cn_rollout_records(self._h, C.byref(io), K, _ptr(blocks)))
        return blocks

    def records_summary(self, blocks, record_capacity=None, out=None):
        K = (int(blocks.shape[1]) - 1) // _lib.RECORD_FIELDS
        cap = K if record_capacity is None else int(record_capacity)
        out = self._summary_out(out)
        check(self._lib.cn_records_summary(self._h, int(blocks.shape[0]), K, cap, _ptr(blocks), _ptr(out)))
        return out

    def _summary_out(self, out):
        if out is None:
            return self._new((_lib.SUMMARY_FIELDS,), torch.float64)
        if not self._dense(out, torch.float64, out.shape) or out.numel() != _lib.SUMMARY_FIELDS:
            raise ValueError('summary output: a contiguous float64 [%d] tensor on %s' % (_lib.SUMMARY_FIELDS, self.device))
        return out

    def rollout_summary(self, out=None):
        io, _ = self._roll()
        out = self._summary_out(out)
        check(self._lib.cn_rollout_summary(self._h, C.byref(io), _ptr(out)))
        return out

    def gather_records_rccl(self, comm, n_ranks, blocks):
        K = (int(blocks.shape[1]) - 1) // _lib.RECORD_FIELDS
        out = self._new((n_ranks * self.B, int(blocks.shape[1])), torch.float64)
        check(self._lib.cn_gather_records(self._h, C.c_void_p(int(comm)), int(n_ranks), K, _ptr(blocks), _ptr(out)))
        return out

    def launch_counts(self):
        out = (C.c_uint64 * len(_lib.LAUNCH_COUNTERS))()
        check(self._lib.cn_launch_counts(self._h, out))
        lagged = C.c_uint64()
        check(self._lib.cn_lagged_fills(self._h, C.byref(lagged)))
        return dict(zip(_lib.LAUNCH_COUNTERS, (int(v) for v in out)), lagged_fills=int(lagged.value))

    def rollout_route(self, n_steps):
        route = C.c_int(-1)
        check(self._lib.cn_rollout_route(self._h, int(n_steps), C.byref(route)))
        return _lib.ROLLOUT_ROUTES[route.value]

    def sarl_network_route(self):
        route = C.c_int(-1)
        check(self._lib.cn_sarl_network_route(self._h, C.byref(route)))
        return _lib.SARL_ROUTES[route.value]

    def mt_random(self, seed, n):
        out = self._new((n,), torch.float64)
        check(self._lib.cn_mt_random(self._h, int(seed), int(n), _ptr(out)))
        return out

    def sarl_configure(self, actions, gamma=0.9, with_om=False, cell_num=4, cell_size=1.0, om_channel_size=3,
                       with_global_state=True, mlp1_dims=(150, 100), mlp2_dims=(100, 50), attention_dims=(100, 100, 1),
                       mlp3_dims=(150, 100, 100, 1), model='sarl', interaction_dims=None, query_env=True, precision='f32'):
        acts = np.ascontiguousarray(np.asarray(actions, dtype=np.float64).reshape(-1, 2))
        cfg = _lib.CnSarlConfig(n_actions=len(acts), with_om=int(bool(with_om)), cell_num=int(cell_num),
                                om_channel_size=int(om_channel_size), cell_size=float(cell_size), gamma=float(gamma),
                                with_global_state=int(bool(with_global_state)),
                                mlp1_dims=(C.c_int32 * 2)(*mlp1_dims), mlp2_dims=(C.c_int32 * 2)(*mlp2_dims),
                                attention_dims=(C.c_int32 * 3)(*attention_dims), mlp3_dims=(C.c_int32 * 4)(*mlp3_dims),
                                model={'sarl': 0, 'cadrl': 1, 'lstm_rl': 2}[model],
                                interaction_dims=(C.c_int32 * 4)(*(interaction_dims or (0, 0, 0, 0))),
                                constant_velocity_model=0 if query_env else 1,
                                precision=_lib.PRECISIONS.index(precision) if isinstance(precision, str) else int(precision))
        check(self._lib.cn_sarl_configure(self._h, C.byref(cfg), acts.ctypes.data_as(C.c_void_p)))
        self.sarl = dict(n_actions=len(acts), in_dim=13 + (cell_num ** 2 * om_channel_size if with_om else 0),
                         actions=acts, model=model, pairwise=bool(interaction_dims))

    def sarl_set_weights(self, state_dict):
        order = {'cadrl': CADRL_PARAM_ORDER, 'lstm_rl': LSTM_PARAM_ORDER}.get(self.sarl['model'], SARL_PARAM_ORDER)
        if self.sarl.get('pairwise'):
            order = LSTM_PAIRWISE_MLP1_ORDER + order
        tensors, temporaries = [], []
        for k in order:
            t = state_dict[k]
            if not (t.device == self.device and t.dtype == torch.float32 and t.is_contiguous()):
                t = t.detach().to(device=self.device, dtype=torch.float32).contiguous()
                temporaries.append(t)
            tensors.append(t)
        ptrs = (C.c_void_p * len(tensors))(*[t.data_ptr() for t in tensors])
        check(self._lib.cn_sarl_set_weights(self._h, ptrs))
        for t in temporaries:
            t.record_stream(self._stream)
        self._sarl_weights_keepalive = tensors

    def sarl_select(self, want_values=True, best=None, action=None, want_attention=False):
        K = self.sarl['n_actions']
        if best is None:
            best = self._new((self.B,), torch.int32)
        if action is None:
            action = self._new((self.B, 2), torch.float64)
        assert best.dtype == torch.int32 and best.is_contiguous() and action.dtype == torch.float64 and action.is_contiguous()
        out = dict(values=self._new((self.B, K), torch.float64) if want_values else None, best=best, action=action)
        if want_attention:
            out['attention'] = self._new((self.B, K, self.H), torch.float32)
            check(self._lib.cn_sarl_select_attention(self._h, _ptr(out['values']), _ptr(out['best']), _ptr(out['action']),
                                                     _ptr(out['attention'])))
        else:
            check(self._lib.cn_sarl_select(self._h, _ptr(out['values']), _ptr(out['best']), _ptr(out['action'])))
        return out

    def sarl_export(self, name):
        K, H = self.sarl['n_actions'], self.H
        if name == 'reward':
            t, which = self._new((self.B, K), torch.float64), 0
        elif name == 'V':
            t, which = self._new((self.B, K), torch.float32), 1
        elif name == 'next_obs':
            t, which = self._new((self.B, H, 5), torch.float64), 2
        elif name == 'om':
            t, which = self._new((self.B, H, self.sarl['in_dim'] - 13), torch.float32), 3
        elif name == 'X':
            d = self.sarl['in_dim']
            ks = max((d + 15) // 16 * 4, ((d + 3) // 4 + 4) // 5 * 5)
            tiles = (self.B * K + 15) // 16
            t, which = self._new((tiles, H, ks, 4, 16), torch.float32), 4
        else:
            raise KeyError(name)
        check(self._lib.cn_sarl_export(self._h, which, _ptr(t), t.numel() * t.element_size()))
        if name == 'X':
            t = t.permute(0, 4, 1, 2, 3).reshape(-1, H, t.shape[2] * 4)[:self.B * K, :, :self.sarl['in_dim']]
            t = t.reshape(self.B, K, H, -1)
        return t

    def sarl_explore(self, sel, epsilon, mask=None, want_explored=True):
        m, _ = self._borrow(mask, torch.uint8, (self.B,))
        explored = self._new((self.B,), torch.uint8) if want_explored else None
        check(self._lib.cn_sarl_explore(self._h, float(epsilon), _ptr(m), _ptr(sel['best']), _ptr(sel['action']),
                                        _ptr(explored)))
        sel['explored'] = explored
        return sel

    def sarl_transform(self, out=None, env_stride=0, sort_humans=None):
        if out is None:
            out = self._new((self.B, self.H, self.sarl['in_dim']), torch.float32)
        assert out.dtype == torch.float32 and out.device.type == self.device.type
        if sort_humans is None:
            sort_humans = self.sarl['model'] == 'lstm_rl'
        check(self._lib.cn_sarl_transform(self._h, C.c_void_p(out.data_ptr()), int(env_stride), int(bool(sort_humans))))
        return out

    def sarl_sampler(self, traj, rew, info, dmin, act, alive, done, action):
        B, T, H, D = traj.shape
        if B != self.B or H != self.H:
            raise ValueError('traj is [%d, T, %d, D]; the engine holds %d envs x %d humans' % (B, H, self.B, self.H))
        specs = ((traj, torch.float32, (B, T, H, D)), (act, torch.int32, (T, B)), (rew, torch.float64, (T, B)),
                 (dmin, torch.float64, (T, B)), (info, torch.uint8, (T, B)), (alive, torch.uint8, (B,)), (done, torch.uint8, (B,)),
                 (action, torch.float64, (B, 2)))
        for t_, dt, shape in specs:
            if not self._dense(t_, dt, shape, pinned_ok=any(t_ is w for w in (info, rew, dmin, act))):
                raise ValueError('sarl_sampler: expected a contiguous %s %s tensor on %s, got %s %s on %s (contiguous: %s)'
                                 % (dt, shape, self.device, t_.dtype, tuple(t_.shape), t_.device, t_.is_contiguous()))
        keep = (traj, rew, info, dmin, act, alive, done, action)
        alive_engine = weakref.ref(self)
        lib, h, V = self._lib, self._h, C.c_void_p
        p_traj, p_rew, p_inf, p_dmn, p_act = traj.data_ptr(), rew.data_ptr(), info.data_ptr(), dmin.data_ptr(), act.data_ptr()
        p_alive, p_done, p_action = V(alive.data_ptr()), V(done.data_ptr()), V(action.data_ptr())
        sort = int(self.sarl['model'] == 'lstm_rl')
        stride = T * H * D

        def step(t, epsilon):
            eng = alive_engine()
            if eng is None or eng._h is not h or not h.value:
                raise RuntimeError('sarl_sampler: the engine has been closed')
            check(lib.cn_sarl_sample_step(h, epsilon, p_alive, V(p_act + 4 * B * t), p_action, V(p_traj + 4 * H * D * t), stride, sort,
                                          V(p_rew + 8 * B * t), p_done, V(p_inf + B * t), V(p_dmn + 8 * B * t)))
        step.keep = keep
        return step

    def sarl_values(self, states, out=None):
        n = int(states.shape[0])
        if not self._dense(states, torch.float32, (n, self.H, 13)):
            raise ValueError('sarl_values: expected a contiguous float32 [n, %d, 13] tensor on %s' % (self.H, self.device))
        if out is None:
            out = self._new((n,), torch.float32)
        check(self._lib.cn_sarl_values(self._h, _ptr(states), n, _ptr(out)))
        return out

    def sarl_state_values(self, state8, theta=None, sort_humans=False, out=None):
        shape = tuple(getattr(state8, 'shape', np.shape(state8)))
        if len(shape) < 3 or shape[-2:] != (self.A, 8):
            raise ValueError('sarl_state_values: state8 must be [n, %d, 8] (or [..., %d, 8]), got %s' % (self.A, self.A, shape))
        n = int(np.prod(shape[:-2], dtype=np.int64))
        tshape = None
        if theta is not None:
            tshape = tuple(getattr(theta, 'shape', np.shape(theta)))
            if int(np.prod(tshape, dtype=np.int64)) != n or (len(tshape) != 1 and tshape != shape[:-2]):
                raise ValueError('sarl_state_values: theta must be [%d] or %s, got %s' % (n, shape[:-2], tshape))
        if out is None:
            out = self._new((n,), torch.float32)
        elif not self._dense(out, torch.float32, (n,)):
            raise ValueError('sarl_state_values: out must be a contiguous float32 [%d] tensor on %s' % (n, self.device))
        s, temporary_s = self._borrow(state8, torch.float64, shape)
        th, temporary_th = self._borrow(theta, torch.float64, tshape)
        check(self._lib.cn_sarl_state_values(self._h, _ptr(s), _ptr(th), n, int(bool(sort_humans)), _ptr(out)))
        self._release(temporary_s, temporary_th)
        return out
```

include/crowdnav_amd.h:

```cpp
#ifndef CROWDNAV_AMD_H
#define CROWDNAV_AMD_H

#include <stdint.h>

#ifdef __cplusplus
extern "C" {
#endif

typedef enum cn_status {
    CN_OK = 0,
    CN_ERR_INVALID = -1,
    CN_ERR_UNSUPPORTED = -2,
    CN_ERR_HIP = -3,
    CN_ERR_NO_DEVICE = -4
} cn_status;

enum { CN_NOTHING = 0, CN_DANGER = 1, CN_REACH_GOAL = 2, CN_COLLISION = 3, CN_TIMEOUT = 4 };
enum { CN_ROBOT_EXTERNAL = 0, CN_ROBOT_ORCA = 1 };
enum { CN_HOLONOMIC = 0, CN_UNICYCLE = 1 };
enum { CN_CIRCLE_CROSSING = 0, CN_SQUARE_CROSSING = 1, CN_MIXED = 2 };

typedef struct cn_config {
    int32_t num_envs;
    int32_t num_humans;
    double time_step;
    double time_limit;
    double success_reward;
    double collision_penalty;
    double discomfort_dist;
    double discomfort_penalty_factor;
    int32_t robot_visible;
    int32_t robot_policy;
    double robot_safety_space;
    double human_safety_space;
    double neighbor_dist;
    int32_t max_neighbors;
    int32_t scenario_rule;
    double time_horizon;
    double time_horizon_obst;
    double circle_radius;
    double square_width;
    double human_radius;
    double human_v_pref;
    double robot_radius;
    double robot_v_pref;
    int32_t randomize_attributes;
    int32_t device;
    int32_t robot_kinematics;
    int32_t flags;
} cn_config;

#define CN_FLAG_ASYNC_SCENARIO_FILL 1

typedef struct cn_engine cn_engine;

const char* cn_last_error(void);
#define CN_ABI_VERSION 12
int cn_abi_version(void);

int cn_create(const cn_config* cfg, cn_engine** out);
int cn_destroy(cn_engine* e);
int cn_set_stream(cn_engine* e, void* hip_stream);
int cn_sync(cn_engine* e);

int cn_set_state(cn_engine* e, const double* state8, const double* global_time);
int cn_get_state(cn_engine* e, double* state8, double* global_time);
int cn_set_theta(cn_engine* e, const double* theta);
int cn_get_theta(cn_engine* e, double* theta);
int cn_get_human_count(cn_engine* e, int32_t* count);
int cn_drop_robot_sim(cn_engine* e);
int cn_drop_sims(cn_engine* e);
int cn_set_robot_sim(cn_engine* e, const float* radii_host, float max_speed);

int cn_reset(cn_engine* e, const uint32_t* seeds, const uint8_t* mask, uint64_t* draws);

int cn_orca(cn_engine* e, float* out_vel);

int cn_step(cn_engine* e, const double* action, int update, double* reward, uint8_t* done, uint8_t* info,
            double* dmin, double* action_out, float* orca_vel, double* obs);

typedef struct cn_rollout_io {
    uint32_t seed_base;
    uint32_t seed_mod;
    int64_t episode_limit;
    int64_t env_offset;
    int64_t env_stride;
    int32_t record_capacity;
    uint8_t* ep_outcome;
    int32_t* ep_steps;
    double* ep_return;
    double* ep_time;
    int32_t* ep_danger;
    double* ep_danger_dmin_sum;
    int32_t* ep_count;
    int32_t* cur_steps;
    double* cur_return;
    int32_t* cur_danger;
    double* cur_danger_dmin_sum;
    uint8_t* active;
    uint64_t* transitions;
    double* summary;
    double* blocks;
    int32_t blocks_records;
    uint64_t* env_transitions;
} cn_rollout_io;

int cn_set_gamma(cn_engine* e, double gamma);

int cn_rollout_begin(cn_engine* e, const cn_rollout_io* io);
int cn_rollout(cn_engine* e, const cn_rollout_io* io, int n_steps);

enum {
    CN_COUNT_ROLLOUT_KERNELS = 0,
    CN_COUNT_SCHEDULED_KERNELS = 1,
    CN_COUNT_RING_FILLS = 2,
    CN_COUNT_ASYNC_FILLS = 3,
    CN_COUNT_SARL_NARROW = 4,
    CN_COUNT_SARL_DECIDE_STEPS = 5
};
#define CN_LAUNCH_COUNTERS 6
int cn_launch_counts(cn_engine* e, uint64_t* counts_host);

int cn_lagged_fills(cn_engine* e, uint64_t* count_host);

enum {
    CN_ROUTE_GENERIC = 0,
    CN_ROUTE_FUSED = 1,
    CN_ROUTE_FUSED_SPLIT = 2,
    CN_ROUTE_SHARD = 3
};
int cn_rollout_route(cn_engine* e, int n_steps, int* route_host);

enum { CN_MODEL_SARL = 0, CN_MODEL_CADRL = 1, CN_MODEL_LSTM_RL = 2 };

typedef struct cn_sarl_config {
    int32_t n_actions;
    int32_t with_om;
    int32_t cell_num;
    int32_t om_channel_size;
    double cell_size;
    double gamma;
    int32_t with_global_state;
    int32_t mlp1_dims[2];
    int32_t mlp2_dims[2];
    int32_t attention_dims[3];
    int32_t mlp3_dims[4];
    int32_t model;
    int32_t interaction_dims[4];
    int32_t constant_velocity_model;
    int32_t precision;
} cn_sarl_config;
enum { CN_PRECISION_F32 = 0, CN_PRECISION_F16X2 = 1 };

int cn_sarl_configure(cn_engine* e, const cn_sarl_config* cfg, const double* actions_host);
int cn_sarl_set_weights(cn_engine* e, const float* const* params_host_array);
int cn_sarl_select(cn_engine* e, double* values, int32_t* best, double* action);
int cn_sarl_select_attention(cn_engine* e, double* values, int32_t* best, double* action, float* attention);
enum {
    CN_SARL_ROUTE_LDS_TILE = 0,
    CN_SARL_ROUTE_LDS_CHUNKED = 1,
    CN_SARL_ROUTE_NARROW = 2,
    CN_SARL_ROUTE_REG_SARL = 3,
    CN_SARL_ROUTE_REG_SARL_CHUNK = 4,
    CN_SARL_ROUTE_REG_CADRL = 5,
    CN_SARL_ROUTE_REG_LSTM = 6,
    CN_SARL_ROUTE_REG_LSTM2 = 7,
    CN_SARL_ROUTE_SPLIT_F16 = 8
};
int cn_sarl_network_route(cn_engine* e, int* route_host);
int cn_sarl_explore(cn_engine* e, double epsilon, const uint8_t* mask, int32_t* best, double* action,
                    uint8_t* explored);
int cn_sarl_transform(cn_engine* e, float* out, int64_t env_stride, int sort_humans);
int cn_sarl_sample_step(cn_engine* e, double epsilon, uint8_t* alive, int32_t* best, double* action, float* state_out,
                        int64_t env_stride, int sort_humans, double* reward, uint8_t* done, uint8_t* info, double* dmin);
int cn_sarl_values(cn_engine* e, const float* states, int64_t n, float* out);
int cn_sarl_export(cn_engine* e, int which, void* dst, uint64_t bytes);

int cn_rollout_step(cn_engine* e, const cn_rollout_io* io, const double* action);

#define CN_RECORD_FIELDS 6
#define CN_SUMMARY_FIELDS 8
#define CN_RECORD_BLOCK_DOUBLES(K) (1 + (K) * CN_RECORD_FIELDS)
int cn_rollout_records(cn_engine* e, const cn_rollout_io* io, int max_records, double* blocks);
int cn_gather_records(cn_engine* e, void* rccl_comm, int n_ranks, int max_records, const double* blocks,
                      double* blocks_all);
int cn_records_summary(cn_engine* e, int64_t n_envs, int max_records, int record_capacity, const double* blocks,
                       double* summary);
int cn_rollout_summary(cn_engine* e, const cn_rollout_io* io, double* summary);

int cn_mt_random(cn_engine* e, uint32_t seed, int n, double* out);

typedef struct cn_trainer cn_trainer;
int cn_trainer_create(const cn_sarl_config* net, int num_humans, int max_batch, int device, cn_trainer** out);
int cn_trainer_destroy(cn_trainer* t);
int cn_trainer_set_stream(cn_trainer* t, void* hip_stream);
int cn_train_step(cn_trainer* t, float* const* params_host_array, float* const* momentum_host_array, const float* states,
                  const float* values, int64_t rows, const int64_t* index, int64_t n, double lr, double momentum_factor,
                  double* loss_sum);
int cn_trainer_steps(const cn_trainer* t, int64_t* steps_host);

typedef struct cn_trace_out {
    double*  state8;
    int32_t* episode;
    int32_t* step;
    double*  reward;
    uint8_t* info;
    double*  dmin;
} cn_trace_out;
int cn_rollout_trace(cn_engine* e, const cn_rollout_io* io, int n_steps, const cn_trace_out* out);

int cn_rollout_actions(cn_engine* e, const cn_rollout_io* io, int n_steps, const double* actions, const cn_trace_out* out);

typedef struct cn_lookahead_out {
    double*  ret;
    uint8_t* info;
    int32_t* steps;
    double*  time;
    double*  final_state8;
    double*  final_theta;
} cn_lookahead_out;
int cn_lookahead_actions(cn_engine* e, int n_steps, int n_candidates, const double* actions ,
                         const cn_lookahead_out* out);

enum { CN_HUMANS_ORCA = 0, CN_HUMANS_CONSTANT_VELOCITY = 1 };
int cn_lookahead_set_human_model(cn_engine* e, int model);
int cn_lookahead_get_human_model(const cn_engine* e, int* model_host);

int cn_lookahead_paths(cn_engine* e, int n_steps, int n_candidates,
                       const double* actions   ,
                       const double* human_vel ,
                       const cn_lookahead_out* out);
int cn_lookahead_paths_values(cn_engine* e, int n_steps, int n_candidates, const double* actions,
                              const double* human_vel, const cn_lookahead_out* out,
                              int sort_humans, float* value, double* score);
typedef struct cn_plan_cfg cn_plan_cfg;
typedef struct cn_plan cn_plan;
int cn_plan_cem_paths (cn_engine* e, const cn_plan_cfg* cfg, const cn_plan* plan,
                       const double* human_vel, uint32_t counter);
int cn_plan_mppi_paths(cn_engine* e, const cn_plan_cfg* cfg, const cn_plan* plan,
                       const double* human_vel, double temperature, int fit_std, uint32_t counter);

enum { CN_MODES_MEAN = 0, CN_MODES_MIN = 1 };
typedef struct cn_path_modes {
    int32_t n_modes;
    int32_t reduce;
    double  risk_penalty;
    const double* human_vel;
    const double* weight;
} cn_path_modes;
typedef struct cn_modes_out {
    double*  score;
    double*  risk;
    int32_t* worst_mode;
    uint8_t* worst_info;
    int32_t* worst_steps;
    double*  worst_time;
    double*  ret;
    uint8_t* info;
    int32_t* steps;
    double*  time;
} cn_modes_out;
int cn_lookahead_modes(cn_engine* e, int n_steps, int n_candidates, const double* actions ,
                       const cn_path_modes* modes, const cn_modes_out* out);
int cn_plan_cem_modes (cn_engine* e, const cn_plan_cfg* cfg, const cn_plan* plan, const cn_path_modes* modes, uint32_t counter);
int cn_plan_mppi_modes(cn_engine* e, const cn_plan_cfg* cfg, const cn_plan* plan, const cn_path_modes* modes,
                       double temperature, int fit_std, uint32_t counter);

int cn_sarl_state_values(cn_engine* e, const double* state8, const double* theta, int64_t n, int sort_humans, float* value);

int cn_lookahead_values(cn_engine* e, int n_steps, int n_candidates, const double* actions, const cn_lookahead_out* out,
                        int sort_humans, float* value, double* score);

typedef struct cn_plan_cfg {
    int32_t n_steps;
    int32_t n_candidates;
    int32_t n_elites;
    int32_t iterations;
    int32_t bootstrap;
    int32_t sort_humans;
    double  init_std;
    double  min_std;
    double  smoothing;
    uint64_t seed;
} cn_plan_cfg;

typedef struct cn_plan {
    double* mean;
    double* std;
    double* best_actions;
    double* best_score;
    double* action;
    double* candidates;
    cn_lookahead_out look;
    float*  value;
    double* score;
    int32_t* order;
} cn_plan;


int cn_plan_reset(cn_engine* e, const cn_plan_cfg* cfg, const cn_plan* plan, const uint8_t* mask );
int cn_plan_draw(cn_engine* e, const cn_plan_cfg* cfg, const cn_plan* plan, uint32_t counter);
int cn_plan_refit(cn_engine* e, const cn_plan_cfg* cfg, const cn_plan* plan, int keep_best);
int cn_plan_cem(cn_engine* e, const cn_plan_cfg* cfg, const cn_plan* plan, uint32_t counter);
int cn_plan_shift(cn_engine* e, const cn_rollout_io* io, const cn_plan_cfg* cfg, const cn_plan* plan);
int cn_plan_rollout(cn_engine* e, const cn_rollout_io* io, int n_real_steps, const cn_plan_cfg* cfg, const cn_plan* plan,
                    uint32_t counter);

int cn_plan_mppi_update(cn_engine* e, const cn_plan_cfg* cfg, const cn_plan* plan, double temperature, int fit_std, int keep_best);
int cn_plan_mppi(cn_engine* e, const cn_plan_cfg* cfg, const cn_plan* plan, double temperature, int fit_std, uint32_t counter);
int cn_plan_mppi_rollout(cn_engine* e, const cn_rollout_io* io, int n_real_steps, const cn_plan_cfg* cfg, const cn_plan* plan,
                         double temperature, int fit_std, uint32_t counter);

enum { CN_PREDICT_CONSTANT_VELOCITY = 0, CN_PREDICT_TO_GOAL = 1 };
int cn_predict(cn_engine* e, int n_steps, int n_modes,
               const int32_t* models ,
               double* human_vel     );

typedef struct cn_predictors {
    int32_t n_modes;
    int32_t model[8];
    int32_t reduce;
    double  risk_penalty;
    double* human_vel;
    const double* weight;
} cn_predictors;
int cn_plan_cem_predict_rollout (cn_engine* e, const cn_rollout_io* io, int n_real_steps, const cn_plan_cfg* cfg,
                                 const cn_plan* plan, const cn_predictors* pred, uint32_t counter);
int cn_plan_mppi_predict_rollout(cn_engine* e, const cn_rollout_io* io, int n_real_steps, const cn_plan_cfg* cfg,
                                 const cn_plan* plan, const cn_predictors* pred, double temperature, int fit_std,
                                 uint32_t counter);

int cn_predict_orca(cn_engine* e, int n_steps, int n_modes, int mode,
                    double* human_vel );
int cn_plan_cem_predict_orca_rollout (cn_engine* e, const cn_rollout_io* io, int n_real_steps, const cn_plan_cfg* cfg,
                                      const cn_plan* plan, const cn_predictors* pred, int orca_mode, uint32_t counter);
int cn_plan_mppi_predict_orca_rollout(cn_engine* e, const cn_rollout_io* io, int n_real_steps, const cn_plan_cfg* cfg,
                                      const cn_plan* plan, const cn_predictors* pred, int orca_mode, double temperature,
                                      int fit_std, uint32_t counter);

int cn_predict_orca_robot(cn_engine* e, int n_steps, int n_modes, int mode,
                          const double* robot_actions ,
                          int64_t env_stride          ,
                          double* human_vel           );
int cn_plan_cem_predict_orca_nominal_rollout (cn_engine* e, const cn_rollout_io* io, int n_real_steps, const cn_plan_cfg* cfg,
                                              const cn_plan* plan, const cn_predictors* pred, int orca_mode, uint32_t counter);
int cn_plan_mppi_predict_orca_nominal_rollout(cn_engine* e, const cn_rollout_io* io, int n_real_steps, const cn_plan_cfg* cfg,
                                              const cn_plan* plan, const cn_predictors* pred, int orca_mode, double temperature,
                                              int fit_std, uint32_t counter);

#ifdef __cplusplus
}
#endif
#endif
```

Baseline: 1.523 billion.

## Precompute first ORCA step of ring scenarios in the background fill pass

Adds a ring_first_step_kernel that solves the first ORCA velocity for each freshly generated ring scenario during the lagged fill on the side stream. When an episode ends, the fused split rollout can then adopt the precomputed first-step velocity instead of spending a stalled step to restage and re-solve. The per-env adoption bitmask is carried through the shared flag word. The cost is extra ring memory, an extra kernel per fill, invalidation memsets on every state change, and more complex restart logic that must stay consistent with the robot-sim state.

New measurement: 1.561 billion, median of 6. 1.03x the previous value.

```diff
diff --git a/crowdnav_amd/_lib.py b/crowdnav_amd/_lib.py
--- a/crowdnav_amd/_lib.py
+++ b/crowdnav_amd/_lib.py
@@ -169,6 +169,8 @@
     'cn_launch_counts': (C.c_int, [_P, _P]),
     'cn_lagged_fills': (C.c_int, [_P, _P]),
     'cn_mt_random': (C.c_int, [_P, C.c_uint32, C.c_int, _P]),
+    'cn_fresh_starts': (C.c_int, [_P, _P]),
+    'cn_ring_slot': (C.c_int, [_P, C.c_int, C.c_int, _P, _P, C.POINTER(C.c_int)]),
     'cn_trainer_create': (C.c_int, [C.POINTER(CnSarlConfig), C.c_int, C.c_int, C.c_int, C.POINTER(_P)]),
     'cn_trainer_destroy': (C.c_int, [_P]),
     'cn_trainer_set_stream': (C.c_int, [_P, _P]),
diff --git a/crowdnav_amd/csrc/crowdnav_amd.hip b/crowdnav_amd/csrc/crowdnav_amd.hip
--- a/crowdnav_amd/csrc/crowdnav_amd.hip
+++ b/crowdnav_amd/csrc/crowdnav_amd.hip
@@ -166,6 +166,8 @@
     e->smem = cn::smem_bytes(P.nA, P.pairs, e->maxl, P.A, P.E);
 }
 
+static int rollout_route(const cn_engine* e, const double* action);
+
 static void read_knobs(cn_engine* e) {
     const cn_config* c = &e->cfg;
     cn::Params& P = e->P;
@@ -194,6 +196,7 @@
             if (hipOccupancyMaxActiveBlocksPerMultiprocessor(&per_cu, kernel, threads, e->smem) == hipSuccess)
                 e->split_slots = per_cu * prop.multiProcessorCount;
         });
+    e->ring.first_step = rollout_route(e, nullptr) == CN_ROUTE_FUSED_SPLIT;
 }
 
 static int alloc_state(cn_engine* e) {
@@ -315,7 +318,7 @@
 
 int cn_set_state(cn_engine* e, const double* state8, const double* global_time) {
     int rc = bind(e);
-    if (rc || (rc = e->ring.settle(e))) return rc;
+    if (rc || (rc = e->ring.settle(e)) || (rc = e->ring.forget_first_steps(e))) return rc;
     const int n = e->P.B * e->P.A;
     if (state8) hipLaunchKernelGGL(pack_state_kernel, dim3((n + 255) / 256), dim3(256), 0, e->stream, n, state8, e->S);
     if (global_time)
@@ -386,6 +389,8 @@
     int rc = bind(e);
     if (rc) return rc;
     if (!radii_host) return fail(CN_ERR_INVALID, "cn_set_robot_sim: NULL");
+    if ((rc = e->ring.settle(e)) || (rc = e->ring.forget_first_steps(e))) return rc;
+    e->ring.robot_sim_known = true;
     float* staged = reinterpret_cast<float*>(e->probe_key);
     CN_HIP(hipMemcpyAsync(staged, radii_host, sizeof(float) * e->P.A, hipMemcpyHostToDevice, e->stream));
     CN_HIP(hipStreamSynchronize(e->stream));
@@ -397,7 +402,8 @@
 
 int cn_drop_robot_sim(cn_engine* e) {
     int rc = bind(e);
-    if (rc) return rc;
+    if (rc || (rc = e->ring.settle(e)) || (rc = e->ring.forget_first_steps(e))) return rc;
+    e->ring.robot_sim_known = false;
     CN_HIP(hipMemsetAsync(e->S.rsim_valid, 0, (size_t)e->P.B, e->stream));
     if (e->P.kd)
         CN_HIP(hipMemset2DAsync(e->S.kd_valid, (size_t)e->P.A, 0, 1, (size_t)e->P.B, e->stream));
@@ -415,6 +421,7 @@
     int rc = bind(e);
     if (rc || (rc = e->ring.settle(e))) return rc;
     if (!seeds) return fail(CN_ERR_INVALID, "cn_reset: seeds is NULL");
+    if ((rc = e->ring.forget_first_steps(e))) return rc;
     if (e->ring.gen_wave)
         hipLaunchKernelGGL(cn::reset_wave_kernel, dim3(e->P.B), dim3(cn::kWave), 0, e->stream, e->P, e->C, e->S, seeds, mask,
                            draws);
@@ -502,6 +509,7 @@
     e->rollout_begun = false;
     if ((rc = upload_io(e, io))) return rc;
     e->rollout_begun = true, e->begin_seed_base = io->seed_base, e->begin_seed_mod = io->seed_mod;
+    if ((rc = e->ring.forget_first_steps(e))) return rc;
     return e->ring.begin(e, io->seed_mod);
 }
 
@@ -772,6 +780,45 @@
     return CN_OK;
 }
 
+int cn_fresh_starts(cn_engine* e, uint64_t* counts_host) {
+    int rc = bind(e);
+    if (rc) return rc;
+    if (!counts_host) return fail(CN_ERR_INVALID, "cn_fresh_starts: counts_host is NULL");
+    unsigned int dev[2] = {0u, 0u};
+    CN_HIP(hipMemcpyAsync(dev, e->S.fresh_counts, sizeof(dev), hipMemcpyDeviceToHost, e->stream));
+    CN_HIP(hipStreamSynchronize(e->stream));
+    counts_host[0] = dev[0], counts_host[1] = dev[1], counts_host[2] = e->ring.first_step_kernels;
+    return CN_OK;
+}
+
+int cn_ring_slot(cn_engine* e, int env, int slot, double* state8_host, float* vel0_host, int* ok_host) {
+    int rc = bind(e);
+    if (rc || (rc = e->ring.settle(e))) return rc;
+    if (!state8_host || !vel0_host || !ok_host) return fail(CN_ERR_INVALID, "cn_ring_slot: NULL argument");
+    if (env < 0 || env >= e->P.B || slot < 0 || slot >= e->P.ring_mod)
+        return fail(CN_ERR_INVALID, "cn_ring_slot: (env, slot) = (%d, %d) outside %d envs x %d slots", env, slot, e->P.B, e->P.ring_mod);
+    const int A = e->P.A;
+    const size_t idx = (size_t)env * e->P.ring_mod + slot;
+    std::vector<double2> pos((size_t)A), goal((size_t)A), rv((size_t)A);
+    std::vector<float2> vel((size_t)A, make_float2(0.0f, 0.0f));
+    uint8_t ok = 0;
+    CN_HIP(hipStreamSynchronize(e->stream));
+    CN_HIP(hipMemcpy(pos.data(), e->S.ring_pos + idx * A, sizeof(double2) * A, hipMemcpyDeviceToHost));
+    CN_HIP(hipMemcpy(goal.data(), e->S.ring_goal + idx * A, sizeof(double2) * A, hipMemcpyDeviceToHost));
+    CN_HIP(hipMemcpy(rv.data(), e->S.ring_rv + idx * A, sizeof(double2) * A, hipMemcpyDeviceToHost));
+    if (e->ring.first_step) {
+        CN_HIP(hipMemcpy(vel.data(), e->S.ring_vel0 + idx * A, sizeof(float2) * A, hipMemcpyDeviceToHost));
+        CN_HIP(hipMemcpy(&ok, e->S.ring_vel0_ok + idx, 1, hipMemcpyDeviceToHost));
+    }
+    for (int a = 0; a < A; ++a) {
+        double* s = state8_host + 8 * (size_t)a;
+        s[0] = pos[a].x, s[1] = pos[a].y, s[2] = 0.0, s[3] = 0.0, s[4] = goal[a].x, s[5] = goal[a].y, s[6] = rv[a].x, s[7] = rv[a].y;
+        vel0_host[2 * a] = vel[a].x, vel0_host[2 * a + 1] = vel[a].y;
+    }
+    *ok_host = ok;
+    return CN_OK;
+}
+
 int cn_launch_counts(cn_engine* e, uint64_t* counts_host) {
     if (!e || !counts_host) return fail(CN_ERR_INVALID, "cn_launch_counts: NULL argument");
     for (int i = 0; i < CN_LAUNCH_COUNTERS; ++i) counts_host[i] = e->launch_counts[i];
diff --git a/crowdnav_amd/csrc/engine_host.h b/crowdnav_amd/csrc/engine_host.h
--- a/crowdnav_amd/csrc/engine_host.h
+++ b/crowdnav_amd/csrc/engine_host.h
@@ -55,6 +55,9 @@
     int fill_queue_wgs = 1;
     int* ep_snap = nullptr;
     uint64_t lagged_fills = 0;
+    bool first_step = false;
+    bool robot_sim_known = false;
+    uint64_t first_step_kernels = 0;
 
     void configure(cn_engine* e, int compute_units);
     int create(cn_engine* e);
@@ -64,6 +67,7 @@
     int around_launch(cn_engine* e, int n_steps, Launch&& launch);
     int settle(cn_engine* e);
     int drain(cn_engine* e);
+    int forget_first_steps(cn_engine* e);
 };
 
 struct cn_engine {
diff --git a/crowdnav_amd/csrc/rollout_fused.h b/crowdnav_amd/csrc/rollout_fused.h
--- a/crowdnav_amd/csrc/rollout_fused.h
+++ b/crowdnav_amd/csrc/rollout_fused.h
@@ -358,7 +358,8 @@
         SPLIT_PROBE_WAIT(0, split_barrier());
         const int2 words = make_int2(s.flag[0], ((ASSIST & kAssistHead) || kSplitProbe) ? s.flag[1] : 0);
         float4 me = s.kin[pq], other = s.kin[pr.my_slot];
-        const bool ended = __builtin_amdgcn_readfirstlane(words.x) != 0;
+        const int word = __builtin_amdgcn_readfirstlane(words.x);
+        const bool ended = (word & 1) != 0;
         const unsigned int pred = ((ASSIST & kAssistHead) || kSplitProbe) ? (unsigned int)__builtin_amdgcn_readfirstlane(words.y) : 0u;
         if (!ended) ++u;
         if (u >= n_steps) {
@@ -367,8 +368,9 @@
         }
         const bool head = (ASSIST & kAssistHead) ? split_has_head<MAXL>(pred, u, n_steps) : false;
         SPLIT_PROBE_AFTER_1(pred, head);
-        if (ended) {
-            if (lane < P.nA) {
+        const bool staged = word != 0;
+        if (staged) {
+            if (lane < P.nA && (ended || ((word >> (1 + lane / P.A)) & 1) != 0)) {
                 const double2 p = s.posd[lane];
                 px = p.x, py = p.y;
                 s.kin[lane] = reinterpret_cast<const float4*>(s.d2)[lane];
@@ -376,12 +378,12 @@
             CN_FUSED_SYNC();
             me = s.kin[pq], other = s.kin[pr.my_slot];
         }
-        if (ended) rsum = pair_rsum(s, pr);
+        if (staged) rsum = pair_rsum(s, pr);
         if (lane < P.pairs) fused_pair_body(P, s, pr, range_sq, rsum, me, other, [] {});
         SPLIT_PROBE_WAIT(1, split_barrier());
         fused_candidates<MAXL>(P, s, lane);
         CN_FUSED_SYNC();
-        if (ended) solved = lane < P.nA && s.sol[lane < P.nA ? lane : 0].w != 0.0f;
+        if (staged) solved = lane < P.nA && s.sol[lane < P.nA ? lane : 0].w != 0.0f;
         const unsigned long long nm = fused_solve<MAXL, kSplitOrcaPrio>(P, s, lane, solved, rx, ry, nullptr, head ? pred : 0u, [&] {
             if (head) SPLIT_PROBE_WAIT(2, split_barrier());
         });
@@ -485,7 +487,7 @@
 #endif
     if constexpr (SPLIT) {
         float2* const vel = reinterpret_cast<float2*>(s.act);
-        if (L.lane == 0) s.flag[0] = 1, s.flag[1] = 0;
+        if (L.lane == 0) s.flag[0] = 1, s.flag[1] = 0, s.flag[2] = 0, s.flag[3] = 0;
         split_barrier();
         bool skip = true;
         const bool mirror = L.lane >= 16 && L.lane < 16 + P.nA;
@@ -499,6 +501,7 @@
             if (mirror) r.px = px, r.py = py, r.gx = gx, r.gy = gy, m_running = run != 0;
         };
         copy_to_mirror();
+        int v0_off = 0;
         SPLIT_PROBE_DECL();
         for (int u = 0;;) {
             SPLIT_PROBE_WAIT(0, split_barrier());
@@ -509,7 +512,8 @@
             const AgentRegs r0 = r;
             double act_x = 0.0, act_y = 0.0, new_vx = 0.0, new_vy = 0.0;
             if (!skip && (L.lane < P.nA || mirror)) {
-                const float2 mine = vel[m_lane], robots = vel[m_ebase];
+                const float2 mine = vel[v0_off + m_lane], robots = vel[v0_off + m_ebase];
+                v0_off = 0;
                 act_x = (double)robots.x, act_y = (double)robots.y;
                 new_vx = m_robot ? act_x : (double)mine.x;
                 new_vy = m_robot ? act_y : (double)mine.y;
@@ -545,11 +549,13 @@
                 }
             }
             bool ended = false;
+            unsigned int adopt = 0u;
+            bool done = false, v0_ok = false;
+            float2 v0 = make_float2(0.0f, 0.0f);
             if (!skip) {
                 const double2 rp = make_double2(__shfl(r0.px, L.ebase), __shfl(r0.py, L.ebase));
                 if (L.valid) s.closest[L.lane] = swept_distance(r0, L.a > 0, rp, act_x, act_y, new_vx, new_vy, K.dt, s.rad[L.ebase]);
                 CN_FUSED_SYNC();
-                bool done = false;
                 if (running) {
                     const double disc_t = s.disc[ep.cur_steps < kMaxDiscount ? ep.cur_steps : kMaxDiscount - 1];
                     const StepOutcome o = reduce_env(P, s, L.ebase, ep.gtime, K);
@@ -561,16 +567,35 @@
                         const cn_rollout_io io = *iop;
                         const StateView S = *Sd;
                         AgentRegs next = r;
-                        load_from_ring(P, S, L, (ep.ep_count + 1) % P.ring_mod, next);
-                        CN_END_EPISODE(P, S, io, L.env, L.a == 0, K.limit, o.info, ep, r = next; theta = 1.5707963267948966);
+                        const int next_slot = (ep.ep_count + 1) % P.ring_mod;
+                        load_from_ring(P, S, L, next_slot, next);
+                        const size_t next_idx = (size_t)L.env * P.ring_mod + next_slot;
+                        const float2 v0_next = S.ring_vel0[next_idx * P.A + L.a];
+                        const bool ok_next = S.ring_vel0_ok[next_idx] != 0;
+                        CN_END_EPISODE(P, S, io, L.env, L.a == 0, K.limit, o.info, ep,
+                                       r = next; theta = 1.5707963267948966; v0 = v0_next; v0_ok = ok_next);
                     }
                 }
-                ended = __ballot(done) != 0ull;
-            }
-            if (ended) stage_agent(P, s, L, r, K.hsafety, kin_stage);
-            if (ended) copy_to_mirror();
-            if (L.lane == 0) s.flag[0] = ended ? 1 : 0;
-            skip = ended;
+                const unsigned long long ended_lanes = __ballot(done);
+                ended = ended_lanes != 0ull;
+                if (ended && u < n_steps && __ballot(done && v0_ok) == ended_lanes)
+                    for (int el = 0; el < P.E; ++el) adopt |= (unsigned int)((ended_lanes >> (el * P.A)) & 1ull) << (1 + el);
+            }
+            if (ended) {
+                AgentRegs st = r;
+                if (adopt != 0u && done) {
+                    st.px = r.px + (double)v0.x * K.dt;
+                    st.py = r.py + (double)v0.y * K.dt;
+                    st.vx = (double)v0.x, st.vy = (double)v0.y;
+                    vel[P.nA + L.lane] = v0;
+                }
+                stage_agent(P, s, L, st, K.hsafety, kin_stage);
+                copy_to_mirror();
+                if (adopt != 0u) v0_off = ((adopt >> (1 + m_ebase / P.A)) & 1u) != 0u ? P.nA : 0;
+                if (L.lane == 0 && u < n_steps) s.flag[adopt != 0u ? 2 : 3] += adopt != 0u ? __popc(adopt) : 1;
+            }
+            if (L.lane == 0) s.flag[0] = ended ? (adopt != 0u ? (int)adopt : 1) : 0;
+            skip = ended && adopt == 0u;
             if constexpr ((ASSIST & kAssistHead) != 0 && CN_SPLIT_HEAD_TAIL_PRIO != 0) __builtin_amdgcn_s_setprio(0);
             if (u >= n_steps) break;
         }
@@ -664,6 +689,13 @@
     const unsigned long long wt_exit = __builtin_amdgcn_s_memrealtime();
 #endif
     const StateView S = *Sd;
+    if constexpr (SPLIT) {
+        if (L.lane == 0) {
+            const int adopted = s.flag[2], redone = s.flag[3];
+            if (adopted != 0) atomicAdd(&S.fresh_counts[0], (unsigned int)adopted);
+            if (redone != 0) atomicAdd(&S.fresh_counts[1], (unsigned int)redone);
+        }
+    }
     if (L.valid) CN_STORE_AGENT(S, L.gi, r);
     const cn_rollout_io io = *iop;
     if (robot) CN_STORE_EPISODE(P, S, io, L.env, ep, theta);
@@ -679,4 +711,61 @@
 #endif
 }
 
-}
+constexpr int kFirstStepWgs = 2048;
+__global__ __launch_bounds__(kWave) void ring_first_step_kernel(Params P_in, StateView S) {
+    constexpr int MAXL = 5;
+    Params P = P_in;
+    P.A = 6, P.NC = 5, P.E = 2, P.nA = 12, P.pairs = 60, P.threads = 64;
+    const Smem s = carve<MAXL>(P);
+    const int lane = threadIdx.x;
+    const int el = lane / P.A;
+    const bool agent = lane < P.nA;
+    build_pairs(P, s, true);
+    if (lane == 0) s.kin[P.nA] = make_float4(std::numeric_limits<float>::infinity(), std::numeric_limits<float>::infinity(), 0.0f, 0.0f);
+    CN_FUSED_SYNC();
+    const PairRow pr = pair_row_of(P, s, lane);
+    const float range_sq = P.orca.neighbor_dist * P.orca.neighbor_dist;
+    const int slots = P.B * P.ring_mod;
+    const int listed = __builtin_amdgcn_readfirstlane(S.redo_count[1]);
+    const int n = listed < slots ? listed : slots;
+    for (int k = 2 * (int)blockIdx.x; k < n; k += 2 * kFirstStepWgs) {
+        const bool both = k + 1 < n;
+        const int listed_idx = S.first_list[k + ((el == 1 && both) ? 1 : 0)];
+        const int ring_idx = listed_idx < 0 ? 0 : (listed_idx < slots ? listed_idx : slots - 1);
+        Lane L;
+        L.lane = lane, L.a = lane - el * P.A, L.ebase = el * P.A, L.env = ring_idx / P.ring_mod, L.valid = agent;
+        L.gi = (size_t)L.env * P.A + (agent ? L.a : 0);
+        const size_t ri = (size_t)ring_idx * P.A + (agent ? L.a : 0);
+        const double2 p = S.ring_pos[ri], g = S.ring_goal[ri], q = S.ring_rv[ri], cur = S.rv[L.gi];
+        const bool have = S.rsim_valid[L.env] != 0;
+        const float rr_kept = S.rsim_radius[L.gi], ms_kept = S.rsim_max_speed[L.env];
+        AgentRegs r;
+        r.px = p.x, r.py = p.y, r.vx = 0.0, r.vy = 0.0, r.gx = g.x, r.gy = g.y, r.rad = q.x, r.vpref = q.y;
+        const float robot_max_speed = have ? ms_kept : (float)cur.y;
+        if (agent) s.rview[lane] = have ? rr_kept : (float)(cur.x + 0.01 + P.robot_safety);
+        stage_agent(P, s, L, r, P.human_safety, s.kin);
+        CN_FUSED_SYNC();
+        if (lane < P.pairs) {
+            float4 sol4, start4;
+            fused_pair_phase(P, s, pr, range_sq, pair_rsum(s, pr), [&] {
+                preferred_velocity(r, (L.a == 0) ? robot_max_speed : (float)r.vpref, agent, sol4, start4);
+            });
+            if (agent) {
+                s.sol[lane] = sol4;
+                s.res[lane] = start4;
+            }
+        }
+        CN_FUSED_SYNC();
+        fused_candidates<MAXL>(P, s, lane);
+        CN_FUSED_SYNC();
+        float rx, ry;
+        fused_solve<MAXL>(P, s, lane, agent, rx, ry, nullptr);
+        if (agent && (el == 0 || both)) {
+            S.ring_vel0[ri] = make_float2(rx, ry);
+            if (L.a == 0) S.ring_vel0_ok[ring_idx] = 1;
+        }
+        CN_FUSED_SYNC();
+    }
+}
+
+}
diff --git a/crowdnav_amd/csrc/scenario_ring.h b/crowdnav_amd/csrc/scenario_ring.h
--- a/crowdnav_amd/csrc/scenario_ring.h
+++ b/crowdnav_amd/csrc/scenario_ring.h
@@ -104,10 +104,11 @@
 constexpr int kRedoLanes = 4096;
 __global__ __launch_bounds__(kWave) void ring_fill_begin_kernel(int B, const int* ep_word, int* ep_snap, int* redo_count) {
     const int b = blockIdx.x * blockDim.x + threadIdx.x;
-    if (b == 0) *redo_count = 0;
+    if (b == 0) redo_count[0] = 0, redo_count[1] = 0;
     if (b < B) ep_snap[b] = __hip_atomic_load(&ep_word[b], __ATOMIC_RELAXED, __HIP_MEMORY_SCOPE_AGENT);
 }
-__global__ __launch_bounds__(kWave) void ring_fill_kernel(Params P, ScenarioCfg C, StateView S, RolloutView R, const int* ep_snap) {
+__global__ __launch_bounds__(kWave) void ring_fill_kernel(Params P, ScenarioCfg C, StateView S, RolloutView R, const int* ep_snap,
+                                                         int first_step) {
     const int idx = blockIdx.x * blockDim.x + threadIdx.x;
     const int D = P.ring_mod;
     if (idx >= P.B * D) return;
@@ -125,16 +126,26 @@
     if (past_episode_limit(*io, c)) return;
     const uint32_t seed = episode_seed(*io, c);
     const int ring_idx = b * D + ordinal % D;
+    if (first_step) {
+        S.ring_vel0_ok[ring_idx] = 0;
+        const unsigned long long m = __ballot(1);
+        const int lane = threadIdx.x & (kWave - 1), leader = __ffsll((long long)m) - 1;
+        int base = 0;
+        if (lane == leader) base = atomicAdd(&S.redo_count[1], __popcll(m));
+        base = __shfl(base, leader);
+        S.first_list[base + __popcll(m & ((1ull << lane) - 1ull))] = ring_idx;
+    }
     Mt19937Head head;
     generate_scenario(C, head, seed, (size_t)ring_idx * P.A, S.ring_pos, nullptr, S.ring_goal, S.ring_rv);
     if (head.dead()) S.redo_list[atomicAdd(S.redo_count, 1)] = make_int2(ring_idx, (int)seed);
 }
 
-__global__ __launch_bounds__(kWave) void ring_redo_kernel(Params P, ScenarioCfg C, StateView S) {
+__global__ __launch_bounds__(kWave) void ring_redo_kernel(Params P, ScenarioCfg C, StateView S, int first_step) {
     const int lane = blockIdx.x * blockDim.x + threadIdx.x;
     const int n = *S.redo_count;
     for (int k = lane; k < n; k += kRedoLanes) {
         const int2 job = S.redo_list[k];
+        if (first_step) S.ring_vel0_ok[job.x] = 0;
         Mt19937 rng{S.ring_mt_key + lane, kRedoLanes, 0};
         generate_scenario(C, rng, (uint32_t)job.y, (size_t)job.x * P.A, S.ring_pos, nullptr, S.ring_goal, S.ring_rv);
     }
diff --git a/crowdnav_amd/csrc/scenario_ring_host.h b/crowdnav_amd/csrc/scenario_ring_host.h
--- a/crowdnav_amd/csrc/scenario_ring_host.h
+++ b/crowdnav_amd/csrc/scenario_ring_host.h
@@ -1,6 +1,6 @@
 #pragma once
 #include "engine_host.h"
-#include "scenario_ring.h"
+#include "rollout_fused.h"
 
 static inline void swap_levels(cn::StateView& S) { std::swap(S.ring_filled_in, S.ring_filled_out); }
 
@@ -33,7 +33,11 @@
         (rc = dev_alloc(e, &S.ring_mt_key, gen_wave ? (size_t)64 : (size_t)624 * cn::kRedoLanes)) ||
         (rc = dev_alloc(e, &S.redo_list, gen_wave ? (size_t)1 : (size_t)P.B * P.ring_mod)) ||
         (rc = dev_alloc(e, &ep_snap, mode == Fill::Beside ? (size_t)P.B : (size_t)1)) ||
-        (rc = dev_alloc(e, &S.redo_count, (size_t)1)) ||
+        (rc = dev_alloc(e, &S.redo_count, (size_t)2)) ||
+        (rc = dev_alloc(e, &S.ring_vel0, first_step ? n * P.ring_mod : (size_t)1)) ||
+        (rc = dev_alloc(e, &S.ring_vel0_ok, first_step ? (size_t)P.B * P.ring_mod : (size_t)1)) ||
+        (rc = dev_alloc(e, &S.first_list, first_step ? (size_t)P.B * P.ring_mod : (size_t)1)) ||
+        (rc = dev_alloc(e, &S.fresh_counts, (size_t)2)) ||
         (rc = dev_alloc(e, &S.ring_filled_in, (size_t)P.B)) || (rc = dev_alloc(e, &S.ring_filled_out, (size_t)P.B)) ||
         (rc = dev_alloc(e, &S.ring_ready, work_list ? slots : (size_t)1)) ||
         (rc = dev_alloc(e, &S.ring_claim, work_list ? slots : (size_t)1)) ||
@@ -86,6 +90,12 @@
 
 inline int ScenarioRing::settle(cn_engine* e) { return plan.pending ? drain(e) : CN_OK; }
 
+inline int ScenarioRing::forget_first_steps(cn_engine* e) {
+    if (!first_step) return CN_OK;
+    CN_HIP(hipMemsetAsync(e->S.ring_vel0_ok, 0, (size_t)e->P.B * e->P.ring_mod, e->stream));
+    return CN_OK;
+}
+
 inline int ScenarioRing::begin(cn_engine* e, uint32_t seed_mod) {
     const cn::RolloutView R{e->io_dev, e->discount, e->discount_len};
     e->S.cache_n = (gen_wave && scenario_cache && seed_mod <= (uint32_t)cn::kScenarioCacheMax) ? (int)seed_mod : 0;
@@ -121,6 +131,11 @@
     }
     const int fill_lanes = e->P.B * e->P.ring_mod;
     const dim3 fill_grid((fill_lanes + cn::kWave - 1) / cn::kWave), redo_grid(cn::kRedoLanes / cn::kWave);
+    const int fs_flag = first_step ? 1 : 0;
+    const auto solve_first_steps = [&](hipStream_t on) {
+        hipLaunchKernelGGL(cn::ring_first_step_kernel, dim3(cn::kFirstStepWgs), dim3(cn::kWave), e->smem, on, e->P, e->S);
+        first_step_kernels += 1;
+    };
     if (plan_says.take_levels) {
         CN_HIP(hipStreamWaitEvent(e->stream, fill_done, 0));
         swap_levels(e->S);
@@ -129,23 +144,27 @@
         if (gen_wave) {
             hipLaunchKernelGGL(cn::ring_fill_wave_kernel, dim3(fill_lanes), dim3(cn::kWave), 0, e->stream, e->P, e->C, e->S, R);
         } else {
-            CN_HIP(hipMemsetAsync(e->S.redo_count, 0, sizeof(int), e->stream));
-            hipLaunchKernelGGL(cn::ring_fill_kernel, fill_grid, dim3(cn::kWave), 0, e->stream, e->P, e->C, e->S, R, nullptr);
-            hipLaunchKernelGGL(cn::ring_redo_kernel, redo_grid, dim3(cn::kWave), 0, e->stream, e->P, e->C, e->S);
+            CN_HIP(hipMemsetAsync(e->S.redo_count, 0, 2 * sizeof(int), e->stream));
+            hipLaunchKernelGGL(cn::ring_fill_kernel, fill_grid, dim3(cn::kWave), 0, e->stream, e->P, e->C, e->S, R, nullptr, fs_flag);
+            hipLaunchKernelGGL(cn::ring_redo_kernel, redo_grid, dim3(cn::kWave), 0, e->stream, e->P, e->C, e->S, fs_flag);
+            if (first_step) solve_first_steps(e->stream);
         }
         swap_levels(e->S);
         e->launch_counts[CN_COUNT_RING_FILLS] += 1;
     }
     if (plan_says.lagged_fill) CN_HIP(hipEventRecord(rollout_done, e->stream));
+    const bool sim_known_before = robot_sim_known;
     launch(R, (const int*)e->S.ring_filled_in);
     CN_HIP(hipGetLastError());
+    if (e->P.robot_orca) robot_sim_known = true;
     if (plan_says.lagged_fill) {
         hipStream_t fs = fill_streams[0];
         CN_HIP(hipStreamWaitEvent(fs, rollout_done, 0));
         hipLaunchKernelGGL(cn::ring_fill_begin_kernel, dim3(grid_lanes(e)), dim3(cn::kWave), 0, fs, e->P.B, e->S.ep_word, ep_snap,
                            e->S.redo_count);
-        hipLaunchKernelGGL(cn::ring_fill_kernel, fill_grid, dim3(cn::kWave), 0, fs, e->P, e->C, e->S, R, (const int*)ep_snap);
-        hipLaunchKernelGGL(cn::ring_redo_kernel, redo_grid, dim3(cn::kWave), 0, fs, e->P, e->C, e->S);
+        hipLaunchKernelGGL(cn::ring_fill_kernel, fill_grid, dim3(cn::kWave), 0, fs, e->P, e->C, e->S, R, (const int*)ep_snap, fs_flag);
+        hipLaunchKernelGGL(cn::ring_redo_kernel, redo_grid, dim3(cn::kWave), 0, fs, e->P, e->C, e->S, fs_flag);
+        if (first_step && sim_known_before) solve_first_steps(fs);
         CN_HIP(hipEventRecord(fill_done, fs));
         e->launch_counts[CN_COUNT_RING_FILLS] += 1;
         lagged_fills += 1;
diff --git a/crowdnav_amd/csrc/step_kernels.h b/crowdnav_amd/csrc/step_kernels.h
--- a/crowdnav_amd/csrc/step_kernels.h
+++ b/crowdnav_amd/csrc/step_kernels.h
@@ -70,6 +70,10 @@
     double* wg_partial;
     double* group_partial;
     unsigned* tickets;
+    float2* ring_vel0;
+    uint8_t* ring_vel0_ok;
+    int* first_list;
+    unsigned int* fresh_counts;
 };
 
 constexpr int kEpilogueGroups = 32;
diff --git a/crowdnav_amd/engine.py b/crowdnav_amd/engine.py
--- a/crowdnav_amd/engine.py
+++ b/crowdnav_amd/engine.py
@@ -643,6 +643,19 @@
         check(self._lib.cn_lagged_fills(self._h, C.byref(lagged)))
         return dict(zip(_lib.LAUNCH_COUNTERS, (int(v) for v in out)), lagged_fills=int(lagged.value))
 
+    def fresh_starts(self):
+        out = (C.c_uint64 * 3)()
+        check(self._lib.cn_fresh_starts(self._h, out))
+        return dict(adopted=int(out[0]), redone=int(out[1]), kernels=int(out[2]))
+
+    def ring_slot(self, env, slot):
+        state8 = np.zeros((self.A, 8), np.float64)
+        vel0 = np.zeros((self.A, 2), np.float32)
+        ok = C.c_int(0)
+        check(self._lib.cn_ring_slot(self._h, int(env), int(slot), state8.ctypes.data_as(C.c_void_p),
+                                     vel0.ctypes.data_as(C.c_void_p), C.byref(ok)))
+        return state8, vel0, bool(ok.value)
+
     def rollout_route(self, n_steps):
         route = C.c_int(-1)
         check(self._lib.cn_rollout_route(self._h, int(n_steps), C.byref(route)))
diff --git a/include/crowdnav_amd.h b/include/crowdnav_amd.h
--- a/include/crowdnav_amd.h
+++ b/include/crowdnav_amd.h
@@ -123,6 +123,9 @@
 
 int cn_lagged_fills(cn_engine* e, uint64_t* count_host);
 
+int cn_fresh_starts(cn_engine* e, uint64_t* counts_host);
+int cn_ring_slot(cn_engine* e, int env, int slot, double* state8_host, float* vel0_host, int* ok_host);
+
 enum {
     CN_ROUTE_GENERIC = 0,
     CN_ROUTE_FUSED = 1,
```
